# latk/hbetune.rs

Hardware: AMD Instinct MI355X
Metric: GP fit+predict/sec (n=4096,d=8,f64) (higher is better)
Workload: dtype f64; 1 GPU; M: rosenbrock d=8 n=4096 f64, Matern nu=5/2 x constant + white noise; fixed-work fit = 3 L-BFGS runs x 150 lml+gradient evaluations + K^-1, then predict mean+variance at m=1600; evals_per_fit=450, n_not_pd=0, m_candidates=1600, parallelism=replicas x1 (independent fits per GPU, no collective)

## Files before the change

csrc/dag_plan.hpp:

```cpp
#pragma once
#include <algorithm>
#include <cstdint>
#include <cstdio>
#include <queue>
#include <string>
#include <vector>

#include "engine.hpp"

namespace hbegp {

inline int dag_split_point(int lo, int hi) { return lo + (hi - lo) / 2; }

struct DagPlan {
  std::vector<DagTask> tasks;
  std::vector<int> totals;
  double gflop = 0;
  double gflop_lauum = 0;
  int n_lauum = 0;
  int n_leaf = 0;
  double sim_us = 0;
  double crit_us = 0;
};

// ... 444 lines not shown
        }
        uprev[i] = DagGate{c, cnt};
      }
      if (lauum) {
        int a = -1;
        for (const auto& gr : kgroups)
          if (gr.second == k + 1) a = gr.first;
        if (a >= 0) {
          const double gl0 = plan_.gflop;
          const int c = new_counter();
          int cnt = 0;
          const std::vector<DagGate> waits = {rowfin[k], kprev};
          if (a > 0) {
            Op l{};
            l.flags = (uint16_t)(DAGF_ABUF | DAGF_BBUF | DAGF_AKM | DAGF_BKM | DAGF_CKINV | cont);
            l.r0 = 0; l.r1 = a; l.c0 = 0; l.c1 = a; l.lower = true; l.k0 = a; l.k1 = k + 1;
            for (const Tile& tl : tiles_of(l, false)) {
              const DagTask tk = make(l, tl, &cu);
              push(tk, waits, c, -1, cu);
              ++cnt;
              plan_.n_lauum++;
            }
          }
          {
            Op l{};
            l.flags = DAGF_ABUF | DAGF_BBUF | DAGF_AKM | DAGF_BKM | DAGF_CKINV;
            l.r0 = a; l.r1 = k + 1; l.c0 = 0; l.c1 = k + 1; l.lower = true; l.k0 = a; l.k1 = k + 1; l.klim = 4; l.tri_a = true; l.tri_b = true;
            for (const Tile& tl : tiles_of(l, false)) {
              const DagTask tk = make(l, tl, &cu);
              push(tk, waits, c, -1, cu);
              ++cnt;
              plan_.n_lauum++;
            }
          }
          kprev = DagGate{c, cnt};
          g_lauum += plan_.gflop - gl0;
        }
      }
    }
    (void)g0;
    plan_.gflop_lauum = g_lauum;
  }
  Sub rl_inverse(int lo, int hi, const std::vector<RlNode>& nodes, const std::vector<DagGate>& leafc) {
    Sub out;
    out.lo = lo; out.hi = hi;
    if (hi - lo == 1) {
      out.rowfin.assign(1, leafc[lo]);
      out.all = leafc[lo];
      return out;
    }
    const int mid = dag_split_point(lo, hi);
    const RlNode* nd = nullptr;
    for (const RlNode& cand : nodes)
      if (cand.lo == lo && cand.hi == hi) nd = &cand;
    const bool small = std::max(mid - lo, hi - mid) <= small_h_;
    const Sub left = rl_inverse(lo, mid, nodes, leafc);
    const Sub right = rl_inverse(mid, hi, nodes, leafc);
    if (lo == top_lo_ && hi == top_hi_) { top_mid_ = mid; top_right_all_ = right.all; top_left_all_ = left.all; }
    double cu = 0;
    Op u{};
    u.flags = DAGF_A3 | DAGF_BBUF | DAGF_BKM;
    u.r0 = mid; u.r1 = hi; u.c0 = lo; u.c1 = mid; u.k0 = lo; u.k1 = mid; u.klim = 2; u.tri_b = true;
    const std::vector<Tile> ut = tiles_of(u, small);
    const DagGate uall{new_counter(), (int)ut.size()};
    for (const Tile& tl : ut) {
      const DagTask tk = make(u, tl, &cu);
      DagGate lrow{nd->lrow[tl.bi - mid], plan_.totals[nd->lrow[tl.bi - mid]]};
      push(tk, {lrow, left.all}, uall.cnt, -1, cu);
    }
    Op x{};
    x.flags = DAGF_ABUF | DAGF_BKM | DAGF_CBUF | DAGF_NEG;
    x.r0 = mid; x.r1 = hi; x.c0 = lo; x.c1 = mid; x.k0 = mid; x.k1 = hi; x.klim = 3; x.tri_a = true; x.crit = 2;
    const std::vector<Tile> xt = tiles_of(x, small);
    RowGates xrow(hi);
    for (int i = mid; i < hi; ++i) xrow[i] = DagGate{new_counter(), count_row(xt, i)};
    const DagGate xall{new_counter(), (int)xt.size()};
    for (const Tile& tl : xt) {
      const DagTask tk = make(x, tl, &cu);
      push(tk, {fine_ ? right.rowfin[tl.bi - mid] : right.all, uall}, xrow[tl.bi].cnt, xall.cnt, cu);
    }
    out.rowfin.resize(hi - lo);
    for (int j = lo; j < mid; ++j) out.rowfin[j - lo] = left.rowfin[j - lo];
    for (int j = mid; j < hi; ++j) out.rowfin[j - lo] = xrow[j];
    out.all = xall;
    return out;
  }

  void order() {
    const int nt = (int)plan_.tasks.size(), nc = (int)plan_.totals.size();
    std::vector<std::vector<int>> waiters(nc);
    for (int i = 0; i < nt; ++i)
      for (int w = 0; w < plan_.tasks[i].nwait; ++w) waiters[plan_.tasks[i].wcnt[w]].push_back(i);
    std::vector<double> bl(nt, 0.0), blc(nc, 0.0);
    for (int i = nt - 1; i >= 0; --i) {
      const DagTask& t = plan_.tasks[i];
      double tail = 0;
      for (int q = 0; q < DAG_MAXSIG; ++q)
        if (t.sig[q] != DAG_NOSIG) tail = std::max(tail, blc[t.sig[q]]);
      bl[i] = t.cost * 0.1 + tail;
      for (int w = 0; w < t.nwait; ++w) blc[t.wcnt[w]] = std::max(blc[t.wcnt[w]], bl[i]);
    }
    plan_.crit_us = *std::max_element(bl.begin(), bl.end());
    std::vector<int> count(nc, 0), missing(nt, 0);
    typedef std::pair<double, int> Pri;
    std::priority_queue<Pri> ready;
    for (int i = 0; i < nt; ++i) {
      missing[i] = plan_.tasks[i].nwait;
      if (missing[i] == 0) ready.push({bl[i], -i});
    }
    typedef std::pair<double, int> Ev;
    std::priority_queue<Ev, std::vector<Ev>, std::greater<Ev>> running;
    std::vector<DagTask> out;
    out.reserve(nt);
    std::vector<int> out_idx;
    std::vector<double> start(nt, 0.0);
    out_idx.reserve(nt);
    int idle = nwg_;
    double now = 0;
    while ((int)out.size() < nt) {
      while (idle > 0 && !ready.empty()) {
        const int i = -ready.top().second;
        ready.pop();
        out.push_back(plan_.tasks[i]);
        out_idx.push_back(i);
        start[i] = now;
        running.push({now + plan_.tasks[i].cost * 0.1, i});
        --idle;
      }
      if (running.empty()) break;
      const Ev e = running.top();
      running.pop();
      now = e.first;
      ++idle;
      const DagTask& t = plan_.tasks[e.second];
      for (int q = 0; q < DAG_MAXSIG; ++q) {
        if (t.sig[q] == DAG_NOSIG) continue;
        const int c = t.sig[q];
        if (++count[c] == plan_.totals[c])
          for (int wtr : waiters[c])
            if (--missing[wtr] == 0) ready.push({bl[wtr], -wtr});
      }
    }
    while (!running.empty()) { now = running.top().first; running.pop(); }
    if ((int)out.size() == nt) {
      plan_.tasks.swap(out);
      plan_.sim_us = now;
    }
  }

 public:
  void set_big128(bool on, bool with_acc = false) { big128_ = on; big128_acc_ = on && with_acc; }
};

inline std::string dag_plan_validate(const DagPlan& plan, int nblocks_total) {
  const int nc = (int)plan.totals.size(), nt = (int)plan.tasks.size();
  const int words = (nc + 63) / 64;
  char buf[256];
  std::vector<int> count(nc, 0);
  std::vector<uint64_t> counter_known((size_t)nc * words, 0), cur(words);
  const int nt64 = nblocks_total * 4;
  struct Cell { int writer = -1; std::vector<int> readers; };
  constexpr int NBUF = 8;
  std::vector<Cell> cells[NBUF];
  for (int b = 0; b < NBUF; ++b) cells[b].resize((size_t)nt64 * nt64);
  std::vector<std::vector<uint64_t>> known(nt);
  auto hb = [&](int a, int b) -> bool {
    for (int q = 0; q < DAG_MAXSIG; ++q) {
      const int c = plan.tasks[a].sig[q];
      if (c != DAG_NOSIG && ((known[b][c / 64] >> (c % 64)) & 1u) != 0) return true;
    }
    return false;
  };
  for (int i = 0; i < nt; ++i) {
    const DagTask& t = plan.tasks[i];
    if (t.kind == DAG_GEMM_128x128 && (t.flags & DAGF_CINIT)) {
      snprintf(buf, sizeof buf, "task %d: the 128x128 tile cannot continue a sum (flags %x)", i, t.flags);
      return buf;
    }
    if (t.kind == DAG_GEMM_32x64 && (t.flags & (DAGF_AKM | DAGF_BKM | DAGF_CINIT | DAGF_CKINV))) {
      snprintf(buf, sizeof buf, "task %d: the 32x64 one-shot tile reads both operands [outer][k] and writes W1/W2/W3 (flags %x)", i, t.flags);
      return buf;
    }
    if ((t.kind == DAG_GEMM_128x64 || t.kind == DAG_GEMM_64x64) && (t.flags & DAGF_CINIT)) {
      if (!(t.flags & DAGF_ACC) || (t.flags & DAGF_NEG) || t.kend <= t.kbeg) {
        snprintf(buf, sizeof buf, "task %d: DAGF_CINIT needs DAGF_ACC, no DAGF_NEG and a non-empty contraction range (flags %x, k [%d, %d))", i,
                 t.flags, t.kbeg, t.kend);
        return buf;
      }
    }
    std::fill(cur.begin(), cur.end(), 0);
    for (int w = 0; w < t.nwait; ++w) {
      const int c = t.wcnt[w];
      if (c >= nc) return "wait on an unknown counter";
      if (t.wval[w] != plan.totals[c]) {
        snprintf(buf, sizeof buf, "task %d waits for %d of counter %d (total %d): partial waits are not allowed", i, t.wval[w], c, plan.totals[c]);
        return buf;
      }
      if (count[c] < t.wval[w]) {
        snprintf(buf, sizeof buf, "task %d waits on counter %d = %d but only %d earlier tasks bump it: queue order is not topological", i,
                 c, t.wval[w], count[c]);
        return buf;
      }
      cur[c / 64] |= 1ull << (c % 64);
      for (int q = 0; q < words; ++q) cur[q] |= counter_known[(size_t)c * words + q];
    }
    known[i] = cur;
    struct Acc { int buf, r, c; bool write; };
    std::vector<Acc> accs;
    auto rect = [&](int bufi, int r0, int r1, int c0, int c1, bool write) {
      for (int r = r0 / 32; r < (r1 + 31) / 32; ++r)
        for (int c = c0 / 64; c < (c1 + 63) / 64; ++c) accs.push_back({bufi, r, c, write});
    };
    auto cell = [&](int bufi, int r, int c, bool write) { accs.push_back({bufi, r, c, write}); };
    if (t.kind == DAG_LEAF) {
      const int b = t.row0 * 128;
      rect(0, b, b + 128, b, b + 128, false);
      rect(1, b, b + 128, b, b + 128, true);
      cell(4, t.row0, 0, true);
    } else {
      const int ta = (t.kind == DAG_GEMM_128x64 || t.kind == DAG_GEMM_128x128) ? 128 : (t.kind == DAG_GEMM_32x64 ? 32 : 64), tb = t.kind == DAG_GEMM_128x128 ? 128 : 64;
      const int ab = (t.flags & DAGF_A3) ? 7 : ((t.flags & DAGF_ABUF) ? 1 : 0), bb = (t.flags & DAGF_B3) ? 7 : ((t.flags & DAGF_BBUF) ? 1 : 0);
      const int cb = (t.flags & DAGF_CKINV) ? 6 : ((t.flags & DAGF_C3) ? 7 : ((t.flags & DAGF_CBUF) ? 1 : 0));
      if (t.kend <= t.kbeg) return "empty contraction range";
      if (t.flags & DAGF_AKM) rect(ab, t.kbeg, t.kend, t.row0, t.row0 + ta, false);
      else rect(ab, t.row0, t.row0 + ta, t.kbeg, t.kend, false);
      if (t.flags & DAGF_BKM) rect(bb, t.kbeg, t.kend, t.col0, t.col0 + tb, false);
      else rect(bb, t.col0, t.col0 + tb, t.kbeg, t.kend, false);
      if (t.flags & DAGF_ACC) rect(cb, t.row0, t.row0 + ta, t.col0, t.col0 + tb, false);
      rect(cb, t.row0, t.row0 + ta, t.col0, t.col0 + tb, true);
    }
    for (const Acc& a : accs) {
      if (a.r >= nt64 || a.c >= nt64 || a.r < 0 || a.c < 0) return "tile outside the matrix";
      Cell& cell = cells[a.buf][(size_t)a.r * nt64 + a.c];
      if (a.buf >= 2 && a.buf != 6 && !a.write && cell.writer < 0) {
        snprintf(buf, sizeof buf, "task %d reads cell (%d,%d) of buffer %d that no earlier task has written", i, a.r, a.c, a.buf);
        return buf;
      }
      if (cell.writer >= 0 && cell.writer != i && !hb(cell.writer, i)) {
        snprintf(buf, sizeof buf, "task %d %s tile (%d,%d) of W%d written by task %d without waiting for it", i,
                 a.write ? "overwrites" : "reads", a.r, a.c, a.buf + 1, cell.writer);
        return buf;
      }
      if (a.write)
        for (int rd : cell.readers)
          if (rd != i && !hb(rd, i)) {
            snprintf(buf, sizeof buf, "task %d overwrites tile (%d,%d) of W%d that task %d reads, without waiting for it", i, a.r, a.c,
                     a.buf + 1, rd);
            return buf;
          }
    }
    for (const Acc& a : accs) {
      Cell& cell = cells[a.buf][(size_t)a.r * nt64 + a.c];
      if (a.write) { cell.writer = i; cell.readers.clear(); }
      else if (cell.readers.empty() || cell.readers.back() != i) cell.readers.push_back(i);
    }
    for (int sq = 0; sq < DAG_MAXSIG; ++sq) {
      if (t.sig[sq] == DAG_NOSIG) continue;
      const int c = t.sig[sq];
      if (c >= nc) return "bump of an unknown counter";
      count[c]++;
      for (int q = 0; q < words; ++q) counter_known[(size_t)c * words + q] |= cur[q];
    }
  }
  for (int c = 0; c < nc; ++c)
    if (count[c] != plan.totals[c]) return "counter total mismatch";
  return "";
}

}
```

csrc/hbegp.cpp:

```cpp
#include "../include/hbegp.h"

#include <hip/hip_runtime_api.h>

#include <algorithm>
#include <atomic>
#include <queue>
#include <cmath>
#include <cstdarg>
#include <cstdio>
#include <cstdlib>
#include <cstring>
#include <limits>
#include <memory>
#include <mutex>
#include <string>
#include <thread>
#include <type_traits>
#include <vector>

#include "dag_plan.hpp"
#include "engine.hpp"
#include "lbfgsb.hpp"
#include "lbfgs_step.hpp"

// ... 412 lines not shown
    gemm(g, PhaseTimer::GEMM);
  }
  {
    GemmLaunch g{};
    g.nops = need_x ? 2 : 1;
    GemmOp& syrk = g.op[0];
    syrk = base;
    syrk.A = L21; syrk.B = L21; syrk.C = W1;
    syrk.ci0 = mid; syrk.cj0 = mid; syrk.mi = hi - mid; syrk.nj = hi - mid; syrk.c_lower = 1;
    syrk.k0 = lo; syrk.k1 = mid; syrk.alpha_neg = 1; syrk.beta_one = 1;
    GemmOp& u = g.op[1];
    u = base;
    u.A = L21; u.B = W2; u.C = W1;
    u.b_kmajor = 1;
    u.ci0 = mid; u.mi = hi - mid; u.cj0 = lo; u.nj = mid - lo;
    u.k0 = lo; u.k1 = mid; u.klim = 2; u.maskB = 1;
    gemm(g, PhaseTimer::GEMM);
  }
  chol_inv_rec<T>(W1, W2, L21, ld, mid, mid + (hi - mid) / 2, hi, false, need_x, gemm, leaf);
  if (need_x) {
    GemmLaunch g{};
    g.nops = 1;
    GemmOp& op = g.op[0];
    op = base;
    op.A = W2; op.B = W1; op.C = W2;
    op.b_kmajor = 1;
    op.ci0 = mid; op.mi = hi - mid; op.cj0 = lo; op.nj = mid - lo;
    op.k0 = mid; op.k1 = hi; op.klim = 3; op.maskA = 1; op.alpha_neg = 1;
    gemm(g, PhaseTimer::GEMM);
  }
}

static double op_gflop(const GemmOp& op) {
  double pairs = 0;
  for (int i = 0; i < op.mi; ++i)
    for (int j = 0; j < (op.c_lower ? i + 1 : op.nj); ++j) {
      const int ti = op.ci0 + i, tj = op.cj0 + j;
      int ka = op.k0, kb = op.k1;
      if (op.klim == 1) kb = std::min(kb, tj + 1);
      if (op.klim == 2) ka = std::max(ka, tj);
      if (op.klim == 3) kb = std::min(kb, ti + 1);
      if (op.klim == 4) ka = std::max(ka, ti);
      for (int k = ka; k < kb; ++k) {
        double w = 1.0;
        if ((op.maskA && k == ti) || (op.maskB && k == tj)) w = 0.5;
        if (op.c_lower && ti == tj) w = std::min(w, 0.5);
        pairs += w;
      }
    }
  return pairs * 2.0 * 128.0 * 128.0 * 128.0 * 1e-9;
}

struct Sched {
  int* d_off = nullptr;
  unsigned* d_items = nullptr;
  int nwg = 0;
  int tile = 0;
};

static void tile_krange(const GemmOp& op, int ti, int tj, int* ka, int* kb) {
  *ka = op.k0; *kb = op.k1;
  if (op.klim == 1) *kb = std::min(*kb, tj + 1);
  if (op.klim == 2) *ka = std::max(*ka, tj);
  if (op.klim == 3) *kb = std::min(*kb, ti + 1);
  if (op.klim == 4) *ka = std::max(*ka, ti);
}

static bool build_sched(const GemmLaunch& g, int tile, std::vector<int>* off, std::vector<unsigned>* items, int* nwg_out) {
  const int f = NB / tile;
  struct It { double w; unsigned code; };
  std::vector<It> its;
  for (int oi = 0; oi < g.nops; ++oi) {
    GemmOp op = g.op[oi];
    op.ci0 *= f; op.cj0 *= f; op.mi *= f; op.nj *= f; op.k0 *= f; op.k1 *= f;
    for (int i = 0; i < op.mi; ++i)
      for (int j = 0; j < (op.c_lower ? i + 1 : op.nj); ++j) {
        int ka, kb;
        tile_krange(op, op.ci0 + i, op.cj0 + j, &ka, &kb);
        its.push_back({(double)(kb - ka) + 0.75, ((unsigned)oi << 30) | ((unsigned)i << 16) | (unsigned)j});
      }
  }
  const int ntiles = (int)its.size();
  const int occmax = tile == 128 ? 2 : 3;
  int nwg = 0;
  if (ntiles < 2048)
    for (int occ = occmax; occ >= 1; --occ)
      if (ntiles >= 2 * 256 * occ) { nwg = 256 * occ; break; }
  if (nwg == 0) return false;
  std::stable_sort(its.begin(), its.end(), [](const It& a, const It& b) { return a.w > b.w; });
  typedef std::pair<double, int> Load;
  std::priority_queue<Load, std::vector<Load>, std::greater<Load>> pq;
  for (int w = 0; w < nwg; ++w) pq.push({0.0, w});
  std::vector<std::vector<unsigned>> per(nwg);
  for (const It& it : its) {
    Load l = pq.top();
    pq.pop();
    per[l.second].push_back(it.code);
    pq.push({l.first + it.w, l.second});
  }
  off->assign(nwg + 1, 0);
  items->clear();
  for (int w = 0; w < nwg; ++w) {
    (*off)[w] = (int)items->size();
    items->insert(items->end(), per[w].begin(), per[w].end());
  }
  (*off)[nwg] = (int)items->size();
  *nwg_out = nwg;
  return true;
}

constexpr int DAG_MAX_VARIANTS = 4;
constexpr int DAG_CROWD_LEVELS = 3;
constexpr int DAG_CROWD_BUSY[DAG_CROWD_LEVELS] = {6, 12, 24};
constexpr int MAX_DEVS = 64;
struct DagPlanKey {
  int blocks, bk, small_h, nwg, lauum, rl, rl_group, rl_near, lauum_split, chain32, prog, big128;
  auto tie() const { return std::tie(blocks, bk, small_h, nwg, lauum, rl, rl_group, rl_near, lauum_split, chain32, prog, big128); }
  bool operator<(const DagPlanKey& o) const { return tie() < o.tie(); }
};
static std::atomic<int> g_dev_busy[MAX_DEVS];

template <typename T>
struct LooIn {
  int dev;
  hipStream_t s;
  int n, d, np, nu2;
  const T *X, *y, *alpha, *Xinv, *Kinv;
  const EvalParams* P;
};
template <typename T>
static int loo_tail(const LooIn<T>& in, T* mean, T* var, T* lpd, double* loo, double* grad);

template <typename T>
struct Slot {
  int dev = 0;
  hipStream_t stream = nullptr;
  T *Xalt = nullptr, *ldalt = nullptr;
  bool x_captured = false;
  T *W1 = nullptr, *W2 = nullptr, *Kinv[2] = {nullptr, nullptr}, *alpha[2] = {nullptr, nullptr};
  T* W3 = nullptr;
  T *ldiag = nullptr, *wbuf = nullptr;
  double *part_t = nullptr, *part_g = nullptr;
  EvalParams* dP = nullptr;
  EvalOut* dOut = nullptr;
  int* tickets = nullptr;
  unsigned long long* dag_trace = nullptr;
  int* dag_ctrl = nullptr;
  EvalParams* hP = nullptr;
  EvalOut* hOut = nullptr;
  void* small_slab = nullptr;
  size_t small_slab_bytes = 0;
  void* host_slab = nullptr;
  size_t host_slab_bytes = 0;
  hipGraphExec_t graph[DAG_MAX_VARIANTS + 1 + DAG_CROWD_LEVELS][2][2] = {};
  int best_idx = -1;
  double best_lml = -std::numeric_limits<double>::infinity();
  int best_run = 0, best_eval = 0;
  std::vector<double> best_theta;
  std::vector<double> best_params;
  int last_target = 0;
  int dag_variant = 1;
  unsigned long long seq = 0;
  bool ctrl_cleared = false;
  bool published = false;
  long long expect_ns = 0;
};

struct ProblemBase {
  hbegp_ctx* ctx = nullptr;
  int n = 0, d = 0, np = 0, nu2 = 5, n_slots = 1;
  bool is_f32 = false;
  virtual ~ProblemBase() {}
  virtual int eval(int dev, int slot, const double* theta, const double* lo, const double* hi, double* lml, double* grad) = 0;
  virtual int eval_loo(int dev, int slot, const double* theta, const double* lo, const double* hi, double* loo, double* grad) = 0;
  virtual int time_eval(int dev, int slot, const double* theta, int reps, double* phase_ms) = 0;
  virtual int time_concurrent(int dev, const double* theta, int reps, double* out) = 0;
};
struct hbegp_problem {
  std::unique_ptr<ProblemBase> impl;
};

template <typename T>
struct Problem : ProblemBase {
  std::vector<T*> Xd, yd;
  std::vector<std::vector<Slot<T>>> slots;
  std::vector<std::vector<Sched>> scheds;
  bool dag_ = false;
  bool dag_lauum_ = false;
  bool dag_rl_ = false;
  double dag_gflop_lauum = 0;
  struct DagVariant {
    int nwg = 0;
    std::vector<DagTask*> tasks;
    std::vector<DagTask> host_tasks;
  };
  std::vector<DagVariant> dag_var;
  std::unique_ptr<std::atomic<int>[]> busy_slots_;
  int dag_ntasks = 0, dag_nwg = 0;
  int dag_nvar_ = 1, dag_ncrowd_ = 0;
  unsigned long long dag_wait_ticks_ = 200000000ull;
  size_t dag_ctrl_bytes = 0;
  double dag_gflop = 0;
  bool adhoc_ = false;
  bool small_ = false;
  bool like_fit_ = false;
  bool hostio_ = true;
  bool eval_published() const { return hostio_ && !small_; }
  int leaf_dbg_ = 0;

  struct Pooled { int dev; void* p; size_t bytes; };
  std::vector<Pooled> pooled_;
  template <typename U>
  U* palloc(int dev, size_t count) {
    bool fresh = false;
    const size_t bytes = std::max<size_t>(16, sizeof(U) * count);
    void* q = g_pool.get(dev, bytes, &fresh);
    pooled_.push_back({dev, q, bytes});
    return static_cast<U*>(q);
  }

  Problem(hbegp_ctx* c, const T* X, const T* y, int n_, int d_, double nu, int n_slots_, bool single_shot = false, bool like_fit = false) {
    try {
      adhoc_ = single_shot;
      like_fit_ = like_fit;
      init(c, X, y, n_, d_, nu, n_slots_);
    } catch (...) {
      release();
      throw;
    }
  }

  void init(hbegp_ctx* c, const T* X, const T* y, int n_, int d_, double nu, int n_slots_) {
    ctx = c; n = n_; d = d_; np = round_up(n_, NB); n_slots = n_slots_;
    nu2 = std::isinf(nu) ? 0 : (int)std::lround(2 * nu);
    is_f32 = sizeof(T) == 4;
    leaf_dbg_ = env_int("HBEGP_LEAF_DBG", 0) & 16;
    small_ = np == NB && d <= SMALL_EVAL_MAXD && env_int("HBEGP_SMALL", 1) != 0;
    hostio_ = env_int("HBEGP_HOSTIO", 1) != 0;
    const size_t nn = (size_t)np * np;
    Xd.assign(c->devs.size(), nullptr);
    yd.assign(c->devs.size(), nullptr);
    slots.resize(c->devs.size());
    for (size_t di = 0; di < c->devs.size(); ++di) {
      HIPCHECK(hipSetDevice(c->devs[di]));
      slots[di].resize(n_slots);
      for (auto& s : slots[di]) {
        s.dev = c->devs[di];
        s.stream = g_stream_pool.get(s.dev);
      }
      hipStream_t st0 = slots[di][0].stream;
      Xd[di] = palloc<T>(c->devs[di], (size_t)n * d);
      yd[di] = palloc<T>(c->devs[di], np);
      HIPCHECK(hipMemsetAsync(yd[di], 0, sizeof(T) * np, st0));
      HIPCHECK(hipMemcpyAsync(Xd[di], X, sizeof(T) * (size_t)n * d, hipMemcpyHostToDevice, st0));
      HIPCHECK(hipMemcpyAsync(yd[di], y, sizeof(T) * n, hipMemcpyHostToDevice, st0));
      for (auto& s : slots[di]) {
        bool fresh1 = false, fresh2 = false, fk = false;
        s.W1 = static_cast<T*>(g_pool.get(s.dev, sizeof(T) * nn, &fresh1));
        s.W2 = static_cast<T*>(g_pool.get(s.dev, sizeof(T) * nn, &fresh2));
        for (int b = 0; b < 2; ++b) s.Kinv[b] = static_cast<T*>(g_pool.get(s.dev, sizeof(T) * nn, &fk));
        HIPCHECK(hipMemsetAsync(s.W2, 0, sizeof(T) * nn, st0));
        (void)fresh1; (void)fresh2; (void)fk;
        {
          auto up = [](size_t v) { return (v + 255) / 256 * 256; };
          const size_t b_vec = up(sizeof(T) * np);
          const size_t b_part_t = up(sizeof(double) * ((size_t)((np + 255) / 256) * np + 2 * (size_t)((np + 255) / 256) + 64));
          const size_t b_part_g = up(sizeof(double) * gradtrace_part_elems(np, d));
          const size_t b_p = up(sizeof(EvalParams)), b_o = up(sizeof(EvalOut));
          s.small_slab_bytes = 4 * b_vec + b_part_t + b_part_g + b_p + b_o + 256;
          bool fs = false;
          s.small_slab = g_pool.get(s.dev, s.small_slab_bytes, &fs);
          char* q = static_cast<char*>(s.small_slab);
          s.alpha[0] = reinterpret_cast<T*>(q); q += b_vec;
          s.alpha[1] = reinterpret_cast<T*>(q); q += b_vec;
          s.ldiag = reinterpret_cast<T*>(q); q += b_vec;
          s.wbuf = reinterpret_cast<T*>(q); q += b_vec;
          s.part_t = reinterpret_cast<double*>(q); q += b_part_t;
          s.part_g = reinterpret_cast<double*>(q); q += b_part_g;
          s.dP = reinterpret_cast<EvalParams*>(q); q += b_p;
          s.dOut = reinterpret_cast<EvalOut*>(q); q += b_o;
          s.tickets = reinterpret_cast<int*>(q);
          HIPCHECK(hipMemsetAsync(s.dOut, 0, b_o + 256, st0));
          const size_t h_p = up(sizeof(EvalParams));
          s.host_slab_bytes = h_p + up(sizeof(EvalOut));
          s.host_slab = g_host_pool.get(s.host_slab_bytes);
          s.hP = reinterpret_cast<EvalParams*>(s.host_slab);
          s.hOut = reinterpret_cast<EvalOut*>(static_cast<char*>(s.host_slab) + h_p);
          memset(s.hP, 0, sizeof(EvalParams));
          memset(s.hOut, 0, sizeof(EvalOut));
        }
      }
      HIPCHECK(hipStreamSynchronize(st0));
    }
    const int dag_env = env_int("HBEGP_DAG", -1);
    const int dag_min_blocks = env_int("HBEGP_DAG_MIN_BLOCKS", DAG_MIN_BLOCKS_FIT);
    dag_ = (dag_env < 0 ? np / NB >= dag_min_blocks : dag_env != 0) && !adhoc_ && np / NB >= 2;
    if (dag_) {
      int cus = 1 << 30;
      for (int dev : c->devs) {
        hipDeviceProp_t prop;
        HIPCHECK(hipGetDeviceProperties(&prop, dev));
        cus = std::min(cus, std::max(1, prop.multiProcessorCount));
      }
      const int forced = env_int("HBEGP_DAG_WG", 0);
      auto share_of = [&](int busy) {
        const int share = busy <= 1 ? cus : std::max(8, (cus * 112 / 100 / busy + 4) / 8 * 8);
        return forced > 0 ? forced : std::max(1, std::min(cus, share));
      };
      dag_lauum_ = env_int("HBEGP_DAG_LAUUM", 1) != 0;
      dag_rl_ = env_int("HBEGP_DAG_RL", np / NB <= 80 ? 1 : 0) != 0;
      static std::mutex cache_mu;
      static std::map<DagPlanKey, std::shared_ptr<const DagPlan>> cache;
      auto plan_for = [&](int nwg) {
        const DagPlanKey key = {np / NB, dag_stage_depth(is_f32), env_int("HBEGP_DAG_SMALLH", dag_rl_ ? 4 : 8), nwg, dag_lauum_, dag_rl_,
                                env_int("HBEGP_DAG_RL_GROUP", 32), env_int("HBEGP_DAG_RL_NEAR", 1),
                                env_int("HBEGP_DAG_LAUUM_SPLIT", n_slots <= 1 ? 1 : 0),
                                env_int("HBEGP_DAG_CHAIN32", 1),
                                env_int("HBEGP_DAG_PROG", np / NB <= DAG_PROG_MAX_BLOCKS ? 1 : 0),
                                env_int("HBEGP_DAG_BIG128", ((n_slots >= 2 && np / NB >= 32) || np / NB >= 64) ? 2 : 0)};
        std::shared_ptr<const DagPlan> cached;
        {
          std::lock_guard<std::mutex> lk(cache_mu);
          auto it = cache.find(key);
          if (it != cache.end()) cached = it->second;
        }
        if (!cached) {
          DagBuilder builder(key.bk, key.small_h, key.nwg);
          builder.set_rl(key.rl_group, key.rl_near, key.lauum_split != 0, key.chain32 != 0);
          builder.set_rl_progressive(key.prog != 0);
          builder.set_big128(key.big128 != 0, key.big128 >= 2);
          cached = std::make_shared<const DagPlan>(builder.build(0, np / NB, dag_lauum_, dag_rl_));
          std::lock_guard<std::mutex> lk(cache_mu);
          if (cache.size() > 64) cache.clear();
          cache[key] = cached;
        }
        return cached;
      };
      const int nvar = std::min(n_slots, DAG_MAX_VARIANTS);
      dag_nwg = share_of(n_slots);
      std::shared_ptr<const DagPlan> cached = plan_for(dag_nwg);
      if (cached->tasks.empty() && dag_rl_) {
        dag_rl_ = false;
        cached = plan_for(dag_nwg);
      }
      const DagPlan& plan = *cached;
      if (plan.tasks.empty()) dag_ = dag_lauum_ = false;
      if (dag_ && env_int("HBEGP_DAG_VALIDATE", 0)) {
        const std::string why = dag_plan_validate(plan, np / NB);
        if (!why.empty()) throw std::runtime_error("task queue of the factorisation is unsound: " + why);
      }
      if (dag_) {
        dag_ntasks = (int)plan.tasks.size();
        dag_nwg = std::min(dag_nwg, dag_ntasks);
        dag_gflop = plan.gflop;
        dag_gflop_lauum = plan.gflop_lauum;
        dag_ctrl_bytes = (sizeof(int) * (DAG_CTRL_WORDS + plan.totals.size()) + 15) / 16 * 16;
        dag_wait_ticks_ = (unsigned long long)(std::max(2.0, 200.0 * plan.sim_us * 1e-6 * std::max(1, n_slots)) * 1e8);
        busy_slots_.reset(new std::atomic<int>[c->devs.size()]);
        for (size_t di = 0; di < c->devs.size(); ++di) busy_slots_[di].store(0);
        const bool adapt = env_int("HBEGP_DAG_ADAPT", 1) != 0 && forced <= 0;
        dag_nvar_ = nvar;
        dag_ncrowd_ = (adapt && n_slots > 1) ? DAG_CROWD_LEVELS : 0;
        dag_var.assign(nvar + 1 + dag_ncrowd_, DagVariant());
        for (int v = 1; v <= nvar + dag_ncrowd_; ++v) {
          DagVariant& var = dag_var[v];
          std::shared_ptr<const DagPlan> pv = cached;
          var.nwg = dag_nwg;
          if (v != nvar && adapt) {
            const int busy = v < nvar ? v : DAG_CROWD_BUSY[v - nvar - 1];
            var.nwg = std::min(share_of(busy), dag_ntasks);
            if (v > nvar) var.nwg = std::min(var.nwg, dag_nwg);
            pv = plan_for(var.nwg);
            if (pv->tasks.size() != plan.tasks.size()) { pv = cached; var.nwg = dag_nwg; }
          }
          var.host_tasks = pv->tasks;
          var.tasks.assign(c->devs.size(), nullptr);
          for (size_t di = 0; di < c->devs.size(); ++di) {
            HIPCHECK(hipSetDevice(c->devs[di]));
            var.tasks[di] = palloc<DagTask>(c->devs[di], pv->tasks.size());
            HIPCHECK(hipMemcpyAsync(var.tasks[di], var.host_tasks.data(), sizeof(DagTask) * var.host_tasks.size(), hipMemcpyHostToDevice, slots[di][0].stream));
          }
        }
        for (size_t di = 0; di < c->devs.size(); ++di) {
          HIPCHECK(hipSetDevice(c->devs[di]));
          for (auto& s : slots[di]) {
            if (dag_rl_) {
              bool f3 = false;
              s.W3 = static_cast<T*>(g_pool.get(s.dev, sizeof(T) * nn, &f3));
            }
            s.dag_ctrl = palloc<int>(s.dev, dag_ctrl_bytes / sizeof(int));
            HIPCHECK(hipMemsetAsync(s.dag_ctrl, 0, dag_ctrl_bytes, slots[di][0].stream));
            if (getenv("HBEGP_DAG_TRACE")) {
              s.dag_trace = palloc<unsigned long long>(s.dev, 5 * plan.tasks.size());
              HIPCHECK(hipMemsetAsync(s.dag_trace, 0, sizeof(unsigned long long) * 5 * plan.tasks.size(), slots[di][0].stream));
            }
          }
          HIPCHECK(hipStreamSynchronize(slots[di][0].stream));
        }
      }
    }
    scheds.resize(c->devs.size());
    if (adhoc_ || small_) return;
    for (size_t di = 0; di < c->devs.size(); ++di) {
      HIPCHECK(hipSetDevice(c->devs[di]));
      Slot<T>& s = slots[di][0];
      auto record = [&](GemmLaunch& g, int) {
        Sched sc;
        sc.tile = pick_tile(g);
        std::vector<int> off;
        std::vector<unsigned> items;
        int nwg = 0;
        if (build_sched(g, sc.tile, &off, &items, &nwg)) {
          sc.nwg = nwg;
          sc.d_off = palloc<int>(s.dev, off.size());
          sc.d_items = palloc<unsigned>(s.dev, items.size());
          HIPCHECK(hipMemcpyAsync(sc.d_off, off.data(), sizeof(int) * off.size(), hipMemcpyHostToDevice, s.stream));
          HIPCHECK(hipMemcpyAsync(sc.d_items, items.data(), sizeof(unsigned) * items.size(), hipMemcpyHostToDevice, s.stream));
          HIPCHECK(hipStreamSynchronize(s.stream));
        }
        scheds[di].push_back(sc);
      };
      eval_gemms(s, s.Kinv[0], record, [](int) {}, [] {});
    }
  }
  ~Problem() override { release(); }

  void release() {
    for (size_t di = 0; di < slots.size(); ++di) {
      (void)hipSetDevice(ctx->devs[di]);
      for (auto& s : slots[di]) {
        if (s.stream) (void)hipStreamSynchronize(s.stream);
        for (int v = 0; v <= DAG_MAX_VARIANTS + DAG_CROWD_LEVELS; ++v)
          for (int a = 0; a < 2; ++a)
            for (int b = 0; b < 2; ++b)
              if (s.graph[v][a][b]) (void)hipGraphExecDestroy(s.graph[v][a][b]);
        const size_t nnb = sizeof(T) * (size_t)np * np;
        g_pool.put(s.dev, s.W1, nnb); g_pool.put(s.dev, s.W2, nnb); g_pool.put(s.dev, s.W3, nnb);
        for (int b = 0; b < 2; ++b) g_pool.put(s.dev, s.Kinv[b], nnb);
        g_pool.put(s.dev, s.small_slab, s.small_slab_bytes);
        g_host_pool.put(s.host_slab, s.host_slab_bytes);
        g_stream_pool.put(s.dev, s.stream);
      }
    }
    for (const Pooled& q : pooled_) g_pool.put(q.dev, q.p, q.bytes);
    pooled_.clear();
    slots.clear();
    scheds.clear();
    dag_var.clear();
    Xd.clear();
    yd.clear();
  }

  auto scheduled(Slot<T>& s, size_t di, PhaseTimer* tm) {
    return [this, &s, di, tm, ord = 0](GemmLaunch& g, int kind) mutable {
      if (adhoc_) return gemm_adhoc<T>(g, &s.dOut->info, s.stream);
      const Sched& sc = scheds[di][ord++];
      g.info = &s.dOut->info;
      g.sched_off = sc.nwg ? sc.d_off : nullptr;
      g.sched_items = sc.nwg ? sc.d_items : nullptr;
      g.sched_nwg = sc.nwg;
      double gf = 0;
      if (tm)
        for (int i = 0; i < g.nops; ++i) gf += op_gflop(g.op[i]);
      if (tm) tm->begin(kind, sc.tile, gf);
      launch_gemm<T>(g, sc.tile, s.stream);
      if (tm) tm->end();
    };
  }

  auto leaf_step(Slot<T>& s, PhaseTimer* tm) {
    return [this, &s, tm](int k) {
      if (tm) tm->begin(PhaseTimer::LEAF);
      launch_leaf<T>(s.W1, s.W2, np, k, s.ldiag, &s.dOut->info, s.stream, leaf_dbg_);
      if (tm) tm->end();
    };
  }

  template <class Gemm, class Leaf, class Alpha>
  void eval_gemms(Slot<T>& s, T* Kinv, Gemm&& gemm, Leaf&& leaf, Alpha&& alpha) {
    const int nb = np / NB;
    if (!dag_) chol_inv_rec<T>(s.W1, s.W2, s.W2, np, 0, nb / 2, nb, false, true, gemm, leaf);
    alpha();
    if (!(dag_ && dag_lauum_)) {
      GemmLaunch g{};
      g.nops = 1;
      GemmOp& op = g.op[0];
      op.lda = op.ldb = op.ldc = np;
      op.A = s.W2; op.B = s.W2; op.C = Kinv;
      op.a_kmajor = 1; op.b_kmajor = 1;
      op.ci0 = 0; op.cj0 = 0; op.mi = nb; op.nj = nb; op.c_lower = 1;
      op.k0 = 0; op.k1 = nb; op.klim = 4; op.maskA = 1; op.maskB = 1;
      gemm(g, PhaseTimer::LAUUM);
    }
  }

  void dag_report_timeout(Slot<T>& s) {
    if (!s.dag_ctrl) return;
    std::vector<int> ctrl(dag_ctrl_bytes / sizeof(int));
    if (hipMemcpyAsync(ctrl.data(), s.dag_ctrl, dag_ctrl_bytes, hipMemcpyDeviceToHost, s.stream) != hipSuccess || hipStreamSynchronize(s.stream) != hipSuccess) return;
    const int row = ctrl[1] - 1;
    fprintf(stderr, "task queue timeout: queue head %d of %d, first task that gave up: %d\n", ctrl[0], dag_ntasks, row);
    const std::vector<DagTask>& host_tasks = dag_var[s.dag_variant].host_tasks;
    if (row >= 0 && row < (int)host_tasks.size()) {
      const DagTask& t = host_tasks[row];
      fprintf(stderr, "  kind %d flags %x row0 %d col0 %d k [%d, %d) waits:", t.kind, t.flags, t.row0, t.col0, t.kbeg, t.kend);
      for (int w = 0; w < t.nwait; ++w) fprintf(stderr, " c%d=%d/%d", t.wcnt[w], ctrl[DAG_CTRL_WORDS + t.wcnt[w]], t.wval[w]);
      fprintf(stderr, "\n");
    }
    (void)hipGetLastError();
  }

  void launch_queue(Slot<T>& s, size_t di, T* Kinv, PhaseTimer* tm) {
    if (!s.ctrl_cleared) HIPCHECK(hipMemsetAsync(s.dag_ctrl, 0, dag_ctrl_bytes, s.stream));
    s.ctrl_cleared = false;
    DagLaunch g{};
    const DagVariant& var = dag_var[s.dag_variant];
    g.tasks = var.tasks[di]; g.ntasks = dag_ntasks; g.ctrl = s.dag_ctrl;
    g.W1 = s.W1; g.W2 = s.W2; g.ld = np; g.ldiag = s.ldiag; g.info = &s.dOut->info;
    g.W3 = s.W3;
    g.Kinv = dag_lauum_ ? Kinv : nullptr;
    g.trace = s.dag_trace;
    g.wait_ticks = dag_wait_ticks_;
    g.leaf_dbg = leaf_dbg_;
    if (tm) tm->begin(PhaseTimer::DAG, 0, g.Kinv ? dag_gflop : dag_gflop - dag_gflop_lauum);
    launch_dag<T>(g, var.nwg, s.stream);
    if (tm) tm->end();
  }

  void small_eval(Slot<T>& s, size_t di, int target, int mode) {
    SmallEval g{};
    g.X = Xd[di]; g.y = yd[di]; g.n = n; g.d = d;
    g.W2 = s.W2; g.ldiag = s.ldiag; g.Kinv = s.Kinv[target]; g.alpha = s.alpha[target]; g.out = s.dOut; g.mode = mode;
    g.P = s.hP; g.hout = s.hOut;
    launch_small_eval<T>(g, nu2, s.stream);
  }

  void enqueue_eval(Slot<T>& s, size_t di, int target, bool want_grad, PhaseTimer* tm) {
    const int* info = &s.dOut->info;
    if (small_) {
      if (tm) tm->begin(PhaseTimer::LEAF);
      small_eval(s, di, target, 1 | 2 | (want_grad ? 4 : 0));
      if (tm) tm->end();
      CHECK_LAUNCHES();
      return;
    }
    const bool hostio = eval_published();
    if (hostio) {
      EvalPrologue pro;
      pro.dP = s.dP; pro.out = s.dOut;
      if (dag_) {
        pro.ctrl = s.dag_ctrl; pro.ctrl_words = (int)(dag_ctrl_bytes / sizeof(int));
        s.ctrl_cleared = true;
      }
      if (tm) tm->begin(PhaseTimer::KMAT);
      launch_kmat<T>(Xd[di], n, d, np, nu2, s.hP, s.W1, info, s.stream, &pro);
      if (tm) tm->end();
    } else {
      HIPCHECK(hipMemcpyAsync(s.dP, s.hP, sizeof(EvalParams), hipMemcpyHostToDevice, s.stream));
      launch_reset_out(s.dOut, s.stream);
      if (tm) tm->begin(PhaseTimer::KMAT);
      launch_kmat<T>(Xd[di], n, d, np, nu2, s.dP, s.W1, info, s.stream);
      if (tm) tm->end();
    }
    if (dag_) launch_queue(s, di, s.Kinv[target], tm);
    eval_gemms(s, s.Kinv[target], scheduled(s, di, tm), leaf_step(s, tm), [&] {
      if (tm) tm->begin(PhaseTimer::ALPHA);
      launch_alpha_lml<T>(s.W2, np, n, yd[di], s.ldiag, s.wbuf, s.part_t, s.alpha[target], s.dOut, info, s.stream, hostio ? s.tickets : nullptr);
      if (tm) tm->end();
    });
    bool fuse_grad = false;
    if (want_grad) {
      if (tm) tm->begin(PhaseTimer::GRAD);
      fuse_grad = hostio && (np / 64) * (np / 64 + 1) / 2 <= 512;
      launch_gradtrace<T>(Xd[di], n, d, np, nu2, s.dP, s.Kinv[target], s.alpha[target], s.part_g, s.dOut, info, s.stream,
                          fuse_grad ? s.tickets + 1 : nullptr, fuse_grad ? s.hOut : nullptr);
      if (tm) tm->end();
    }
    if (hostio) {
      if (!want_grad || !fuse_grad) launch_publish_out(s.dOut, s.hOut, s.dP, s.stream);
      s.published = true;
    }
    CHECK_LAUNCHES();
    if (!hostio) {
      HIPCHECK(hipMemcpyAsync(s.hOut, s.dOut, sizeof(EvalOut), hipMemcpyDeviceToHost, s.stream));
      s.published = false;
    }
  }

  void wait_eval(Slot<T>& s, std::chrono::steady_clock::time_point t_launch) {
    if (s.published) {
      using namespace std::chrono;
      const volatile unsigned long long* q = &s.hOut->seq;
      if (s.expect_ns > 1500000) {
        const long long margin = std::max<long long>(300000, s.expect_ns / 8);
        std::this_thread::sleep_until(t_launch + nanoseconds(s.expect_ns - margin));
        if (*q == s.seq) {
          std::atomic_thread_fence(std::memory_order_acquire);
          s.expect_ns = s.expect_ns * 9 / 10;
          return;
        }
      }
      const auto t0 = steady_clock::now();
      for (unsigned it = 1;; ++it) {
        if (*q == s.seq) {
          std::atomic_thread_fence(std::memory_order_acquire);
          s.expect_ns = duration_cast<nanoseconds>(steady_clock::now() - t_launch).count();
          return;
        }
        __builtin_ia32_pause();
        if ((it & 4095u) == 0 && steady_clock::now() - t0 > seconds(2)) {
          static std::atomic<bool> said{false};
          if (!said.exchange(true))
            fprintf(stderr, "hbegp: an evaluation did not publish its serial number within 2 s; falling back to hipStreamSynchronize\n");
          break;
        }
      }
    }
    HIPCHECK(hipStreamSynchronize(s.stream));
  }

  int factor_only(size_t di, int si) {
    Slot<T>& s = slots[di][si];
    HIPCHECK(hipSetDevice(s.dev));
    s.dag_variant = variant_now(di);
    HIPCHECK(hipMemcpyAsync(s.dP, s.hP, sizeof(EvalParams), hipMemcpyHostToDevice, s.stream));
    launch_reset_out(s.dOut, s.stream);
    if (small_) {
      small_eval(s, di, 0, 0);
      CHECK_LAUNCHES();
      HIPCHECK(hipStreamSynchronize(s.stream));
      return s.hOut->info != 0 ? HBEGP_NOT_PD : HBEGP_OK;
    }
    launch_kmat<T>(Xd[di], n, d, np, nu2, s.dP, s.W1, &s.dOut->info, s.stream);
    const int nb = np / NB;
    if (dag_) launch_queue(s, di, nullptr, nullptr);
    else chol_inv_rec<T>(s.W1, s.W2, s.W2, np, 0, nb / 2, nb, false, true, scheduled(s, di, nullptr), leaf_step(s, nullptr));
    CHECK_LAUNCHES();
    HIPCHECK(hipMemcpyAsync(s.hOut, s.dOut, sizeof(EvalOut), hipMemcpyDeviceToHost, s.stream));
    HIPCHECK(hipStreamSynchronize(s.stream));
    if (s.hOut->info < 0) {
      dag_report_timeout(s);
      throw HipError{hipErrorLaunchTimeOut, "factorisation task queue: a dependency wait exceeded its bound", __LINE__};
    }
    return s.hOut->info != 0 ? HBEGP_NOT_PD : HBEGP_OK;
  }

  int extend_from(size_t di, int si, const T* pX, const T* pXinv, const T* pKinv, const T* pldiag, int pn, int pnp) {
    Slot<T>& s = slots[di][si];
    HIPCHECK(hipSetDevice(s.dev));
    const int nb = np / NB, q0 = std::min(pn / NB, nb - 1);
    if (q0 < 1 || pn > n) return HBEGP_EINVAL;
    const int* info = &s.dOut->info;
    HIPCHECK(hipMemcpyAsync(s.dP, s.hP, sizeof(EvalParams), hipMemcpyHostToDevice, s.stream));
    launch_reset_out(s.dOut, s.stream);
    launch_prefix_differs<T>(Xd[di], pX, (size_t)pn * d, &s.dOut->n_warn, s.stream);
    CHECK_LAUNCHES();
    HIPCHECK(hipMemcpyAsync(s.hOut, s.dOut, sizeof(EvalOut), hipMemcpyDeviceToHost, s.stream));
    HIPCHECK(hipStreamSynchronize(s.stream));
    if (s.hOut->n_warn != 0) {
      HIPCHECK(hipMemsetAsync(&s.dOut->n_warn, 0, sizeof(int), s.stream));
      return HBEGP_EINVAL;
    }
    const size_t w = (size_t)q0 * NB;
    HIPCHECK(hipMemcpy2DAsync(s.W2, sizeof(T) * np, pXinv, sizeof(T) * pnp, sizeof(T) * w, w, hipMemcpyDeviceToDevice, s.stream));
    HIPCHECK(hipMemcpy2DAsync(s.Kinv[0], sizeof(T) * np, pKinv, sizeof(T) * pnp, sizeof(T) * w, w, hipMemcpyDeviceToDevice, s.stream));
    HIPCHECK(hipMemcpyAsync(s.ldiag, pldiag, sizeof(T) * w, hipMemcpyDeviceToDevice, s.stream));
    launch_kmat<T>(Xd[di], n, d, np, nu2, s.dP, s.W1, info, s.stream);
    chol_inv_rec<T>(s.W1, s.W2, s.W2, np, 0, q0, nb, true, true, [&](GemmLaunch& g, int) { gemm_adhoc<T>(g, info, s.stream); },
                    leaf_step(s, nullptr));
    launch_alpha_lml<T>(s.W2, np, n, yd[di], s.ldiag, s.wbuf, s.part_t, s.alpha[0], s.dOut, info, s.stream);
    if (pnp / NB > q0) {
      GemmLaunch gf{};
      gf.nops = 1;
      GemmOp& fix = gf.op[0];
      fix.A = pXinv; fix.B = pXinv; fix.C = s.Kinv[0];
      fix.lda = fix.ldb = pnp; fix.ldc = np;
      fix.a_kmajor = 1; fix.b_kmajor = 1;
      fix.mi = fix.nj = q0; fix.c_lower = 1;
      fix.k0 = q0; fix.k1 = pnp / NB; fix.alpha_neg = 1; fix.beta_one = 1;
      gemm_adhoc<T>(gf, info, s.stream);
    }
    GemmLaunch g{};
    GemmOp base{};
    base.lda = base.ldb = base.ldc = np;
    base.A = s.W2; base.B = s.W2; base.C = s.Kinv[0];
    base.a_kmajor = 1; base.b_kmajor = 1;
    base.k0 = q0; base.k1 = nb; base.maskA = 1; base.maskB = 1;
    GemmOp& keep = g.op[g.nops++];
    keep = base; keep.mi = keep.nj = q0; keep.c_lower = 1; keep.beta_one = 1;
    GemmOp& rect = g.op[g.nops++];
    rect = base; rect.ci0 = q0; rect.mi = nb - q0; rect.nj = q0; rect.klim = 4;
    GemmOp& tri = g.op[g.nops++];
    tri = base; tri.ci0 = tri.cj0 = q0; tri.mi = tri.nj = nb - q0; tri.c_lower = 1; tri.klim = 4;
    gemm_adhoc<T>(g, info, s.stream);
    CHECK_LAUNCHES();
    HIPCHECK(hipMemcpyAsync(s.hOut, s.dOut, sizeof(EvalOut), hipMemcpyDeviceToHost, s.stream));
    HIPCHECK(hipStreamSynchronize(s.stream));
    s.last_target = 0;
    if (s.hOut->info == 0 && !(s.hOut->done & 1)) throw HipError{hipErrorLaunchFailure, "extend: the evaluation kernels did not run", __LINE__};
    return s.hOut->info != 0 ? HBEGP_NOT_PD : HBEGP_OK;
  }

  int variant_now(size_t di) const {
    if (!dag_ || dag_var.size() < 2) return 1;
    const int nvar = dag_nvar_;
    const int busy = busy_slots_ ? busy_slots_[di].load(std::memory_order_relaxed) : 0;
    if (dag_ncrowd_ > 0) {
      const int dev = ctx->devs[di];
      const int total = dev < MAX_DEVS ? g_dev_busy[dev].load(std::memory_order_relaxed) : 0;
      if (total > std::max(busy, nvar)) {
        int l = 0;
        while (l + 1 < dag_ncrowd_ && DAG_CROWD_BUSY[l] < total) ++l;
        return nvar + 1 + l;
      }
    }
    return busy <= 0 ? nvar : std::min(busy, nvar);
  }
  int run_eval(size_t di, int si, int target, bool want_grad, bool use_graph, double* lml, double* grad) {
    Slot<T>& s = slots[di][si];
    HIPCHECK(hipSetDevice(s.dev));
    static const bool graphs_on = env_int("HBEGP_NO_GRAPH", 0) == 0;
    s.dag_variant = variant_now(di);
    s.hP->seq = ++s.seq;
    const auto t_launch = std::chrono::steady_clock::now();
    if (use_graph && graphs_on) {
      hipGraphExec_t& ge = s.graph[s.dag_variant][target][want_grad ? 1 : 0];
      if (!ge) {
        hipGraph_t gr = nullptr;
        HIPCHECK(hipStreamBeginCapture(s.stream, hipStreamCaptureModeThreadLocal));
        try {
          enqueue_eval(s, di, target, want_grad, nullptr);
        } catch (...) {
          (void)hipStreamEndCapture(s.stream, &gr);
          throw;
        }
        HIPCHECK(hipStreamEndCapture(s.stream, &gr));
        HIPCHECK(hipGraphInstantiate(&ge, gr, nullptr, nullptr, 0));
        HIPCHECK(hipGraphDestroy(gr));
      }
      HIPCHECK(hipGraphLaunch(ge, s.stream));
    } else {
      enqueue_eval(s, di, target, want_grad, nullptr);
    }
    s.published = eval_published();
    wait_eval(s, t_launch);
    s.last_target = target;
    const int p = d + 2;
    if (s.hOut->info < 0) {
      dag_report_timeout(s);
      throw HipError{hipErrorLaunchTimeOut, "factorisation task queue: a dependency wait exceeded its bound", __LINE__};
    }
    if (s.hOut->info != 0) {
      *lml = -std::numeric_limits<double>::infinity();
      if (grad) for (int j = 0; j < p; ++j) grad[j] = 0.0;
      return HBEGP_NOT_PD;
    }
    if (!(s.hOut->done & 1) || (want_grad && !(s.hOut->done & 2)))
      throw HipError{hipErrorLaunchFailure, "evaluation: the lml/gradient kernels did not run", __LINE__};
    *lml = s.hOut->lml;
    if (grad) for (int j = 0; j < p; ++j) grad[j] = s.hOut->grad[j];
    bool finite = std::isfinite(*lml);
    if (grad) for (int j = 0; j < p; ++j) finite = finite && std::isfinite(grad[j]);
    if (!finite) {
      auto poisoned = [](double v) { unsigned long long b; memcpy(&b, &v, 8); return b == 0x7ff8000000005eedull; };
      bool never_written = poisoned(s.hOut->lml);
      if (grad) for (int j = 0; j < p; ++j) never_written = never_written || poisoned(s.hOut->grad[j]);
      if (never_written) throw HipError{hipErrorLaunchFailure, "evaluation: an output of the lml/gradient kernels was never written", __LINE__};
    }
    if (!finite) {
      *lml = -std::numeric_limits<double>::infinity();
      if (grad) for (int j = 0; j < p; ++j) grad[j] = 0.0;
      return HBEGP_NOT_PD;
    }
    return HBEGP_OK;
  }

  int eval(int dev, int slot, const double* theta, const double* lo, const double* hi, double* lml, double* grad) override {
    if (dev < 0 || dev >= (int)slots.size() || slot < 0 || slot >= n_slots) return fail(HBEGP_EINVAL, "bad device/slot index");
    Slot<T>& s = slots[dev][slot];
    theta_to_params(theta, lo, hi, d, s.hP);
    const int target = (s.best_idx < 0) ? 0 : 1 - s.best_idx;
    return run_eval((size_t)dev, slot, target, grad != nullptr, true, lml, grad);
  }

  int loo_on_slot(size_t di, int si, double* loo, double* grad) {
    Slot<T>& s = slots[di][si];
    const LooIn<T> in{s.dev, s.stream, n, d, np, nu2, Xd[di], yd[di], s.alpha[s.last_target], s.W2, s.Kinv[s.last_target], s.hP};
    return loo_tail<T>(in, nullptr, nullptr, nullptr, loo, grad);
  }

  int eval_loo(int dev, int slot, const double* theta, const double* lo, const double* hi, double* loo, double* grad) override {
    double lml;
    const int st = eval(dev, slot, theta, lo, hi, &lml, nullptr);
    if (st != HBEGP_OK) {
      if (st == HBEGP_NOT_PD) {
        *loo = -std::numeric_limits<double>::infinity();
        if (grad) for (int j = 0; j < d + 2; ++j) grad[j] = 0.0;
      }
      return st;
    }
    return loo_on_slot((size_t)dev, slot, loo, grad);
  }

  int time_eval(int dev, int slot, const double* theta, int reps, double* phase_ms) override {
    if (dev < 0 || dev >= (int)slots.size() || slot < 0 || slot >= n_slots) return fail(HBEGP_EINVAL, "bad device/slot index");
    Slot<T>& s = slots[dev][slot];
    HIPCHECK(hipSetDevice(s.dev));
    theta_to_params(theta, nullptr, nullptr, d, s.hP);
    double lml;
    std::vector<double> grad(d + 2);
    int st = run_eval((size_t)dev, slot, 0, true, true, &lml, grad.data());
    if (st != HBEGP_OK) return st;
    hipEvent_t e0, e1;
    HIPCHECK(hipEventCreate(&e0));
    HIPCHECK(hipEventCreate(&e1));
    HIPCHECK(hipEventRecord(e0, s.stream));
    hipGraphExec_t timed_graph = s.graph[s.dag_variant][0][1];
    for (int r = 0; r < reps; ++r) {
      if (timed_graph) HIPCHECK(hipGraphLaunch(timed_graph, s.stream));
      else enqueue_eval(s, (size_t)dev, 0, true, nullptr);
    }
    HIPCHECK(hipEventRecord(e1, s.stream));
    HIPCHECK(hipEventSynchronize(e1));
    float ms = 0;
    HIPCHECK(hipEventElapsedTime(&ms, e0, e1));
    if (phase_ms) {
      for (int i = 0; i < 24; ++i) phase_ms[i] = 0;
      phase_ms[6] = ms / reps;
      const int treps = std::max(1, std::min(reps, 3));
      for (int r = 0; r < treps; ++r) {
        PhaseTimer tm;
        tm.s = s.stream;
        hipEvent_t t0, t1;
        HIPCHECK(hipEventCreate(&t0));
        HIPCHECK(hipEventCreate(&t1));
        HIPCHECK(hipEventRecord(t0, s.stream));
        enqueue_eval(s, (size_t)dev, 0, true, &tm);
        HIPCHECK(hipEventRecord(t1, s.stream));
        HIPCHECK(hipStreamSynchronize(s.stream));
        float tot = 0;
        HIPCHECK(hipEventElapsedTime(&tot, t0, t1));
        phase_ms[14] += tot / treps;
        for (auto& rec : tm.recs) {
          float dt = 0;
          HIPCHECK(hipEventElapsedTime(&dt, rec.a, rec.b));
          const double v = dt / treps;
          if (rec.kind == PhaseTimer::KMAT) phase_ms[0] += v;
          if (rec.kind == PhaseTimer::GEMM) { phase_ms[1] += v; phase_ms[7] += 1.0 / treps; }
          if (rec.kind == PhaseTimer::LEAF) { phase_ms[2] += v; phase_ms[15] += 1.0 / treps; }
          if (rec.kind == PhaseTimer::LAUUM) phase_ms[3] += v;
          if (rec.kind == PhaseTimer::ALPHA) phase_ms[4] += v;
          if (rec.kind == PhaseTimer::GRAD) phase_ms[5] += v;
          if (rec.kind == PhaseTimer::DAG) { phase_ms[19] += v; phase_ms[20] += rec.gflop / treps; }
          if (rec.kind == PhaseTimer::GEMM || rec.kind == PhaseTimer::LAUUM) {
            const int o = rec.tile == 128 ? 8 : (rec.tile == 64 ? 10 : 12);
            phase_ms[o] += v;
            phase_ms[o + 1] += rec.gflop / treps;
            phase_ms[rec.tile == 128 ? 16 : (rec.tile == 64 ? 17 : 18)] += 1.0 / treps;
          }
          (void)hipEventDestroy(rec.a);
          (void)hipEventDestroy(rec.b);
        }
        (void)hipEventDestroy(t0);
        (void)hipEventDestroy(t1);
      }
    }
    (void)hipEventDestroy(e0);
    (void)hipEventDestroy(e1);
    if (s.dag_trace && getenv("HBEGP_DAG_TRACE")) {
      if (timed_graph) HIPCHECK(hipGraphLaunch(timed_graph, s.stream));
      HIPCHECK(hipStreamSynchronize(s.stream));
      const std::vector<DagTask>& dag_host_tasks = dag_var[s.dag_variant].host_tasks;
      std::vector<unsigned long long> tr((size_t)5 * dag_ntasks);
      HIPCHECK(hipMemcpyAsync(tr.data(), s.dag_trace, sizeof(unsigned long long) * tr.size(), hipMemcpyDeviceToHost, s.stream));
      HIPCHECK(hipStreamSynchronize(s.stream));
      if (FILE* f = fopen(getenv("HBEGP_DAG_TRACE"), "w")) {
        for (int i = 0; i < dag_ntasks; ++i) {
          const DagTask& t = dag_host_tasks[i];
          fprintf(f, "%d %d %d %d %d %d %llu %llu %llu %llu %llu %llu\n", i, t.kind, t.row0, t.col0, t.kend - t.kbeg, t.nwait, tr[5 * i], tr[5 * i + 1],
                  tr[5 * i + 2], tr[5 * i + 3], tr[5 * i + 4] >> 32, tr[5 * i + 4] & 0xffffffffull);
        }
        fclose(f);
      }
    }
    return HBEGP_OK;
  }

  int time_concurrent(int dev, const double* theta, int reps, double* out) override {
    if (dev < 0 || dev >= (int)slots.size()) return fail(HBEGP_EINVAL, "bad device index");
    const size_t di = (size_t)dev;
    const int ns = n_slots;
    for (int i = 0; i < 16; ++i) out[i] = 0;
    out[1] = ns;
    out[10] = dag_ ? dag_nwg : 0;
    std::string err;
    std::mutex err_mu;
    std::vector<double> acc(12, 0.0);
    std::mutex acc_mu;
    for (int pass = 0; pass < 3; ++pass) {
      std::atomic<int> arrived{0};
      std::vector<double> wall(ns, 0.0);
      auto worker = [&](int si) {
        try {
          Slot<T>& s = slots[di][si];
          HIPCHECK(hipSetDevice(s.dev));
          theta_to_params(theta, nullptr, nullptr, d, s.hP);
          std::vector<double> grad(d + 2);
          double lml;
          arrived.fetch_add(1);
// ... 957 lines not shown
template <typename T>
static void paths_eval_locked(hbegp_paths* p, const T* Xs, int cnt, int per_path, T* f, T* df) {
  hbegp_model* m = p->model;
  hipStream_t s = m->stream;
  const int d = m->d, S = p->S;
  const size_t per_point = sizeof(double) * (size_t)paths_eval_chunks(m->n, p->F) * S * (d + 1);
  const int mb = (int)std::max<size_t>(1, std::min<size_t>({(size_t)cnt, PATHS_EVAL_ROWS / (size_t)S, PATHS_EVAL_PART / per_point}));
  p->grow(&p->Xs, &p->cap_x, sizeof(T) * (size_t)(per_path ? S : 1) * mb * d);
  p->grow(&p->part, &p->cap_part, per_point * mb);
  p->grow(&p->f, &p->cap_f, sizeof(T) * (size_t)S * mb);
  if (df) p->grow(&p->df, &p->cap_df, sizeof(T) * (size_t)S * mb * d);
  for (int p0 = 0; p0 < cnt; p0 += mb) {
    const int c = std::min(mb, cnt - p0);
    if (per_path)
      HIPCHECK(hipMemcpy2DAsync(p->Xs, sizeof(T) * (size_t)c * d, Xs + (size_t)p0 * d, sizeof(T) * (size_t)cnt * d, sizeof(T) * (size_t)c * d, S,
                                hipMemcpyHostToDevice, s));
    else
      HIPCHECK(hipMemcpyAsync(p->Xs, Xs + (size_t)p0 * d, sizeof(T) * (size_t)c * d, hipMemcpyHostToDevice, s));
    launch_paths_eval<T>(static_cast<T*>(p->Xs), c, per_path, S, static_cast<T*>(m->X), m->n, d, m->np, m->nu2, m->dP, static_cast<T*>(p->Vt),
                         p->omT, p->phase, p->Wf, p->F, df ? 1 : 0, static_cast<double*>(p->part), static_cast<T*>(p->f),
                         static_cast<T*>(p->df), s);
    CHECK_LAUNCHES();
    HIPCHECK(hipMemcpy2DAsync(f + p0, sizeof(T) * (size_t)cnt, p->f, sizeof(T) * (size_t)c, sizeof(T) * (size_t)c, S, hipMemcpyDeviceToHost, s));
    if (df)
      HIPCHECK(hipMemcpy2DAsync(df + (size_t)p0 * d, sizeof(T) * (size_t)cnt * d, p->df, sizeof(T) * (size_t)c * d, sizeof(T) * (size_t)c * d, S,
                                hipMemcpyDeviceToHost, s));
    HIPCHECK(hipStreamSynchronize(s));
  }
}

template <typename T>
static int paths_eval(hbegp_paths* p, const T* Xs, int cnt, int per_path, T* f, T* df) {
  std::lock_guard<std::mutex> lock(p->model->mu);
  HIPCHECK(hipSetDevice(p->model->dev));
  paths_eval_locked<T>(p, Xs, cnt, per_path, f, df);
  return HBEGP_OK;
}

template <typename T>
static int paths_minimize(hbegp_paths* p, const T* starts, int R, const double* lo, const double* hi, int maxeval, T* x_best, double* f_best,
                          int* n_evals) {
  hbegp_model* m = p->model;
  std::lock_guard<std::mutex> lock(m->mu);
  HIPCHECK(hipSetDevice(m->dev));
  const int d = m->d, S = p->S;
  const size_t NR = (size_t)S * R;
  const LbfgsOptions o;
  std::vector<LbfgsState> st(NR);
  std::vector<char> running(NR, 1);
  std::vector<double> best(S, std::numeric_limits<double>::infinity());
  std::vector<double> x0(d), g(d);
  for (size_t r = 0; r < NR; ++r) {
    for (int k = 0; k < d; ++k) x0[k] = (double)starts[r * d + k];
    lbfgs_begin(st[r], x0.data(), lo, hi, d, maxeval, o.memory, o.pgtol, o.ftol, false);
  }
  for (int sp = 0; sp < S; ++sp)
    for (int k = 0; k < d; ++k) x_best[(size_t)sp * d + k] = starts[(size_t)sp * R * d + k];
  std::vector<std::vector<int>> act(S);
  std::vector<T> xs, fv, dfv;
  for (;;) {
    int mr = 0;
    for (int sp = 0; sp < S; ++sp) {
      act[sp].clear();
      for (int r = 0; r < R; ++r)
        if (running[(size_t)sp * R + r]) act[sp].push_back(r);
      mr = std::max(mr, (int)act[sp].size());
    }
    if (mr == 0) break;
    xs.assign((size_t)S * mr * d, T(0));
    fv.resize((size_t)S * mr);
    dfv.resize((size_t)S * mr * d);
    for (int sp = 0; sp < S; ++sp) {
      T* row = xs.data() + (size_t)sp * mr * d;
      const int na = (int)act[sp].size();
      for (int i = 0; i < mr; ++i) {
        if (i < na) {
          const double* q = lbfgs_request(st[(size_t)sp * R + act[sp][i]]);
          for (int k = 0; k < d; ++k) row[(size_t)i * d + k] = to_box<T>(q[k], lo[k], hi[k]);
        } else {
          const T* src = i > 0 ? row + (size_t)(i - 1) * d : x_best + (size_t)sp * d;
          for (int k = 0; k < d; ++k) row[(size_t)i * d + k] = src[k];
        }
      }
    }
    paths_eval_locked<T>(p, xs.data(), mr, 1, fv.data(), dfv.data());
    for (int sp = 0; sp < S; ++sp) {
      for (int i = 0; i < (int)act[sp].size(); ++i) {
        const size_t r = (size_t)sp * R + act[sp][i], at = (size_t)sp * mr + i;
        double fx = (double)fv[at];
        bool ok = std::isfinite(fx);
        for (int k = 0; k < d; ++k) {
          g[k] = (double)dfv[at * d + k];
          ok = ok && std::isfinite(g[k]);
        }
        if (!ok) {
          fx = std::numeric_limits<double>::infinity();
          for (int k = 0; k < d; ++k) g[k] = 0.0;
        } else if (fx < best[sp]) {
          best[sp] = fx;
          for (int k = 0; k < d; ++k) x_best[(size_t)sp * d + k] = xs[at * d + k];
        }
        running[r] = lbfgs_advance(st[r], fx, g.data()) ? 1 : 0;
      }
    }
  }
  for (int sp = 0; sp < S; ++sp) {
    f_best[sp] = best[sp];
    if (n_evals) {
      n_evals[sp] = 0;
      for (int r = 0; r < R; ++r) n_evals[sp] += st[(size_t)sp * R + r].nevals;
    }
  }
  return HBEGP_OK;
}

template <typename T>
static int check_paths_create(hbegp_model* model, const T* omega0, const T* phase, const T* w, int F, int S, hbegp_paths** paths) {
  if (F < 1 || F > HBEGP_PATHS_MAX_FEATURES) return fail(HBEGP_EINVAL, "F must be in [1, %d] (got %d)", HBEGP_PATHS_MAX_FEATURES, F);
  if (S < 1 || S > HBEGP_PATHS_MAX_PATHS) return fail(HBEGP_EINVAL, "S must be in [1, %d] (got %d)", HBEGP_PATHS_MAX_PATHS, S);
  if (!model) return fail(HBEGP_EINVAL, "NULL model");
  if (!omega0 || !phase || !w || !paths) return fail(HBEGP_EINVAL, "omega0/phase/w/paths is NULL");
  if (model->is_f32 != (sizeof(T) == 4)) return fail(HBEGP_EINVAL, "model holds %s data", model->is_f32 ? "f32" : "f64");
  return HBEGP_OK;
}
template <typename T>
static int check_paths_eval(hbegp_paths* paths, const T* Xs, int m, int per_path, T* f) {
  if (m < 0) return fail(HBEGP_EINVAL, "m must be >= 0 (got %d)", m);
  if (per_path != 0 && per_path != 1) return fail(HBEGP_EINVAL, "per_path must be 0 or 1 (got %d)", per_path);
  if (!paths) return fail(HBEGP_EINVAL, "NULL paths handle");
  if (paths->is_f32 != (sizeof(T) == 4)) return fail(HBEGP_EINVAL, "paths handle holds %s data", paths->is_f32 ? "f32" : "f64");
  if (m > 0 && (!Xs || !f)) return fail(HBEGP_EINVAL, "Xs/f is NULL");
  return HBEGP_OK;
}
template <typename T>
static int check_paths_minimize(hbegp_paths* paths, const T* starts, int R, const double* lo, const double* hi, int maxeval, T* x_best,
                                double* f_best) {
  if (R < 1) return fail(HBEGP_EINVAL, "R must be >= 1 (got %d)", R);
  if (maxeval < 1) return fail(HBEGP_EINVAL, "maxeval must be >= 1 (got %d)", maxeval);
  if (!paths) return fail(HBEGP_EINVAL, "NULL paths handle");
  if (!starts || !lo || !hi || !x_best || !f_best) return fail(HBEGP_EINVAL, "starts/lo/hi/x_best/f_best is NULL");
  if (paths->is_f32 != (sizeof(T) == 4)) return fail(HBEGP_EINVAL, "paths handle holds %s data", paths->is_f32 ? "f32" : "f64");
  const int d = paths->model->d;
  if (d > LBFGS_MAXN) return fail(HBEGP_EINVAL, "d = %d exceeds the optimiser's %d variables", d, LBFGS_MAXN);
  for (int k = 0; k < d; ++k)
    if (!(lo[k] <= hi[k])) return fail(HBEGP_EINVAL, "lo[%d] > hi[%d] (%g > %g)", k, k, lo[k], hi[k]);
  for (size_t r = 0; r < (size_t)paths->S * R; ++r)
    for (int k = 0; k < d; ++k) {
      const double v = (double)starts[r * d + k];
      if (!(v >= lo[k] && v <= hi[k])) return fail(HBEGP_EINVAL, "start %zu lies outside the box (feature %d: %g)", r, k, v);
    }
  return HBEGP_OK;
}

static int read_fit_options(const hbegp_fit_options* in, hbegp_fit_options* out) {
  *out = hbegp_fit_options{};
  out->struct_size = sizeof(hbegp_fit_options);
  if (!in) return HBEGP_OK;
  if (in->struct_size < offsetof(hbegp_fit_options, maxeval) + sizeof(int) || in->struct_size > ((size_t)1 << 16))
    return fail(HBEGP_EINVAL, "hbegp_fit_options.struct_size = %zu: set it to sizeof(hbegp_fit_options) (HBEGP_FIT_OPTIONS_INIT)",
                in->struct_size);
  memcpy(out, in, std::min(in->struct_size, sizeof(*out)));
  return HBEGP_OK;
}

template <typename T>
static int do_extend(hbegp_ctx* ctx, const T* X, const T* y, int n, int d, double nu, const double* theta, const double* lo,
                     const double* hi, hbegp_model** model_out);

template <typename T>
static int do_fit(hbegp_ctx* ctx, const T* X, const T* y, int n, int d, double nu, const double* theta0, const double* lo,
                  const double* hi, const double* starts, int n_restarts, const hbegp_fit_options* opt_in,
                  double* theta_best, double* lml_best, hbegp_model** model_out, bool loo = false) {
  hbegp_fit_options opt{};
  if (int e = read_fit_options(opt_in, &opt)) return e;
  if (opt.maxeval <= 0) opt.maxeval = 150;
  const int p = d + 2;
  const int nruns = 1 + std::max(0, n_restarts);
  const int ndev = (int)ctx->devs.size();
  const int max_conc = std::max(1, env_int("HBEGP_MAX_CONCURRENT", 3));
  std::vector<int> runs_on(ndev, 0);
  for (int r = 0; r < nruns; ++r) runs_on[r % ndev]++;
  int n_slots = 1;
  for (int di = 0; di < ndev; ++di) n_slots = std::max(n_slots, std::min(runs_on[di], max_conc));
  constexpr int SMALL_FIT_MAX_RUNS = 64;
  bool small_fit = !loo && round_up(n, NB) == NB && d <= SMALL_EVAL_MAXD && env_int("HBEGP_SMALL", 1) != 0 && env_int("HBEGP_SMALL_FIT", 1) != 0;
  for (int di = 0; di < ndev; ++di) small_fit = small_fit && runs_on[di] <= SMALL_FIT_MAX_RUNS;
  if (small_fit)
    for (int di = 0; di < ndev; ++di) n_slots = std::max(n_slots, runs_on[di]);
  static const int timing = env_int("HBEGP_TIMING", 0);
  const auto tf0 = std::chrono::steady_clock::now();
  SmallArrival arrival;
  if (small_fit) arrival.announce();
  static const int host_serial_max = env_int("HBEGP_SMALL_HOST_SERIAL", 16);
  struct SmallActive {
    bool on = false;
    int enter() { on = true; return g_small_active.fetch_add(1) + 1; }
    ~SmallActive() { if (on) g_small_active.fetch_sub(1); }
  } small_active;
  const bool host_serial = small_fit && small_active.enter() <= host_serial_max;
  std::unique_lock<std::mutex> host_lk(g_small_host_mu, std::defer_lock);
  if (host_serial) host_lk.lock();
  const auto th0 = std::chrono::steady_clock::now();
  double held_ms = 0;
  Problem<T> prob(ctx, X, y, n, d, nu, n_slots, false, true);
  const auto tf1 = std::chrono::steady_clock::now();
  if (!(small_fit && prob.small_)) arrival.arrived();
  if (!(small_fit && prob.small_) && host_lk.owns_lock()) host_lk.unlock();

  std::vector<double> lnlo(p), lnhi(p);
  for (int i = 0; i < p; ++i) {
    lnlo[i] = std::log(lo[i]);
    lnhi[i] = std::log(hi[i]);
  }
  std::mutex trace_mu;
  int trace_n = 0;
  std::atomic<int> n_evals{0}, n_not_pd{0};
  std::string err;
  std::mutex err_mu;

  if (small_fit && prob.small_) {
    struct RunWs {
      int di = 0, si = 0, run = 0;
      LbfgsState* st = nullptr;
      SmallFitResult* res = nullptr;
      double *x0 = nullptr, *tr_theta = nullptr, *tr_lml = nullptr, *tr_grad = nullptr;
    };
    const int cap = opt.trace_cap > 0 ? opt.maxeval : 0;
    std::vector<RunWs> ws(nruns);
    struct alignas(64) HostRun {
      SmallFitResult res;
      unsigned long long done;
    };
    const size_t hruns_bytes = (sizeof(HostRun) * (size_t)nruns + 4095) / 4096 * 4096;
    HostRun* hruns = static_cast<HostRun*>(g_host_pool.get(hruns_bytes));
    std::vector<std::shared_ptr<SmallBatch>> batches(ndev);
    bool runs_over = false;
    auto free_all = [&]() {
      for (auto& b : batches) small_batch_leave(b, runs_over);
      batches.clear();
      g_host_pool.put(hruns, hruns_bytes);
    };
    try {
      std::vector<int> next_slot(ndev, 0);
      std::vector<std::vector<SmallFit>> fits_on(ndev);
      std::vector<double*> boxes_dev(ndev, nullptr);
      std::vector<std::vector<double>> boxes_host(ndev);
      for (int r = 0; r < nruns; ++r) {
        RunWs& w = ws[r];
        w.di = r % ndev; w.si = next_slot[w.di]++; w.run = r;
        HIPCHECK(hipSetDevice(ctx->devs[w.di]));
        Slot<T>& s = prob.slots[w.di][w.si];
        hipStream_t st = prob.slots[w.di][0].stream;
        static_assert(sizeof(LbfgsState) + sizeof(SmallFitResult) + 3 * MAXP * sizeof(double) + 64 <= (size_t)NB * NB * sizeof(float),
                      "the run's workspace fits the slot's W1");
        char* base = reinterpret_cast<char*>(s.W1);
        w.st = reinterpret_cast<LbfgsState*>(base);
        w.res = reinterpret_cast<SmallFitResult*>(base + (sizeof(LbfgsState) + 15) / 16 * 16);
        if (!boxes_dev[w.di]) {
          boxes_dev[w.di] = prob.template palloc<double>(s.dev, (size_t)runs_on[w.di] * 3 * p);
          boxes_host[w.di].assign((size_t)runs_on[w.di] * 3 * p, 0.0);
        }
        w.x0 = boxes_dev[w.di] + (size_t)w.si * 3 * p;
        if (cap > 0) {
          w.tr_theta = prob.template palloc<double>(s.dev, (size_t)cap * p);
          w.tr_lml = prob.template palloc<double>(s.dev, cap);
          w.tr_grad = prob.template palloc<double>(s.dev, (size_t)cap * p);
        }
        const double* start = r == 0 ? theta0 : starts + (size_t)(r - 1) * p;
        double* box = boxes_host[w.di].data() + (size_t)w.si * 3 * p;
        memcpy(box, start, sizeof(double) * p);
        memcpy(box + p, lo, sizeof(double) * p);
        memcpy(box + 2 * p, hi, sizeof(double) * p);
        SmallFit f{};
        f.ev.X = prob.Xd[w.di]; f.ev.y = prob.yd[w.di]; f.ev.n = n; f.ev.d = d; f.ev.P = s.dP;
        f.ev.W2 = s.W2; f.ev.ldiag = s.ldiag; f.ev.out = s.dOut; f.ev.hout = s.dOut;
        f.Kinv[0] = s.Kinv[0]; f.Kinv[1] = s.Kinv[1]; f.alpha[0] = s.alpha[0]; f.alpha[1] = s.alpha[1];
        if (!s.Xalt) {
          s.Xalt = prob.template palloc<T>(s.dev, (size_t)NB * NB);
          s.ldalt = prob.template palloc<T>(s.dev, NB);
          HIPCHECK(hipMemsetAsync(s.Xalt, 0, sizeof(T) * NB * NB, st));
        }
        f.Xinv[0] = s.W2; f.Xinv[1] = s.Xalt; f.ldiag[0] = s.ldiag; f.ldiag[1] = s.ldalt;
        s.x_captured = true;
        f.st = w.st; f.x0 = w.x0; f.lo = w.x0 + p; f.hi = w.x0 + 2 * p;
        LbfgsOptions lo_opt;
        f.maxeval = opt.maxeval; f.memory = opt.lbfgs_memory > 0 ? opt.lbfgs_memory : lo_opt.memory; f.fixed_work = opt.fixed_work != 0;
        f.pgtol = lo_opt.pgtol; f.ftol = lo_opt.ftol;
        f.res = w.res; f.trace_theta = w.tr_theta; f.trace_lml = w.tr_lml; f.trace_grad = w.tr_grad; f.trace_cap = cap;
        hruns[r].done = 0;
        f.hres = &hruns[r].res; f.hdone = &hruns[r].done;
        fits_on[w.di].push_back(f);
      }
      for (int di = 0; di < ndev; ++di) {
        if (fits_on[di].empty()) continue;
        HIPCHECK(hipSetDevice(ctx->devs[di]));
        HIPCHECK(hipMemcpyAsync(boxes_dev[di], boxes_host[di].data(), sizeof(double) * boxes_host[di].size(), hipMemcpyHostToDevice, prob.slots[di][0].stream));
        HIPCHECK(hipStreamSynchronize(prob.slots[di][0].stream));
      }
      held_ms += std::chrono::duration<double, std::milli>(std::chrono::steady_clock::now() - th0).count();
      if (host_lk.owns_lock()) host_lk.unlock();
      for (int di = 0; di < ndev; ++di) {
        if (fits_on[di].empty()) continue;
        HIPCHECK(hipSetDevice(ctx->devs[di]));
        batches[di] = small_batch_submit<T>(ctx->devs[di], prob.nu2, fits_on[di], arrival);
      }
      auto wait_run = [&](int r, int di) {
        using namespace std::chrono;
        const volatile unsigned long long* q = &hruns[r].done;
        auto last_query = steady_clock::now();
        for (unsigned it = 1;; ++it) {
          if (*q == 1ull) break;
          if (it < 256) {
            __builtin_ia32_pause();
          } else {
            std::this_thread::sleep_for(microseconds(40));
            if (steady_clock::now() - last_query > milliseconds(20)) {
              last_query = steady_clock::now();
              const hipError_t e = hipStreamQuery(batches[di]->stream);
              if (e == hipSuccess) {
                if (*q == 1ull) break;
                throw HipError{hipErrorLaunchFailure, "small fit: the launch is over and a run never reported", __LINE__};
              }
              if (e != hipErrorNotReady) throw HipError{e, "hipStreamQuery (small-fit launch)", __LINE__};
            }
          }
        }
        std::atomic_thread_fence(std::memory_order_acquire);
      };
      for (int r = 0; r < nruns; ++r) wait_run(r, ws[r].di);
      runs_over = true;
      int total_evals = 0, total_not_pd = 0, trace_n = 0;
      for (int r = 0; r < nruns; ++r) {
        RunWs& w = ws[r];
        HIPCHECK(hipSetDevice(ctx->devs[w.di]));
        Slot<T>& s = prob.slots[w.di][w.si];
        hipStream_t st = prob.slots[w.di][0].stream;
        const SmallFitResult hr = hruns[r].res;
        total_evals += hr.n_evals;
        total_not_pd += hr.n_not_pd;
        s.best_idx = hr.best_idx;
        s.best_lml = hr.best_lml;
        s.best_run = r;
        s.best_eval = hr.best_eval;
        s.best_theta.assign(hr.best_theta, hr.best_theta + p);
        s.best_params.assign(hr.best_params, hr.best_params + p);
        s.last_target = hr.best_idx < 0 ? 0 : hr.best_idx;
        if (cap > 0 && trace_n < opt.trace_cap) {
          const int take = std::min(std::min(hr.n_evals, cap), opt.trace_cap - trace_n);
          if (opt.trace_theta) HIPCHECK(hipMemcpyAsync(opt.trace_theta + (size_t)trace_n * p, w.tr_theta, sizeof(double) * (size_t)take * p, hipMemcpyDeviceToHost, st));
          if (opt.trace_lml) HIPCHECK(hipMemcpyAsync(opt.trace_lml + trace_n, w.tr_lml, sizeof(double) * take, hipMemcpyDeviceToHost, st));
          if (opt.trace_grad) HIPCHECK(hipMemcpyAsync(opt.trace_grad + (size_t)trace_n * p, w.tr_grad, sizeof(double) * (size_t)take * p, hipMemcpyDeviceToHost, st));
          HIPCHECK(hipStreamSynchronize(st));
          if (opt.trace_run) for (int e = 0; e < take; ++e) opt.trace_run[trace_n + e] = r;
          trace_n += take;
        }
      }
      if (opt.trace_count) *opt.trace_count = trace_n;
      if (opt.n_evals) *opt.n_evals = total_evals;
      if (opt.n_not_pd) *opt.n_not_pd = total_not_pd;
      n_evals.store(total_evals);
    } catch (...) {
      for (int di = 0; di < ndev && di < (int)prob.slots.size(); ++di) {
        if (prob.slots[di].empty()) continue;
        (void)hipSetDevice(ctx->devs[di]);
        (void)hipStreamSynchronize(prob.slots[di][0].stream);
      }
      free_all();
      throw;
    }
    free_all();
  } else {
  if (prob.busy_slots_)
    for (int di = 0; di < ndev; ++di) prob.busy_slots_[di].store(std::min(runs_on[di], max_conc));
  auto worker = [&](int di, int si) {
    struct Leave {
      std::atomic<int>* busy;
      std::atomic<int>* dev_busy;
      ~Leave() {
        if (busy) busy->fetch_sub(1);
        if (dev_busy) dev_busy->fetch_sub(1);
      }
    } leave{prob.busy_slots_ ? &prob.busy_slots_[di] : nullptr, ctx->devs[di] < MAX_DEVS ? &g_dev_busy[ctx->devs[di]] : nullptr};
    if (leave.dev_busy) leave.dev_busy->fetch_add(1);
    try {
      HIPCHECK(hipSetDevice(ctx->devs[di]));
      Slot<T>& s = prob.slots[di][si];
      const int nslots_here = std::min(runs_on[di], max_conc);
      int local = 0;
      for (int r = di; r < nruns; r += ndev, ++local) {
        if (local % nslots_here != si) continue;
        std::vector<double> x(p);
        if (r == 0) for (int i = 0; i < p; ++i) x[i] = theta0[i];
        else for (int i = 0; i < p; ++i) x[i] = starts[(size_t)(r - 1) * p + i];
        int eval_idx = 0;
        Objective obj = [&](const double* th, double* grad) -> double {
          theta_to_params(th, lo, hi, d, s.hP);
          const int target = (s.best_idx < 0) ? 0 : 1 - s.best_idx;
          double lml;
          int st = prob.run_eval((size_t)di, si, target, !loo, true, &lml, loo ? nullptr : grad);
          if (loo) {
            if (st == HBEGP_OK) st = prob.loo_on_slot((size_t)di, si, &lml, grad);
            else for (int j = 0; j < p; ++j) grad[j] = 0.0;
            if (st != HBEGP_OK && st != HBEGP_NOT_PD) throw std::runtime_error(g_last_error);
          }
          const int my_eval = eval_idx++;
          n_evals.fetch_add(1);
          if (st != HBEGP_OK) n_not_pd.fetch_add(1);
          if (opt.trace_cap > 0) {
            std::lock_guard<std::mutex> lk(trace_mu);
            if (trace_n < opt.trace_cap) {
              const int tI = trace_n++;
              if (opt.trace_theta) memcpy(opt.trace_theta + (size_t)tI * p, th, sizeof(double) * p);
              if (opt.trace_lml) opt.trace_lml[tI] = lml;
              if (opt.trace_grad) memcpy(opt.trace_grad + (size_t)tI * p, grad, sizeof(double) * p);
              if (opt.trace_run) opt.trace_run[tI] = r;
            }
          }
          if (st != HBEGP_OK) return std::numeric_limits<double>::infinity();
          if (s.best_idx < 0 || lml > s.best_lml) {
            s.best_idx = target;
            s.best_lml = lml;
            s.best_run = r;
            s.best_eval = my_eval;
            s.best_theta.assign(th, th + p);
          }
          for (int j = 0; j < p; ++j) grad[j] = -grad[j];
          return -lml;
        };
        LbfgsOptions lo_opt;
        lo_opt.maxeval = opt.maxeval;
        lo_opt.fixed_work = opt.fixed_work != 0;
        if (opt.lbfgs_memory > 0) lo_opt.memory = opt.lbfgs_memory;
        lbfgsb_minimize(obj, x.data(), lnlo.data(), lnhi.data(), p, lo_opt);
      }
    } catch (const HipError& he) {
      hip_fail(he);
      std::lock_guard<std::mutex> lk(err_mu);
      err = g_last_error;
    } catch (const std::exception& e) {
      std::lock_guard<std::mutex> lk(err_mu);
      err = std::string("worker thread: ") + e.what();
    }
  };

  std::vector<std::thread> threads;
  try {
    for (int di = 0; di < ndev; ++di)
      for (int si = 0; si < std::min(runs_on[di], max_conc); ++si) threads.emplace_back(worker, di, si);
  } catch (...) {
    for (auto& t : threads) t.join();
    throw;
  }
  for (auto& t : threads) t.join();
  if (opt.trace_cap > 0 && trace_n > 1 && opt.trace_run) {
    std::vector<int> order(trace_n);
    for (int i = 0; i < trace_n; ++i) order[i] = i;
    std::stable_sort(order.begin(), order.end(), [&](int a, int b) { return opt.trace_run[a] < opt.trace_run[b]; });
    auto permute = [&](auto* arr, int width) {
      if (!arr) return;
      std::vector<typename std::remove_pointer<decltype(arr)>::type> tmp((size_t)trace_n * width);
      for (int i = 0; i < trace_n; ++i) memcpy(&tmp[(size_t)i * width], arr + (size_t)order[i] * width, sizeof(tmp[0]) * width);
      memcpy(arr, tmp.data(), sizeof(tmp[0]) * tmp.size());
    };
    permute(opt.trace_theta, p);
    permute(opt.trace_lml, 1);
    permute(opt.trace_grad, p);
    permute(opt.trace_run, 1);
  }
  if (opt.trace_count) *opt.trace_count = trace_n;
  if (opt.n_evals) *opt.n_evals = n_evals.load();
  if (opt.n_not_pd) *opt.n_not_pd = n_not_pd.load();
  if (!err.empty()) return fail(HBEGP_EHIP, "%s", err.c_str());
  }

  int bdi = -1, bsi = -1;
  for (int di = 0; di < ndev; ++di)
    for (int si = 0; si < (int)prob.slots[di].size(); ++si) {
      const Slot<T>& s = prob.slots[di][si];
      if (s.best_idx < 0) continue;
      bool better = bdi < 0;
      if (!better) {
        const Slot<T>& b = prob.slots[bdi][bsi];
        better = s.best_lml > b.best_lml ||
                 (s.best_lml == b.best_lml && (s.best_run < b.best_run || (s.best_run == b.best_run && s.best_eval < b.best_eval)));
      }
      if (better) { bdi = di; bsi = si; }
    }
  if (bdi < 0) return fail(HBEGP_ALL_FAILED, "every evaluation of the fit failed (kernel matrix not positive definite)");
  Slot<T>& best = prob.slots[bdi][bsi];
  std::vector<double> th(p);
  for (int i = 0; i < p; ++i) {
    double v = std::exp(best.best_theta[i]);
    if (v < lo[i]) v = lo[i];
    if (hi[i] < v) v = hi[i];
    th[i] = std::log(v);
  }
  if (theta_best) memcpy(theta_best, th.data(), sizeof(double) * p);
  if (lml_best) *lml_best = best.best_lml;
  if (loo) {
    prob.release();
    return model_out ? do_extend<T>(ctx, X, y, n, d, nu, th.data(), nullptr, nullptr, model_out) : HBEGP_OK;
  }
  const auto tf2 = std::chrono::steady_clock::now();
  if (host_serial && prob.small_ && !host_lk.owns_lock()) host_lk.lock();
  const auto th1 = std::chrono::steady_clock::now();
  if (model_out) *model_out = make_model<T>(prob, (size_t)bdi, bsi, th.data(), best.best_lml, false, best.best_params.empty() ? nullptr : best.best_params.data());
  if (host_lk.owns_lock()) {
    prob.release();
    held_ms += std::chrono::duration<double, std::milli>(std::chrono::steady_clock::now() - th1).count();
    host_lk.unlock();
    if (timing) fprintf(stderr, "fit: host-side turns held for %.3f ms (set-up + model / release)\n", held_ms);
  }
  if (timing) {
    const auto tf3 = std::chrono::steady_clock::now();
    auto ms = [](std::chrono::steady_clock::time_point a, std::chrono::steady_clock::time_point b) { return std::chrono::duration<double, std::milli>(b - a).count(); };
    fprintf(stderr, "fit: problem %.2f ms, optimiser runs %.2f ms (%d evaluations), model %.2f ms\n", ms(tf0, tf1), ms(tf1, tf2), n_evals.load(), ms(tf2, tf3));
  }
  return HBEGP_OK;
}

template <typename T>
static int do_extend(hbegp_ctx* ctx, const T* X, const T* y, int n, int d, double nu, const double* theta, const double* lo,
                     const double* hi, hbegp_model** model_out) {
  hbegp_ctx one;
  one.devs = {ctx->devs[0]};
  const int dag_env = env_int("HBEGP_DAG", -1);
  const bool queue_like_fit = (dag_env < 0 ? round_up(n, NB) / NB >= env_int("HBEGP_DAG_MIN_BLOCKS", DAG_MIN_BLOCKS_FIT) : dag_env != 0) && round_up(n, NB) / NB >= 2;
  Problem<T> prob(&one, X, y, n, d, nu, 1, !queue_like_fit, true);
  const int p = d + 2;
  Slot<T>& s = prob.slots[0][0];
  theta_to_params(theta, lo, hi, d, s.hP);
  double lml;
  const int st = prob.run_eval(0, 0, 0, false, false, &lml, nullptr);
  if (st != HBEGP_OK) return fail(HBEGP_NOT_PD, "Kernel matrix must be invertible.");
  s.best_idx = 0;
  std::vector<double> th(theta, theta + p);
  if (lo && hi)
    for (int i = 0; i < p; ++i) {
      double v = std::exp(theta[i]);
      if (v < lo[i]) v = lo[i];
      if (hi[i] < v) v = hi[i];
      th[i] = std::log(v);
    }
  if (model_out) *model_out = make_model<T>(prob, 0, 0, th.data(), lml, true);
  return HBEGP_OK;
}

template <typename T>
static int do_extend_from(hbegp_ctx* ctx, hbegp_model* prior, const T* X, const T* y, int n, hbegp_model** model_out,
                          int* incremental) {
  if (incremental) *incremental = 0;
  const int d = prior->d, p = d + 2;
  const double nu = prior->nu2 == 0 ? std::numeric_limits<double>::infinity() : prior->nu2 / 2.0;
  if (prior->dev != ctx->devs[0] || n < prior->n || prior->n < NB || !prior->ldiag)
    return do_extend<T>(ctx, X, y, n, d, nu, prior->theta.data(), nullptr, nullptr, model_out);
  hbegp_ctx one;
  one.devs = {ctx->devs[0]};
  static const int timing = env_int("HBEGP_TIMING", 0);
  auto now = [] { return std::chrono::steady_clock::now(); };
  auto ms = [](std::chrono::steady_clock::time_point a, std::chrono::steady_clock::time_point b) { return std::chrono::duration<double, std::milli>(b - a).count(); };
  const auto t0 = now();
  Problem<T> prob(&one, X, y, n, d, nu, 1, true);
  const auto t1 = now();
  Slot<T>& s = prob.slots[0][0];
  theta_to_params(prior->theta.data(), nullptr, nullptr, d, s.hP);
  int st;
  {
    std::lock_guard<std::mutex> lock(prior->mu);
    st = prob.extend_from(0, 0, static_cast<const T*>(prior->X), static_cast<const T*>(prior->Xinv),
                          static_cast<const T*>(prior->Kinv), static_cast<const T*>(prior->ldiag), prior->n, prior->np);
  }
  if (st == HBEGP_EINVAL) return do_extend<T>(ctx, X, y, n, d, nu, prior->theta.data(), nullptr, nullptr, model_out);
  if (st != HBEGP_OK) return fail(HBEGP_NOT_PD, "Kernel matrix must be invertible.");
  s.best_idx = 0;
  if (incremental) *incremental = 1;
  (void)p;
  const auto t2 = now();
  if (model_out) *model_out = make_model<T>(prob, 0, 0, prior->theta.data(), s.hOut->lml, true);
  const auto t3 = now();
  if (timing) fprintf(stderr, "extend_from: problem %.3f ms, factor %.3f ms, model %.3f ms\n", ms(t0, t1), ms(t1, t2), ms(t2, t3));
  return HBEGP_OK;
}

static int check_args(hbegp_ctx* ctx, const void* X, const void* y, int n, int d, double nu) {
  if (!ctx) return fail(HBEGP_EINVAL, "ctx is NULL");
  if (!X || !y) return fail(HBEGP_EINVAL, "X/y is NULL");
  if (n < 1) return fail(HBEGP_EINVAL, "n must be >= 1 (got %d)", n);
  if (d < 1 || d > MAXD) return fail(HBEGP_EINVAL, "d must be in 1..%d (got %d)", MAXD, d);
  if (!(nu == 0.5 || nu == 1.5 || nu == 2.5 || (std::isinf(nu) && nu > 0)))
    return fail(HBEGP_EINVAL, "Matern kernel with arbitrary values for nu is unimplemented (got %g)", nu);
  return HBEGP_OK;
}

#define GUARD_BEGIN try {
#define GUARD_END                                   \
  }                                                 \
  catch (const HipError& he) { return hip_fail(he); } \
  catch (const std::bad_alloc&) { return fail(HBEGP_ENOMEM, "host allocation failed"); } \
  catch (const std::exception& e) { return fail(HBEGP_EHIP, "internal error: %s", e.what()); } \
  catch (...) { return fail(HBEGP_EHIP, "internal error: unknown exception"); }

extern "C" {

int hbegp_version(void) { return HBEGP_VERSION; }

int hbegp_device_count(void) {
  int cnt = 0;
  if (hipGetDeviceCount(&cnt) != hipSuccess) return 0;
  int ok = 0;
  for (int i = 0; i < cnt; ++i) {
    hipDeviceProp_t prop;
    if (hipGetDeviceProperties(&prop, i) == hipSuccess && strncmp(prop.gcnArchName, "gfx950", 6) == 0) ++ok;
  }
  return ok;
}

const char* hbegp_last_error(void) { return g_last_error.c_str(); }

int hbegp_ctx_create(int n_devices, const int* device_ids, hbegp_ctx** out) {
  if (!out || n_devices < 1) return fail(HBEGP_EINVAL, "n_devices must be >= 1");
  int cnt = 0;
  if (hipGetDeviceCount(&cnt) != hipSuccess || cnt < 1)
    return fail(HBEGP_ENODEV, "no HIP device available: libhbegp has no CPU fallback");
  GUARD_BEGIN
// ... 533 lines not shown
  GUARD_END
}
int hbegp_model_loo_f32(hbegp_model* model, float* mean, float* var, float* lpd, double* loo, double* grad) {
  if (int rc = check_model_loo(model, true, mean || var || lpd || loo || grad)) return rc;
  GUARD_BEGIN
  return model_loo<float>(model, mean, var, lpd, loo, grad);
  GUARD_END
}
int hbegp_debug_loo_phases(int enable, double* phase_ms) {
  if (phase_ms)
    for (int i = 0; i < 4; ++i) phase_ms[i] = t_loo_ms[i];
  t_time_loo = enable != 0;
  return HBEGP_OK;
}
int hbegp_debug_qei_phases(int enable, double* phase_ms) {
  if (phase_ms)
    for (int i = 0; i < 2; ++i) phase_ms[i] = t_qei_ms[i];
  t_time_qei = enable != 0;
  return HBEGP_OK;
}
}

template <typename T>
static int check_select(hbegp_model* model, const T* Xs, int m, int k, double fmin, const double* lie, int* idx) {
  if (m < 0) return fail(HBEGP_EINVAL, "m must be >= 0 (got %d)", m);
  if (k < 0) return fail(HBEGP_EINVAL, "k must be >= 0 (got %d)", k);
  if (k > m) return fail(HBEGP_EINVAL, "k must be <= m (got k = %d, m = %d)", k, m);
  if (k > 0 && !idx) return fail(HBEGP_EINVAL, "idx is NULL");
  if (!std::isfinite(fmin)) return fail(HBEGP_EINVAL, "fmin must be finite (got %g)", fmin);
  if (lie && !std::isfinite(*lie)) return fail(HBEGP_EINVAL, "the lie must be finite (got %g)", *lie);
  return check_posterior<T>(model, Xs, m, 0.0);
}
extern "C" {
int hbegp_select_batch_f64(hbegp_model* model, const double* Xs, int m, int k, double fmin_normalized, const double* lie, int* idx,
                           double* ei, double* mean_out, double* var_out) {
  if (int rc = check_select<double>(model, Xs, m, k, fmin_normalized, lie, idx)) return rc;
  if (k == 0) return HBEGP_OK;
  GUARD_BEGIN
  return model_select_batch<double>(model, Xs, m, k, fmin_normalized, lie, idx, ei, mean_out, var_out);
  GUARD_END
}
int hbegp_select_batch_f32(hbegp_model* model, const float* Xs, int m, int k, double fmin_normalized, const double* lie, int* idx,
                           double* ei, float* mean_out, float* var_out) {
  if (int rc = check_select<float>(model, Xs, m, k, fmin_normalized, lie, idx)) return rc;
  if (k == 0) return HBEGP_OK;
  GUARD_BEGIN
  return model_select_batch<float>(model, Xs, m, k, fmin_normalized, lie, idx, ei, mean_out, var_out);
  GUARD_END
}
int hbegp_debug_batch_select_phases(int enable, double* phase_ms) {
  if (phase_ms)
    for (int i = 0; i < 2; ++i) phase_ms[i] = t_select_ms[i];
  t_time_select = enable != 0;
  return HBEGP_OK;
}
}

template <typename T>
static int check_kg(hbegp_model* model, const T* Xs, int m, int mc, const double* kg) {
  if (m < 0) return fail(HBEGP_EINVAL, "m must be >= 0 (got %d)", m);
  if (mc < 0) return fail(HBEGP_EINVAL, "mc must be >= 0 (got %d)", mc);
  if (mc > m) return fail(HBEGP_EINVAL, "mc must be <= m (got mc = %d, m = %d)", mc, m);
  if (mc > 0 && !kg) return fail(HBEGP_EINVAL, "kg is NULL");
  return check_posterior<T>(model, Xs, m, 0.0);
}
extern "C" {
int hbegp_knowledge_gradient_f64(hbegp_model* model, const double* Xs, int m, int mc, double* kg, int* best, int* imin, double* mean_out,
                                 double* var_out) {
  if (int rc = check_kg<double>(model, Xs, m, mc, kg)) return rc;
  if (best) *best = -1;
  if (imin) *imin = -1;
  if (m == 0) return HBEGP_OK;
  GUARD_BEGIN
  return model_knowledge_gradient<double>(model, Xs, m, mc, kg, best, imin, mean_out, var_out);
  GUARD_END
}
int hbegp_knowledge_gradient_f32(hbegp_model* model, const float* Xs, int m, int mc, double* kg, int* best, int* imin, float* mean_out,
                                 float* var_out) {
  if (int rc = check_kg<float>(model, Xs, m, mc, kg)) return rc;
  if (best) *best = -1;
  if (imin) *imin = -1;
  if (m == 0) return HBEGP_OK;
  GUARD_BEGIN
  return model_knowledge_gradient<float>(model, Xs, m, mc, kg, best, imin, mean_out, var_out);
  GUARD_END
}
int hbegp_debug_kg_phases(int enable, double* phase_ms) {
  if (phase_ms)
    for (int i = 0; i < 2; ++i) phase_ms[i] = t_kg_ms[i];
  t_time_kg = enable != 0;
  return HBEGP_OK;
}
int hbegp_debug_posterior_phases(int enable, double* phase_ms) {
  if (phase_ms)
    for (int i = 0; i < 4; ++i) phase_ms[i] = t_posterior_ms[i];
  t_time_posterior = enable != 0;
  return HBEGP_OK;
}

int hbegp_model_info(const hbegp_model* model, int* n, int* d, int* is_f32, double* nu, double* lml) {
  if (!model) return fail(HBEGP_EINVAL, "NULL model");
  if (n) *n = model->n;
  if (d) *d = model->d;
  if (is_f32) *is_f32 = model->is_f32 ? 1 : 0;
  if (nu) *nu = model->nu2 == 0 ? std::numeric_limits<double>::infinity() : model->nu2 / 2.0;
  if (lml) *lml = model->lml;
  return HBEGP_OK;
}

}
template <typename T>
static int model_get(hbegp_model* m, double* theta, T* alpha, T* kinv) {
  if (!m) return fail(HBEGP_EINVAL, "NULL model");
  if (m->is_f32 != (sizeof(T) == 4)) return fail(HBEGP_EINVAL, "element type mismatch");
  GUARD_BEGIN
  std::lock_guard<std::mutex> lock(m->mu);
  HIPCHECK(hipSetDevice(m->dev));
  if (theta) memcpy(theta, m->theta.data(), sizeof(double) * m->theta.size());
  if (alpha) HIPCHECK(hipMemcpyAsync(alpha, m->alpha, sizeof(T) * m->n, hipMemcpyDeviceToHost, m->stream));
  if (kinv) HIPCHECK(hipMemcpy2DAsync(kinv, sizeof(T) * m->n, m->Kinv, sizeof(T) * m->np, sizeof(T) * m->n, m->n, hipMemcpyDeviceToHost, m->stream));
  HIPCHECK(hipStreamSynchronize(m->stream));
  return HBEGP_OK;
  GUARD_END
}
extern "C" {
int hbegp_model_get_f64(hbegp_model* model, double* theta, double* alpha, double* kinv) {
  return model_get<double>(model, theta, alpha, kinv);
}
int hbegp_model_get_f32(hbegp_model* model, double* theta, float* alpha, float* kinv) {
  return model_get<float>(model, theta, alpha, kinv);
}
int hbegp_model_debug_params(hbegp_model* model, double* out) {
  if (!model) return fail(HBEGP_EINVAL, "NULL model");
  if (!out) return fail(HBEGP_EINVAL, "NULL out");
  GUARD_BEGIN
  std::lock_guard<std::mutex> lock(model->mu);
  HIPCHECK(hipSetDevice(model->dev));
  EvalParams P;
  HIPCHECK(hipMemcpyAsync(&P, model->dP, sizeof(P), hipMemcpyDeviceToHost, model->stream));
  HIPCHECK(hipStreamSynchronize(model->stream));
  out[0] = P.noise;
  out[1] = P.amp;
  for (int k = 0; k < model->d; ++k) out[2 + k] = P.ell[k];
  return HBEGP_OK;
  GUARD_END
}
void hbegp_model_retain(hbegp_model* model) {
  if (model) model->refs.fetch_add(1);
}
void hbegp_model_release(hbegp_model* model) {
  if (model && model->refs.fetch_sub(1) == 1) delete model;
}

int hbegp_debug_lbfgs_replay(int n, const double* x0, const double* lo, const double* hi, int maxeval, int memory, int fixed_work,
                             int count, const double* f, const double* g, double* requested, int* n_requested) {
  if (n < 1 || n > LBFGS_MAXN || count < 0 || !x0 || !lo || !hi || !requested || !n_requested || (count > 0 && (!f || !g)))
    return fail(HBEGP_EINVAL, "bad argument");
  GUARD_BEGIN
  LbfgsOptions o;
  std::unique_ptr<LbfgsState> st(new LbfgsState);
  lbfgs_begin(*st, x0, lo, hi, n, maxeval, memory > 0 ? memory : o.memory, o.pgtol, o.ftol, fixed_work != 0);
  int produced = 0;
  memcpy(requested, lbfgs_request(*st), sizeof(double) * n);
  produced = 1;
  for (int i = 0; i < count; ++i) {
    if (!lbfgs_advance(*st, f[i], g + (size_t)i * n)) break;
    if (i + 1 < count) {
      memcpy(requested + (size_t)(i + 1) * n, lbfgs_request(*st), sizeof(double) * n);
      produced = i + 2;
    }
  }
  *n_requested = produced;
  return HBEGP_OK;
  GUARD_END
}

int hbegp_debug_dag_plan(int nblocks, int bk, int small_h, int nwg, int fine, int* ntasks, int* ncounters, int* nleaf,
                         double* gflop, double* crit_us, double* sim_us, char* err, int errlen) {
  if (nblocks < 1 || (bk != 16 && bk != 32) || small_h < 0 || nwg < 0) return fail(HBEGP_EINVAL, "bad argument");
  GUARD_BEGIN
  DagBuilder builder(bk, small_h, nwg, (fine & 1) != 0);
  builder.set_rl_progressive((fine & 16) != 0);
  builder.set_big128(getenv("HBEGP_DAG_BIG128") && atoi(getenv("HBEGP_DAG_BIG128")) != 0, getenv("HBEGP_DAG_BIG128") && atoi(getenv("HBEGP_DAG_BIG128")) >= 2);
  if (fine & 2) return fail(HBEGP_EINVAL, "fine bit 1 (kernel-matrix / reduction tasks in the queue) no longer exists");
  DagPlan plan = builder.build(0, nblocks, (fine & 4) != 0, (fine & 8) != 0);
  if (const char* fault = getenv("HBEGP_DAG_TEST_FAULT")) {
    int a = 0, b = 0;
    if (sscanf(fault, "drop:%d", &a) == 1 && a >= 0 && a < (int)plan.tasks.size() && plan.tasks[a].nwait > 0) {
      DagTask& t = plan.tasks[a];
      for (int w = 1; w < t.nwait; ++w) { t.wcnt[w - 1] = t.wcnt[w]; t.wval[w - 1] = t.wval[w]; }
      t.nwait--;
    } else if (sscanf(fault, "move:%d:%d", &a, &b) == 2 && a >= 0 && b >= 0 && a < (int)plan.tasks.size() && b < (int)plan.tasks.size()) {
      const DagTask t = plan.tasks[a];
      plan.tasks.erase(plan.tasks.begin() + a);
      plan.tasks.insert(plan.tasks.begin() + b, t);
    }
  }
  const std::string why = plan.tasks.empty() ? std::string("too many counters") : dag_plan_validate(plan, nblocks);
  if (ntasks) *ntasks = (int)plan.tasks.size();
  if (ncounters) *ncounters = (int)plan.totals.size();
  if (nleaf) *nleaf = plan.n_leaf;
  if (gflop) *gflop = plan.gflop;
  if (crit_us) *crit_us = plan.crit_us;
  if (sim_us) *sim_us = plan.sim_us;
  if (err && errlen > 0) snprintf(err, (size_t)errlen, "%s", why.c_str());
  return why.empty() ? HBEGP_OK : fail(HBEGP_EINVAL, "%s", why.c_str());
  GUARD_END
}

double hbegp_minimize_by_gradient(hbegp_objective_fn f, void* user, double* x, const double* lo, const double* hi, int n,
                                  int maxeval) {
  if (!f || !x || !lo || !hi || n < 1) {
    fail(HBEGP_EINVAL, "hbegp_minimize_by_gradient: NULL argument or n < 1");
    return std::numeric_limits<double>::quiet_NaN();
  }
  try {
    LbfgsOptions opt;
    opt.maxeval = maxeval > 0 ? maxeval : 150;
    Objective obj = [&](const double* xx, double* g) { return f(xx, g, user); };
    return lbfgsb_minimize(obj, x, lo, hi, n, opt).f;
  } catch (const std::exception& e) {
    fail(HBEGP_EHIP, "hbegp_minimize_by_gradient: %s", e.what());
  } catch (...) {
    fail(HBEGP_EHIP, "hbegp_minimize_by_gradient: unknown exception");
  }
  return std::numeric_limits<double>::quiet_NaN();
}

}
```

csrc/lbfgs_step.hpp:

```cpp
#pragma once
#include <cmath>
#if !defined(__HIP_DEVICE_COMPILE__)
#include <vector>
#endif

#if defined(__HIPCC__)
#define LBFGS_HD __host__ __device__
#else
#define LBFGS_HD
#endif

namespace hbegp {

constexpr int LBFGS_MAXN = 66;
constexpr int LBFGS_MAXM = 10;

struct LbfgsState {
  int n, maxeval, m;
  double pgtol, ftol;
  int fixed_work;
  double lo[LBFGS_MAXN], hi[LBFGS_MAXN];
  int phase;
  int nevals, iterations, converged;
  int hcount;
  double f, step, gs;
  double x[LBFGS_MAXN], g[LBFGS_MAXN], xn[LBFGS_MAXN], d[LBFGS_MAXN];
  double S[LBFGS_MAXM][LBFGS_MAXN], Y[LBFGS_MAXM][LBFGS_MAXN], rho[LBFGS_MAXM];
};

template <class St>
struct LbfgsWork {
  static constexpr int N = LBFGS_MAXN;
  LBFGS_HD static double* get(St&, double* stack, int) { return stack; }
};

namespace lbfgs_detail {
LBFGS_HD inline double dmin(double a, double b) { return a < b ? a : b; }
LBFGS_HD inline double dmax(double a, double b) { return a > b ? a : b; }
LBFGS_HD inline bool finite(double v) { return v - v == 0.0; }

template <class St>
LBFGS_HD inline bool propose(St& s) {
  const int n = s.n;
  double gs = 0, moved = 0;
  for (int i = 0; i < n; ++i) {
    double v = s.x[i] + s.step * s.d[i];
    v = dmin(dmax(v, s.lo[i]), s.hi[i]);
    s.xn[i] = v;
    gs += s.g[i] * (v - s.x[i]);
    moved = dmax(moved, fabs(v - s.x[i]));
  }
  s.gs = gs;
  return moved != 0.0;
}

template <class St>
LBFGS_HD inline int begin_iteration(St& s) {
  const int n = s.n;
  for (;;) {
    if (s.nevals >= s.maxeval) return 2;
    double pg_stack[LbfgsWork<St>::N], q_stack[LbfgsWork<St>::N], a[LBFGS_MAXM];
    double* pg = LbfgsWork<St>::get(s, pg_stack, 0);
    double* q = LbfgsWork<St>::get(s, q_stack, 1);
    double pgnorm = 0;
    for (int i = 0; i < n; ++i) {
      const bool at_lo = s.x[i] <= s.lo[i] && s.g[i] > 0, at_hi = s.x[i] >= s.hi[i] && s.g[i] < 0;
      pg[i] = (at_lo || at_hi) ? 0.0 : s.g[i];
      pgnorm = dmax(pgnorm, fabs(pg[i]));
    }
    if (pgnorm <= s.pgtol * dmax(1.0, fabs(s.f))) {
      s.converged = 1;
      return 2;
    }
    for (int i = 0; i < n; ++i) q[i] = pg[i];
    const int hcount = s.hcount;
    for (int h = hcount - 1; h >= 0; --h) {
      double sq = 0;
      for (int i = 0; i < n; ++i) sq += s.S[h][i] * q[i];
      a[h] = s.rho[h] * sq;
      for (int i = 0; i < n; ++i) q[i] -= a[h] * s.Y[h][i];
    }
    double gamma = 1.0;
    if (hcount > 0) {
      double sy = 0, yy = 0;
      for (int i = 0; i < n; ++i) {
        sy += s.S[hcount - 1][i] * s.Y[hcount - 1][i];
        yy += s.Y[hcount - 1][i] * s.Y[hcount - 1][i];
      }
      if (yy > 0) gamma = sy / yy;
    }
    for (int i = 0; i < n; ++i) q[i] *= gamma;
    for (int h = 0; h < hcount; ++h) {
      double yq = 0;
      for (int i = 0; i < n; ++i) yq += s.Y[h][i] * q[i];
      const double b = s.rho[h] * yq;
      for (int i = 0; i < n; ++i) q[i] += s.S[h][i] * (a[h] - b);
    }
    double dg = 0;
    for (int i = 0; i < n; ++i) {
      s.d[i] = (pg[i] == 0.0) ? 0.0 : -q[i];
      dg += s.d[i] * s.g[i];
    }
    if (!(dg < 0)) {
      s.hcount = 0;
      dg = 0;
      for (int i = 0; i < n; ++i) {
        s.d[i] = -pg[i];
        dg += s.d[i] * s.g[i];
      }
    }
    s.step = 1.0;
    if (s.hcount == 0) {
      double dn = 0;
      for (int i = 0; i < n; ++i) dn += s.d[i] * s.d[i];
      s.step = dmin(1.0, 1.0 / sqrt(dmax(dn, 1e-300)));
    }
    if (propose(s)) return 1;
    if (s.hcount > 0) {
      s.hcount = 0;
      continue;
    }
    return 2;
  }
}
}

template <class St>
LBFGS_HD inline void lbfgs_begin(St& s, const double* x0, const double* lo, const double* hi, int n, int maxeval, int memory,
                                 double pgtol, double ftol, bool fixed_work) {
  s.n = n;
  s.maxeval = maxeval;
  s.m = memory < 1 ? 1 : (memory > LBFGS_MAXM ? LBFGS_MAXM : memory);
  s.pgtol = pgtol;
  s.ftol = ftol;
  s.fixed_work = fixed_work ? 1 : 0;
  s.phase = 0;
  s.nevals = s.iterations = s.converged = s.hcount = 0;
  s.f = INFINITY;
  s.step = 1.0;
  s.gs = 0;
  for (int i = 0; i < n; ++i) {
    s.lo[i] = lo[i];
    s.hi[i] = hi[i];
    s.x[i] = lbfgs_detail::dmin(lbfgs_detail::dmax(x0[i], lo[i]), hi[i]);
  }
}

template <class St>
LBFGS_HD inline const double* lbfgs_request(const St& s) { return s.phase == 1 ? s.xn : s.x; }

template <class St>
LBFGS_HD inline bool lbfgs_advance(St& s, double fe, const double* ge) {
  using namespace lbfgs_detail;
  const int n = s.n;
  ++s.nevals;
  if (fe != fe) fe = INFINITY;
  int next = 2;
  if (s.phase == 0) {
    s.f = fe;
    for (int i = 0; i < n; ++i) s.g[i] = ge[i];
    next = finite(fe) ? begin_iteration(s) : 2;
  } else if (s.phase == 1) {
    const double fn = fe;
    if (finite(fn) && fn <= s.f + 1e-4 * s.gs) {
      ++s.iterations;
      double sv_stack[LbfgsWork<St>::N], yv_stack[LbfgsWork<St>::N];
      double* sv = LbfgsWork<St>::get(s, sv_stack, 2);
      double* yv = LbfgsWork<St>::get(s, yv_stack, 3);
      double sy = 0, ss = 0, yy = 0;
      for (int i = 0; i < n; ++i) {
        sv[i] = s.xn[i] - s.x[i];
        yv[i] = ge[i] - s.g[i];
        sy += sv[i] * yv[i];
        ss += sv[i] * sv[i];
        yy += yv[i] * yv[i];
      }
      if (sy > 1e-10 * sqrt(ss * yy) && sy > 0) {
        if (s.hcount == s.m) {
          for (int h = 1; h < s.hcount; ++h) {
            for (int i = 0; i < n; ++i) {
              s.S[h - 1][i] = s.S[h][i];
              s.Y[h - 1][i] = s.Y[h][i];
            }
            s.rho[h - 1] = s.rho[h];
          }
          --s.hcount;
        }
        for (int i = 0; i < n; ++i) {
          s.S[s.hcount][i] = sv[i];
          s.Y[s.hcount][i] = yv[i];
        }
        s.rho[s.hcount] = 1.0 / sy;
        ++s.hcount;
      }
      const double fold = s.f;
      for (int i = 0; i < n; ++i) {
        s.x[i] = s.xn[i];
        s.g[i] = ge[i];
      }
      s.f = fn;
      if (fold - s.f <= s.ftol * dmax(1.0, fabs(s.f))) {
        s.converged = 1;
        next = 2;
      } else {
        next = begin_iteration(s);
      }
    } else {
      double nstep = 0.5 * s.step;
      if (finite(fn) && s.gs < 0) {
        const double denom = 2.0 * (fn - s.f - s.gs);
        if (denom > 0) nstep = dmin(dmax(-s.gs * s.step / denom, 0.1 * s.step), 0.5 * s.step);
      }
      s.step = nstep;
      bool again = !(s.step < 1e-20) && s.nevals < s.maxeval && propose(s);
      if (again) {
        next = 1;
      } else if (s.hcount > 0) {
        s.hcount = 0;
        next = s.nevals < s.maxeval ? begin_iteration(s) : 2;
      } else {
        next = 2;
      }
    }
  } else {
    next = 2;
  }
  if (next == 1) {
    s.phase = 1;
    return true;
  }
  if (s.fixed_work && s.nevals < s.maxeval) {
    s.phase = 2;
    return true;
  }
  s.phase = 3;
  return false;
}

#if !defined(__HIP_DEVICE_COMPILE__)
struct LbfgsStateHost {
  int n, maxeval, m;
  double pgtol, ftol;
  int fixed_work;
  double *lo, *hi;
  int phase;
  int nevals, iterations, converged;
  int hcount;
  double f, step, gs;
  double *x, *g, *xn, *d;
  double* S[LBFGS_MAXM];
  double* Y[LBFGS_MAXM];
  double rho[LBFGS_MAXM];
  double* work[4];
  explicit LbfgsStateHost(int nvars) : buf_((size_t)(10 + 2 * LBFGS_MAXM) * (nvars < 1 ? 1 : nvars), 0.0) {
    const size_t w = (size_t)(nvars < 1 ? 1 : nvars);
    double* p = buf_.data();
    auto take = [&]() { double* r = p; p += w; return r; };
    lo = take(); hi = take(); x = take(); g = take(); xn = take(); d = take();
    for (auto& v : work) v = take();
    for (int h = 0; h < LBFGS_MAXM; ++h) { S[h] = take(); Y[h] = take(); }
  }
  LbfgsStateHost(const LbfgsStateHost&) = delete;
  LbfgsStateHost& operator=(const LbfgsStateHost&) = delete;

 private:
  std::vector<double> buf_;
};
template <>
struct LbfgsWork<LbfgsStateHost> {
  static constexpr int N = 1;
  static double* get(LbfgsStateHost& s, double*, int which) { return s.work[which]; }
};
#endif

}
```

hbetune_rs_amd/_lib.py:

```python
import ctypes as C
import os

import numpy as np

HERE = os.path.dirname(os.path.abspath(__file__))
LIB_PATH = os.environ.get("HBEGP_LIB") or os.path.join(HERE, "libhbegp.so")

OK, NOT_PD, ALL_FAILED = 0, 1, 2
EINVAL, EHIP, ENODEV, ENOMEM = -1, -2, -3, -4
PATHS_MAX_FEATURES, PATHS_MAX_PATHS = 16384, 1024


class HbegpError(RuntimeError):
    def __init__(self, code, msg):
        super().__init__(f"hbegp error {code}: {msg}")
        self.code = code


class FitOptions(C.Structure):

    _fields_ = [
        ("struct_size", C.c_size_t),
        ("maxeval", C.c_int),
        ("fixed_work", C.c_int),
        ("lbfgs_memory", C.c_int),
        ("trace_cap", C.c_int),
        ("trace_theta", C.POINTER(C.c_double)),
        ("trace_lml", C.POINTER(C.c_double)),
        ("trace_grad", C.POINTER(C.c_double)),
        ("trace_run", C.POINTER(C.c_int)),
        ("trace_count", C.POINTER(C.c_int)),
        ("n_evals", C.POINTER(C.c_int)),
        ("n_not_pd", C.POINTER(C.c_int)),
    ]

    def __init__(self, *a, **k):
        super().__init__(*a, **k)
        self.struct_size = C.sizeof(FitOptions)


OBJECTIVE_FN = C.CFUNCTYPE(C.c_double, C.POINTER(C.c_double), C.POINTER(C.c_double), C.c_void_p)

_dp = C.POINTER(C.c_double)
_fp = C.POINTER(C.c_float)
_ip = C.POINTER(C.c_int)
_vp = C.c_void_p

SIGNATURES = {
    "hbegp_version": (C.c_int, []),
    "hbegp_device_count": (C.c_int, []),
    "hbegp_ctx_create": (C.c_int, [C.c_int, _ip, C.POINTER(_vp)]),
    "hbegp_ctx_destroy": (None, [_vp]),
    "hbegp_last_error": (C.c_char_p, []),
    "hbegp_problem_create_f64": (C.c_int, [_vp, _dp, _dp, C.c_int, C.c_int, C.c_double, C.c_int, C.POINTER(_vp)]),
    "hbegp_problem_create_f32": (C.c_int, [_vp, _fp, _fp, C.c_int, C.c_int, C.c_double, C.c_int, C.POINTER(_vp)]),
    "hbegp_problem_destroy": (None, [_vp]),
    "hbegp_problem_eval": (C.c_int, [_vp, C.c_int, C.c_int, _dp, _dp, _dp, _dp, _dp]),
    "hbegp_problem_get_f64": (C.c_int, [_vp, C.c_int, C.c_int, _dp, _dp, _dp]),
    "hbegp_problem_get_f32": (C.c_int, [_vp, C.c_int, C.c_int, _fp, _fp, _fp]),
    "hbegp_problem_debug_get_f64": (C.c_int, [_vp, C.c_int, C.c_int, C.c_int, _dp]),
    "hbegp_problem_debug_get_f32": (C.c_int, [_vp, C.c_int, C.c_int, C.c_int, _fp]),
    "hbegp_problem_kmat_f64": (C.c_int, [_vp, C.c_int, C.c_int, _dp, _dp, _dp, _dp]),
    "hbegp_problem_kmat_f32": (C.c_int, [_vp, C.c_int, C.c_int, _dp, _dp, _dp, _fp]),
    "hbegp_problem_time_eval": (C.c_int, [_vp, C.c_int, C.c_int, _dp, C.c_int, _dp]),
    "hbegp_problem_time_concurrent": (C.c_int, [_vp, C.c_int, _dp, C.c_int, _dp]),
    "hbegp_fit_f64": (C.c_int, [_vp, _dp, _dp, C.c_int, C.c_int, C.c_double, _dp, _dp, _dp, _dp, C.c_int,
                                C.POINTER(FitOptions), _dp, _dp, C.POINTER(_vp)]),
    "hbegp_fit_f32": (C.c_int, [_vp, _fp, _fp, C.c_int, C.c_int, C.c_double, _dp, _dp, _dp, _dp, C.c_int,
                                C.POINTER(FitOptions), _dp, _dp, C.POINTER(_vp)]),
    "hbegp_extend_f64": (C.c_int, [_vp, _dp, _dp, C.c_int, C.c_int, C.c_double, _dp, _dp, _dp, C.POINTER(_vp)]),
    "hbegp_extend_f32": (C.c_int, [_vp, _fp, _fp, C.c_int, C.c_int, C.c_double, _dp, _dp, _dp, C.POINTER(_vp)]),
    "hbegp_extend_from_f64": (C.c_int, [_vp, _vp, _dp, _dp, C.c_int, C.POINTER(_vp), _ip]),
    "hbegp_extend_from_f32": (C.c_int, [_vp, _vp, _fp, _fp, C.c_int, C.POINTER(_vp), _ip]),
    "hbegp_predict_f64": (C.c_int, [_vp, _dp, C.c_int, _dp, _dp, _ip]),
    "hbegp_predict_f32": (C.c_int, [_vp, _fp, C.c_int, _fp, _fp, _ip]),
    "hbegp_predict_grad_f64": (C.c_int, [_vp, _dp, C.c_int, _dp, _dp, _dp, _dp, _ip]),
    "hbegp_predict_grad_f32": (C.c_int, [_vp, _fp, C.c_int, _fp, _fp, _fp, _fp, _ip]),
    "hbegp_maximize_ei_f64": (C.c_int, [_vp, _dp, C.c_int, _dp, _dp, C.c_double, C.c_int, _dp, _dp, _ip]),
    "hbegp_maximize_ei_f32": (C.c_int, [_vp, _fp, C.c_int, _dp, _dp, C.c_double, C.c_int, _fp, _dp, _ip]),
    "hbegp_predict_cov_f64": (C.c_int, [_vp, _dp, C.c_int, C.c_double, _dp, _dp]),
    "hbegp_predict_cov_f32": (C.c_int, [_vp, _fp, C.c_int, C.c_double, _fp, _fp]),
    "hbegp_sample_posterior_f64": (C.c_int, [_vp, _dp, C.c_int, _dp, C.c_int, C.c_double, _dp, _ip, _ip]),
    "hbegp_sample_posterior_f32": (C.c_int, [_vp, _fp, C.c_int, _fp, C.c_int, C.c_double, _fp, _ip, _ip]),
    "hbegp_select_batch_f64": (C.c_int, [_vp, _dp, C.c_int, C.c_int, C.c_double, _dp, _ip, _dp, _dp, _dp]),
    "hbegp_select_batch_f32": (C.c_int, [_vp, _fp, C.c_int, C.c_int, C.c_double, _dp, _ip, _dp, _fp, _fp]),
    "hbegp_knowledge_gradient_f64": (C.c_int, [_vp, _dp, C.c_int, C.c_int, _dp, _ip, _ip, _dp, _dp]),
    "hbegp_knowledge_gradient_f32": (C.c_int, [_vp, _fp, C.c_int, C.c_int, _dp, _ip, _ip, _fp, _fp]),
    "hbegp_qei_f64": (C.c_int, [_vp, _dp, C.c_int, C.c_int, _dp, C.c_int, C.c_double, C.c_double, _dp, _dp, _ip]),
    "hbegp_qei_f32": (C.c_int, [_vp, _fp, C.c_int, C.c_int, _fp, C.c_int, C.c_double, C.c_double, _dp, _fp, _ip]),
    "hbegp_maximize_qei_f64": (C.c_int, [_vp, _dp, C.c_int, C.c_int, _dp, _dp, _dp, C.c_int, C.c_double, C.c_double, C.c_int, _dp,
                                         _dp, _ip]),
    "hbegp_maximize_qei_f32": (C.c_int, [_vp, _fp, C.c_int, C.c_int, _dp, _dp, _fp, C.c_int, C.c_double, C.c_double, C.c_int, _fp,
                                         _dp, _ip]),
    "hbegp_debug_qei_phases": (C.c_int, [C.c_int, _dp]),
    "hbegp_problem_eval_loo": (C.c_int, [_vp, C.c_int, C.c_int, _dp, _dp, _dp, _dp, _dp]),
    "hbegp_fit_loo_f64": (C.c_int, [_vp, _dp, _dp, C.c_int, C.c_int, C.c_double, _dp, _dp, _dp, _dp, C.c_int,
                                    C.POINTER(FitOptions), _dp, _dp, C.POINTER(_vp)]),
    "hbegp_fit_loo_f32": (C.c_int, [_vp, _fp, _fp, C.c_int, C.c_int, C.c_double, _dp, _dp, _dp, _dp, C.c_int,
                                    C.POINTER(FitOptions), _dp, _dp, C.POINTER(_vp)]),
    "hbegp_model_loo_f64": (C.c_int, [_vp, _dp, _dp, _dp, _dp, _dp]),
    "hbegp_model_loo_f32": (C.c_int, [_vp, _fp, _fp, _fp, _dp, _dp]),
    "hbegp_debug_loo_phases": (C.c_int, [C.c_int, _dp]),
    "hbegp_paths_create_f64": (C.c_int, [_vp, _dp, _dp, _dp, _dp, C.c_int, C.c_int, C.POINTER(_vp)]),
    "hbegp_paths_create_f32": (C.c_int, [_vp, _fp, _fp, _fp, _fp, C.c_int, C.c_int, C.POINTER(_vp)]),
    "hbegp_paths_eval_f64": (C.c_int, [_vp, _dp, C.c_int, C.c_int, _dp, _dp]),
    "hbegp_paths_eval_f32": (C.c_int, [_vp, _fp, C.c_int, C.c_int, _fp, _fp]),
    "hbegp_paths_minimize_f64": (C.c_int, [_vp, _dp, C.c_int, _dp, _dp, C.c_int, _dp, _dp, _ip]),
    "hbegp_paths_minimize_f32": (C.c_int, [_vp, _fp, C.c_int, _dp, _dp, C.c_int, _fp, _dp, _ip]),
    "hbegp_paths_info": (C.c_int, [_vp, _ip, _ip, _ip, _ip, _ip]),
    "hbegp_paths_release": (None, [_vp]),
    "hbegp_debug_paths_phases": (C.c_int, [C.c_int, _dp]),
    "hbegp_debug_posterior_phases": (C.c_int, [C.c_int, _dp]),
    "hbegp_debug_batch_select_phases": (C.c_int, [C.c_int, _dp]),
    "hbegp_debug_kg_phases": (C.c_int, [C.c_int, _dp]),
    "hbegp_model_info": (C.c_int, [_vp, _ip, _ip, _ip, _dp, _dp]),
    "hbegp_model_get_f64": (C.c_int, [_vp, _dp, _dp, _dp]),
    "hbegp_model_get_f32": (C.c_int, [_vp, _dp, _fp, _fp]),
    "hbegp_model_debug_params": (C.c_int, [_vp, _dp]),
    "hbegp_model_retain": (None, [_vp]),
    "hbegp_model_release": (None, [_vp]),
    "hbegp_debug_lbfgs_replay": (C.c_int, [C.c_int, _dp, _dp, _dp, C.c_int, C.c_int, C.c_int, C.c_int, _dp, _dp, _dp, _ip]),
    "hbegp_debug_dag_plan": (C.c_int, [C.c_int, C.c_int, C.c_int, C.c_int, C.c_int, _ip, _ip, _ip, _dp, _dp, _dp, C.c_char_p,
                                       C.c_int]),
    "hbegp_minimize_by_gradient": (C.c_double, [OBJECTIVE_FN, _vp, _dp, _dp, _dp, C.c_int, C.c_int]),
}

_lib = None


def load():
    global _lib
    if _lib is not None:
        return _lib
    if not os.path.exists(LIB_PATH):
        raise ImportError(
            f"{LIB_PATH} is missing: build it with `python -c 'import __graft_entry__ as g; g.build()'` or `make`. "
            "hbetune_rs_amd has no CPU fallback."
        )
    try:
        import torch
    except Exception:
        pass
    lib = C.CDLL(LIB_PATH, mode=C.RTLD_GLOBAL)
    for name, (res, args) in SIGNATURES.items():
        fn = getattr(lib, name)
        fn.restype = res
        fn.argtypes = args
    _lib = lib
    return lib


def last_error():
    return load().hbegp_last_error().decode("utf-8", "replace")


def check(code, allow=()):
    if code != OK and code not in allow:
        raise HbegpError(code, last_error())
    return code


def dptr(a):
    return None if a is None else a.ctypes.data_as(_dp)


def fptr(a):
    return None if a is None else a.ctypes.data_as(_fp)


def aptr(a):
    if a is None:
        return None
    return fptr(a) if a.dtype == np.float32 else dptr(a)


def as_c(a, dtype):
    return np.ascontiguousarray(a, dtype=dtype)
```

hbetune_rs_amd/gpr.py:

```python
import ctypes as C
import math

import numpy as np

from . import _lib
from ._lib import HbegpError, NOT_PD, ALL_FAILED


def _suffix(dtype):
    dt = np.dtype(dtype)
    if dt == np.float64:
        return "f64"
    if dt == np.float32:
        return "f32"
    raise TypeError(f"element type must be float64 or float32, got {dt}")


class Context:

    def __init__(self, n_devices=1, device_ids=None):
        lib = _lib.load()
        self._h = C.c_void_p()
        ids = None
        if device_ids is not None:
# ... 53 lines not shown
    def __del__(self):
        try:
            self.close()
        except Exception:
            pass

    def lml_with_gradient(self, theta, lo=None, hi=None, want_grad=True, dev=0, slot=0):
        lib = _lib.load()
        theta = _lib.as_c(theta, np.float64)
        lo = None if lo is None else _lib.as_c(lo, np.float64)
        hi = None if hi is None else _lib.as_c(hi, np.float64)
        lml = C.c_double()
        grad = np.zeros(self.p) if want_grad else None
        code = lib.hbegp_problem_eval(self._h, dev, slot, _lib.dptr(theta), _lib.dptr(lo), _lib.dptr(hi), C.byref(lml), _lib.dptr(grad))
        if _lib.check(code, allow=(NOT_PD,)) == NOT_PD:
            return None
        return lml.value, grad

    def loo_with_gradient(self, theta, lo=None, hi=None, want_grad=True, dev=0, slot=0):
        lib = _lib.load()
        theta = _lib.as_c(theta, np.float64)
        lo = None if lo is None else _lib.as_c(lo, np.float64)
        hi = None if hi is None else _lib.as_c(hi, np.float64)
        loo = C.c_double()
        grad = np.zeros(self.p) if want_grad else None
        code = lib.hbegp_problem_eval_loo(self._h, dev, slot, _lib.dptr(theta), _lib.dptr(lo), _lib.dptr(hi), C.byref(loo), _lib.dptr(grad))
        if _lib.check(code, allow=(NOT_PD,)) == NOT_PD:
            return None
        return loo.value, grad

    def results(self, want_kinv=True, dev=0, slot=0):
        lib = _lib.load()
        alpha = np.zeros(self.n, dtype=self.dtype)
        ldiag = np.zeros(self.n, dtype=self.dtype)
        kinv = np.zeros((self.n, self.n), dtype=self.dtype) if want_kinv else None
        get = getattr(lib, f"hbegp_problem_get_{self._sfx}")
        _lib.check(get(self._h, dev, slot, _lib.aptr(alpha), _lib.aptr(kinv), _lib.aptr(ldiag)))
        return alpha, kinv, ldiag

    def debug_work_matrix(self, which, dev=0, slot=0):
        npad = (self.n + 127) // 128 * 128
        out = np.zeros((npad, npad), dtype=self.dtype)
        get = getattr(_lib.load(), f"hbegp_problem_debug_get_{self._sfx}")
        _lib.check(get(self._h, dev, slot, which, _lib.aptr(out)))
        return out

    def kernel_matrix(self, theta, lo=None, hi=None, dev=0, slot=0):
        lib = _lib.load()
        theta = _lib.as_c(theta, np.float64)
        lo = None if lo is None else _lib.as_c(lo, np.float64)
        hi = None if hi is None else _lib.as_c(hi, np.float64)
        K = np.zeros((self.n, self.n), dtype=self.dtype)
        kmat = getattr(lib, f"hbegp_problem_kmat_{self._sfx}")
        _lib.check(kmat(self._h, dev, slot, _lib.dptr(theta), _lib.dptr(lo), _lib.dptr(hi), _lib.aptr(K)))
        return K

    def time_eval(self, theta, reps=5, dev=0, slot=0):
        lib = _lib.load()
        theta = _lib.as_c(theta, np.float64)
        phases = np.zeros(24)
        _lib.check(lib.hbegp_problem_time_eval(self._h, dev, slot, _lib.dptr(theta), reps, _lib.dptr(phases)))
        keys = ["kmat_ms", "chol_gemm_ms", "leaf_ms", "lauum_ms", "alpha_ms", "gradtrace_ms", "eval_graph_ms", "n_gemm",
                "gemm128_ms", "gemm128_gflop", "gemm64_ms", "gemm64_gflop", "gemm32_ms", "gemm32_gflop", "eval_eager_ms", "n_leaf",
                "n_gemm128", "n_gemm64", "n_gemm32", "dag_ms", "dag_gflop", "r1", "r2", "r3"]
        return dict(zip(keys, phases.tolist()))

    def time_concurrent(self, theta, reps=5, dev=0):
        lib = _lib.load()
        theta = _lib.as_c(theta, np.float64)
        out = np.zeros(16)
        _lib.check(lib.hbegp_problem_time_concurrent(self._h, dev, _lib.dptr(theta), reps, _lib.dptr(out)))
        keys = ["round_ms", "n_slots", "round_eager_ms", "kmat_ms", "factor_ms", "factor_gflop", "lauum_ms", "lauum_gflop", "alpha_ms",
                "gradtrace_ms", "task_queue_workgroups", "factor_launches"]
        return dict(zip(keys, out.tolist()))


class FittedKernel:

    def __init__(self, handle, dtype, n, d, nu):
        self._h = handle
        self.dtype = np.dtype(dtype)
        self.n, self.d, self.nu = n, d, nu
        self.x_train = self.y_train = None
        self._sfx = _suffix(dtype)
        lml = C.c_double()
        _lib.check(_lib.load().hbegp_model_info(self._h, None, None, None, None, C.byref(lml)))
        self.lml = lml.value
        self.theta = np.zeros(d + 2)
        get = getattr(_lib.load(), f"hbegp_model_get_{self._sfx}")
        _lib.check(get(self._h, _lib.dptr(self.theta), None, None))

    @property
    def noise(self):
        return math.exp(self.theta[0])

    @property
    def amplitude(self):
        return math.exp(self.theta[1])

    @property
    def length_scale(self):
        return np.exp(self.theta[2:])

    def device_params(self):
        out = np.zeros(self.d + 2)
        _lib.check(_lib.load().hbegp_model_debug_params(self._h, _lib.dptr(out)))
        return float(out[0]), float(out[1]), out[2:].copy()

    def arrays(self, want_kinv=True):
        alpha = np.zeros(self.n, dtype=self.dtype)
        kinv = np.zeros((self.n, self.n), dtype=self.dtype) if want_kinv else None
        get = getattr(_lib.load(), f"hbegp_model_get_{self._sfx}")
        _lib.check(get(self._h, None, _lib.aptr(alpha), _lib.aptr(kinv)))
        return alpha, kinv

    @staticmethod
    def new(x_train, y_train, theta0, lo, hi, starts=None, nu=2.5, ctx=None, maxeval=150, fixed_work=False, trace=False):
        return FittedKernel._fit("hbegp_fit", x_train, y_train, theta0, lo, hi, starts, nu, ctx, maxeval, fixed_work, trace)

    @staticmethod
    def new_by_loo(x_train, y_train, theta0, lo, hi, starts=None, nu=2.5, ctx=None, maxeval=150, fixed_work=False, trace=False):
        return FittedKernel._fit("hbegp_fit_loo", x_train, y_train, theta0, lo, hi, starts, nu, ctx, maxeval, fixed_work, trace)

    @staticmethod
    def _fit(symbol, x_train, y_train, theta0, lo, hi, starts, nu, ctx, maxeval, fixed_work, trace):
        lib = _lib.load()
        ctx = ctx or default_context()
        dtype = np.dtype(x_train.dtype)
        sfx = _suffix(dtype)
        x = _lib.as_c(x_train, dtype)
        y = _lib.as_c(y_train, dtype)
        n, d = x.shape
        p = d + 2
        theta0 = _lib.as_c(theta0, np.float64)
        lo = _lib.as_c(lo, np.float64)
        hi = _lib.as_c(hi, np.float64)
        assert theta0.shape == (p,) and lo.shape == (p,) and hi.shape == (p,)
        n_restarts = 0 if starts is None else len(starts)
        starts_c = None if n_restarts == 0 else _lib.as_c(np.asarray(starts).reshape(n_restarts, p), np.float64)
        opt = _lib.FitOptions()
        opt.maxeval = maxeval
        opt.fixed_work = 1 if fixed_work else 0
        n_evals, n_not_pd = C.c_int(0), C.c_int(0)
        opt.n_evals = C.pointer(n_evals)
        opt.n_not_pd = C.pointer(n_not_pd)
        tr = None
        if trace:
            cap = (1 + n_restarts) * maxeval
            tr = dict(theta=np.zeros((cap, p)), lml=np.zeros(cap), grad=np.zeros((cap, p)), run=np.zeros(cap, dtype=np.int32),
                      count=C.c_int(0))
            opt.trace_cap = cap
            opt.trace_theta = _lib.dptr(tr["theta"])
            opt.trace_lml = _lib.dptr(tr["lml"])
            opt.trace_grad = _lib.dptr(tr["grad"])
            opt.trace_run = tr["run"].ctypes.data_as(C.POINTER(C.c_int))
            opt.trace_count = C.pointer(tr["count"])
        handle = C.c_void_p()
        theta_best = np.zeros(p)
        lml_best = C.c_double()
        fit = getattr(lib, f"{symbol}_{sfx}")
        _lib.check(fit(ctx._h, _lib.aptr(x), _lib.aptr(y), n, d, float(nu), _lib.dptr(theta0), _lib.dptr(lo), _lib.dptr(hi),
                       _lib.dptr(starts_c), n_restarts, C.byref(opt), _lib.dptr(theta_best), C.byref(lml_best), C.byref(handle)))
        fk = FittedKernel(handle, dtype, n, d, nu)
        fk.x_train, fk.y_train = x, y
        fk.n_evals, fk.n_not_pd = n_evals.value, n_not_pd.value
        fk.theta_best = theta_best
        if symbol == "hbegp_fit_loo":
            fk.loo_best = lml_best.value
        if trace:
            k = tr["count"].value
            fk.trace = dict(theta=tr["theta"][:k], lml=tr["lml"][:k], grad=tr["grad"][:k], run=tr["run"][:k])
        return fk

    @staticmethod
    def extend(x_train, y_train, theta, lo=None, hi=None, nu=2.5, ctx=None):
        lib = _lib.load()
        ctx = ctx or default_context()
        dtype = np.dtype(x_train.dtype)
        sfx = _suffix(dtype)
        x = _lib.as_c(x_train, dtype)
        y = _lib.as_c(y_train, dtype)
        n, d = x.shape
        theta = _lib.as_c(theta, np.float64)
        lo = None if lo is None else _lib.as_c(lo, np.float64)
        hi = None if hi is None else _lib.as_c(hi, np.float64)
        handle = C.c_void_p()
        ext = getattr(lib, f"hbegp_extend_{sfx}")
        _lib.check(ext(ctx._h, _lib.aptr(x), _lib.aptr(y), n, d, float(nu), _lib.dptr(theta), _lib.dptr(lo), _lib.dptr(hi),
                       C.byref(handle)))
        fk = FittedKernel(handle, dtype, n, d, nu)
        fk.x_train, fk.y_train = x, y
        return fk

    def extend_with(self, x_train, y_train, ctx=None):
        lib = _lib.load()
        ctx = ctx or default_context()
        x = _lib.as_c(x_train, self.dtype)
        y = _lib.as_c(y_train, self.dtype)
        n, d = x.shape
        assert d == self.d
        handle = C.c_void_p()
        inc = C.c_int(0)
        ext = getattr(lib, f"hbegp_extend_from_{self._sfx}")
        _lib.check(ext(ctx._h, self._h, _lib.aptr(x), _lib.aptr(y), n, C.byref(handle), C.byref(inc)))
        fk = FittedKernel(handle, self.dtype, n, d, self.nu)
        fk.x_train, fk.y_train = x, y
        fk.incremental = bool(inc.value)
        return fk

    def loo(self, want_grad=False):
        mean = np.zeros(self.n, dtype=self.dtype)
        var = np.zeros(self.n, dtype=self.dtype)
        lpd = np.zeros(self.n, dtype=self.dtype)
        loo = C.c_double()
        grad = np.zeros(self.d + 2) if want_grad else None
        fn = getattr(_lib.load(), f"hbegp_model_loo_{self._sfx}")
        _lib.check(fn(self._h, _lib.aptr(mean), _lib.aptr(var), _lib.aptr(lpd), C.byref(loo), _lib.dptr(grad)))
        return (mean, var, lpd, loo.value, grad) if want_grad else (mean, var, lpd, loo.value)

    def predict(self, x, want_variance=True):
        lib = _lib.load()
        x = _lib.as_c(x, self.dtype)
        assert x.ndim == 2 and x.shape[1] == self.d
        m = x.shape[0]
        mean = np.zeros(m, dtype=self.dtype)
        var = np.zeros(m, dtype=self.dtype) if want_variance else None
        n_warn = C.c_int(0)
        pred = getattr(lib, f"hbegp_predict_{self._sfx}")
        _lib.check(pred(self._h, _lib.aptr(x), m, _lib.aptr(mean), _lib.aptr(var), C.byref(n_warn)))
        return mean, var, n_warn.value

    def predict_with_gradient(self, x, want_variance=True):
        lib = _lib.load()
        x = _lib.as_c(x, self.dtype)
        assert x.ndim == 2 and x.shape[1] == self.d
        m = x.shape[0]
        mean = np.zeros(m, dtype=self.dtype)
        dmean = np.zeros((m, self.d), dtype=self.dtype)
        var = np.zeros(m, dtype=self.dtype) if want_variance else None
        dvar = np.zeros((m, self.d), dtype=self.dtype) if want_variance else None
        n_warn = C.c_int(0)
        fn = getattr(lib, f"hbegp_predict_grad_{self._sfx}")
        _lib.check(fn(self._h, _lib.aptr(x), m, _lib.aptr(mean), _lib.aptr(var), _lib.aptr(dmean), _lib.aptr(dvar), C.byref(n_warn)))
        return mean, var, dmean, dvar, n_warn.value

    def maximize_ei(self, starts, lo, hi, fmin_normalized, maxeval=150):
        lib = _lib.load()
        starts = _lib.as_c(np.atleast_2d(starts), self.dtype)
        assert starts.shape[1] == self.d
        S = starts.shape[0]
        lo = _lib.as_c(lo, np.float64)
        hi = _lib.as_c(hi, np.float64)
        assert lo.shape == (self.d,) and hi.shape == (self.d,)
        x = np.zeros((S, self.d), dtype=self.dtype)
        ei = np.zeros(S)
        nevals = np.zeros(S, dtype=np.int32)
        fn = getattr(lib, f"hbegp_maximize_ei_{self._sfx}")
        _lib.check(fn(self._h, _lib.aptr(starts), S, _lib.dptr(lo), _lib.dptr(hi), float(fmin_normalized), int(maxeval), _lib.aptr(x),
                      _lib.dptr(ei), nevals.ctypes.data_as(C.POINTER(C.c_int))))
        return x, ei, nevals

    def predict_cov(self, x, jitter=0.0):
        lib = _lib.load()
        x = _lib.as_c(np.atleast_2d(x), self.dtype)
        assert x.ndim == 2 and x.shape[1] == self.d
        m = x.shape[0]
        mean = np.zeros(m, dtype=self.dtype)
        cov = np.zeros((m, m), dtype=self.dtype)
        fn = getattr(lib, f"hbegp_predict_cov_{self._sfx}")
        _lib.check(fn(self._h, _lib.aptr(x), m, float(jitter), _lib.aptr(mean), _lib.aptr(cov)))
        return mean, cov

    def sample_posterior(self, x, z, jitter=0.0, want_samples=True):
        lib = _lib.load()
        x = _lib.as_c(np.atleast_2d(x), self.dtype)
        assert x.ndim == 2 and x.shape[1] == self.d
        m = x.shape[0]
        z = _lib.as_c(np.atleast_2d(z), self.dtype)
        assert z.ndim == 2 and z.shape[1] == m, (z.shape, m)
        S = z.shape[0]
        samples = np.zeros((S, m), dtype=self.dtype) if want_samples else None
        argmin = np.zeros(S, dtype=np.int32)
        fn = getattr(lib, f"hbegp_sample_posterior_{self._sfx}")
        _lib.check(fn(self._h, _lib.aptr(x), m, _lib.aptr(z), S, float(jitter), _lib.aptr(samples),
                      argmin.ctypes.data_as(C.POINTER(C.c_int)), None))
        return samples, argmin

    def select_batch(self, x, k, fmin_normalized, lie=None):
        lib = _lib.load()
        x = _lib.as_c(np.atleast_2d(x), self.dtype)
        assert x.ndim == 2 and x.shape[1] == self.d
        m, k = x.shape[0], int(k)
        idx = np.zeros(k, dtype=np.int32)
        ei = np.zeros(k)
        mean = np.zeros(m, dtype=self.dtype)
        var = np.zeros(m, dtype=self.dtype)
        lie_c = None if lie is None else C.byref(C.c_double(float(lie)))
        fn = getattr(lib, f"hbegp_select_batch_{self._sfx}")
        _lib.check(fn(self._h, _lib.aptr(x), m, k, float(fmin_normalized), lie_c, idx.ctypes.data_as(C.POINTER(C.c_int)), _lib.dptr(ei),
                      _lib.aptr(mean), _lib.aptr(var)))
        return idx.astype(np.int64), ei, mean, var

    def knowledge_gradient(self, x, n_candidates=None, want_posterior=False):
        lib = _lib.load()
        x = _lib.as_c(np.atleast_2d(x), self.dtype)
        assert x.ndim == 2 and x.shape[1] == self.d
        m = x.shape[0]
        mc = m if n_candidates is None else int(n_candidates)
        kg = np.zeros(max(mc, 0))
        best, imin = C.c_int(-1), C.c_int(-1)
        mean = np.zeros(m, dtype=self.dtype) if want_posterior else None
        var = np.zeros(m, dtype=self.dtype) if want_posterior else None
        fn = getattr(lib, f"hbegp_knowledge_gradient_{self._sfx}")
        _lib.check(fn(self._h, _lib.aptr(x), m, mc, _lib.dptr(kg), C.byref(best), C.byref(imin), _lib.aptr(mean), _lib.aptr(var)))
        if want_posterior:
            return kg, best.value, imin.value, mean, var
        return kg, best.value, imin.value

    def qei(self, x, z, fmin_normalized, jitter=0.0, want_grad=True, raise_not_pd=False):
        lib = _lib.load()
        x = _lib.as_c(x, self.dtype)
        if x.ndim == 2:
            x = x[None]
        assert x.ndim == 3 and x.shape[2] == self.d, x.shape
# ... 142 lines not shown
```

include/hbegp.h:

```cpp
#ifndef HBEGP_H
#define HBEGP_H

#include <stddef.h>

#ifdef __cplusplus
extern "C" {
#endif

#define HBEGP_VERSION 200

enum {
  HBEGP_OK = 0,
  HBEGP_NOT_PD = 1,
  HBEGP_ALL_FAILED = 2,
  HBEGP_EINVAL = -1,
  HBEGP_EHIP = -2,
  HBEGP_ENODEV = -3,
  HBEGP_ENOMEM = -4
};

typedef struct hbegp_ctx hbegp_ctx;
typedef struct hbegp_problem hbegp_problem;
typedef struct hbegp_model hbegp_model;

int hbegp_version(void);
int hbegp_device_count(void);
int hbegp_ctx_create(int n_devices, const int* device_ids, hbegp_ctx** out);
void hbegp_ctx_destroy(hbegp_ctx* ctx);
const char* hbegp_last_error(void);

int hbegp_problem_create_f64(hbegp_ctx* ctx, const double* X, const double* y, int n, int d, double nu,
                             int n_slots, hbegp_problem** out);
int hbegp_problem_create_f32(hbegp_ctx* ctx, const float* X, const float* y, int n, int d, double nu,
                             int n_slots, hbegp_problem** out);
void hbegp_problem_destroy(hbegp_problem* prob);

int hbegp_problem_eval(hbegp_problem* prob, int dev, int slot, const double* theta, const double* lo,
                       const double* hi, double* lml, double* grad);

int hbegp_problem_eval_loo(hbegp_problem* prob, int dev, int slot, const double* theta, const double* lo, const double* hi,
                           double* loo, double* grad);

int hbegp_problem_get_f64(hbegp_problem* prob, int dev, int slot, double* alpha, double* kinv, double* ldiag);
int hbegp_problem_get_f32(hbegp_problem* prob, int dev, int slot, float* alpha, float* kinv, float* ldiag);

int hbegp_problem_kmat_f64(hbegp_problem* prob, int dev, int slot, const double* theta, const double* lo,
                           const double* hi, double* K);
int hbegp_problem_kmat_f32(hbegp_problem* prob, int dev, int slot, const double* theta, const double* lo,
                           const double* hi, float* K);

int hbegp_problem_time_eval(hbegp_problem* prob, int dev, int slot, const double* theta, int reps,
                            double* phase_ms);

int hbegp_problem_time_concurrent(hbegp_problem* prob, int dev, const double* theta, int reps, double* out);

typedef struct hbegp_fit_options {
  size_t struct_size;
  int maxeval;
  int fixed_work;
  int lbfgs_memory;
  int trace_cap;
  double* trace_theta;
  double* trace_lml;
  double* trace_grad;
  int* trace_run;
  int* trace_count;
  int* n_evals;
  int* n_not_pd;
} hbegp_fit_options;
#define HBEGP_FIT_OPTIONS_INIT { sizeof(hbegp_fit_options) }

int hbegp_fit_f64(hbegp_ctx* ctx, const double* X, const double* y, int n, int d, double nu, const double* theta0,
                  const double* lo, const double* hi, const double* starts, int n_restarts,
                  const hbegp_fit_options* opt, double* theta_best, double* lml_best, hbegp_model** model);
int hbegp_fit_f32(hbegp_ctx* ctx, const float* X, const float* y, int n, int d, double nu, const double* theta0,
                  const double* lo, const double* hi, const double* starts, int n_restarts,
                  const hbegp_fit_options* opt, double* theta_best, double* lml_best, hbegp_model** model);

int hbegp_fit_loo_f64(hbegp_ctx* ctx, const double* X, const double* y, int n, int d, double nu, const double* theta0,
                      const double* lo, const double* hi, const double* starts, int n_restarts,
                      const hbegp_fit_options* opt, double* theta_best, double* loo_best, hbegp_model** model);
int hbegp_fit_loo_f32(hbegp_ctx* ctx, const float* X, const float* y, int n, int d, double nu, const double* theta0,
                      const double* lo, const double* hi, const double* starts, int n_restarts,
                      const hbegp_fit_options* opt, double* theta_best, double* loo_best, hbegp_model** model);

int hbegp_extend_f64(hbegp_ctx* ctx, const double* X, const double* y, int n, int d, double nu, const double* theta,
                     const double* lo, const double* hi, hbegp_model** model);
int hbegp_extend_f32(hbegp_ctx* ctx, const float* X, const float* y, int n, int d, double nu, const double* theta,
                     const double* lo, const double* hi, hbegp_model** model);

int hbegp_extend_from_f64(hbegp_ctx* ctx, hbegp_model* prior, const double* X, const double* y, int n, hbegp_model** model,
                          int* incremental);
int hbegp_extend_from_f32(hbegp_ctx* ctx, hbegp_model* prior, const float* X, const float* y, int n, hbegp_model** model,
                          int* incremental);

int hbegp_predict_f64(hbegp_model* model, const double* Xs, int m, double* mean, double* var, int* n_warn);
int hbegp_predict_f32(hbegp_model* model, const float* Xs, int m, float* mean, float* var, int* n_warn);

int hbegp_predict_grad_f64(hbegp_model* model, const double* Xs, int m, double* mean, double* var, double* dmean, double* dvar,
                           int* n_warn);
int hbegp_predict_grad_f32(hbegp_model* model, const float* Xs, int m, float* mean, float* var, float* dmean, float* dvar,
                           int* n_warn);

int hbegp_maximize_ei_f64(hbegp_model* model, const double* starts, int S, const double* lo, const double* hi, double fmin_normalized,
                          int maxeval, double* x_out, double* ei_out, int* nevals_out);
int hbegp_maximize_ei_f32(hbegp_model* model, const float* starts, int S, const double* lo, const double* hi, double fmin_normalized,
                          int maxeval, float* x_out, double* ei_out, int* nevals_out);

int hbegp_predict_cov_f64(hbegp_model* model, const double* Xs, int m, double jitter, double* mean, double* cov);
int hbegp_predict_cov_f32(hbegp_model* model, const float* Xs, int m, double jitter, float* mean, float* cov);

int hbegp_sample_posterior_f64(hbegp_model* model, const double* Xs, int m, const double* z, int S, double jitter,
                               double* samples, int* argmin, int* info);
int hbegp_sample_posterior_f32(hbegp_model* model, const float* Xs, int m, const float* z, int S, double jitter,
                               float* samples, int* argmin, int* info);

int hbegp_select_batch_f64(hbegp_model* model, const double* Xs, int m, int k, double fmin_normalized, const double* lie, int* idx,
                           double* ei, double* mean_out, double* var_out);
int hbegp_select_batch_f32(hbegp_model* model, const float* Xs, int m, int k, double fmin_normalized, const double* lie, int* idx,
                           double* ei, float* mean_out, float* var_out);

int hbegp_knowledge_gradient_f64(hbegp_model* model, const double* Xs, int m, int mc, double* kg, int* best, int* imin,
                                 double* mean_out, double* var_out);
int hbegp_knowledge_gradient_f32(hbegp_model* model, const float* Xs, int m, int mc, double* kg, int* best, int* imin,
                                 float* mean_out, float* var_out);

int hbegp_qei_f64(hbegp_model* model, const double* Xb, int B, int q, const double* z, int S, double fmin_normalized, double jitter,
                  double* qei, double* grad, int* info);
int hbegp_qei_f32(hbegp_model* model, const float* Xb, int B, int q, const float* z, int S, double fmin_normalized, double jitter,
                  double* qei, float* grad, int* info);

int hbegp_maximize_qei_f64(hbegp_model* model, const double* starts, int R, int q, const double* lo, const double* hi, const double* z,
                           int S, double fmin_normalized, double jitter, int maxeval, double* x_out, double* qei_out, int* nevals_out);
int hbegp_maximize_qei_f32(hbegp_model* model, const float* starts, int R, int q, const double* lo, const double* hi, const float* z,
                           int S, double fmin_normalized, double jitter, int maxeval, float* x_out, double* qei_out, int* nevals_out);

int hbegp_model_loo_f64(hbegp_model* model, double* mean, double* var, double* lpd, double* loo, double* grad);
int hbegp_model_loo_f32(hbegp_model* model, float* mean, float* var, float* lpd, double* loo, double* grad);

int hbegp_model_info(const hbegp_model* model, int* n, int* d, int* is_f32, double* nu, double* lml);
int hbegp_model_get_f64(hbegp_model* model, double* theta, double* alpha, double* kinv);
int hbegp_model_get_f32(hbegp_model* model, double* theta, float* alpha, float* kinv);
void hbegp_model_retain(hbegp_model* model);
void hbegp_model_release(hbegp_model* model);

typedef double (*hbegp_objective_fn)(const double* x, double* grad, void* user);
double hbegp_minimize_by_gradient(hbegp_objective_fn f, void* user, double* x, const double* lo, const double* hi,
                                  int n, int maxeval);

int hbegp_problem_debug_get_f64(hbegp_problem* prob, int dev, int slot, int which, double* out);
int hbegp_problem_debug_get_f32(hbegp_problem* prob, int dev, int slot, int which, float* out);

int hbegp_model_debug_params(hbegp_model* model, double* out);

int hbegp_debug_dag_plan(int nblocks, int bk, int small_h, int nwg, int fine, int* ntasks, int* ncounters, int* nleaf,
                         double* gflop, double* crit_us, double* sim_us, char* err, int errlen);

int hbegp_debug_lbfgs_replay(int n, const double* x0, const double* lo, const double* hi, int maxeval, int memory, int fixed_work,
                             int count, const double* f, const double* g, double* requested, int* n_requested);

int hbegp_debug_posterior_phases(int enable, double* phase_ms);
int hbegp_debug_batch_select_phases(int enable, double* phase_ms);
int hbegp_debug_kg_phases(int enable, double* phase_ms);
int hbegp_debug_qei_phases(int enable, double* phase_ms);

int hbegp_debug_loo_phases(int enable, double* phase_ms);

#define HBEGP_PATHS_MAX_FEATURES 16384
#define HBEGP_PATHS_MAX_PATHS 1024
typedef struct hbegp_paths hbegp_paths;
int hbegp_paths_create_f64(hbegp_model* model, const double* omega0, const double* phase, const double* w, const double* eps, int F, int S,
                           hbegp_paths** paths);
int hbegp_paths_create_f32(hbegp_model* model, const float* omega0, const float* phase, const float* w, const float* eps, int F, int S,
                           hbegp_paths** paths);
int hbegp_paths_eval_f64(hbegp_paths* paths, const double* Xs, int m, int per_path, double* f, double* df);
int hbegp_paths_eval_f32(hbegp_paths* paths, const float* Xs, int m, int per_path, float* f, float* df);
int hbegp_paths_minimize_f64(hbegp_paths* paths, const double* starts, int R, const double* lo, const double* hi, int maxeval,
                             double* x_best, double* f_best, int* n_evals);
int hbegp_paths_minimize_f32(hbegp_paths* paths, const float* starts, int R, const double* lo, const double* hi, int maxeval,
                             float* x_best, double* f_best, int* n_evals);
int hbegp_paths_info(const hbegp_paths* paths, int* n, int* d, int* n_features, int* n_paths, int* is_f32);
void hbegp_paths_release(hbegp_paths* paths);
int hbegp_debug_paths_phases(int enable, double* phase_ms);

#ifdef __cplusplus
}
#endif
#endif
```

Measured before the change: 1.774 fit+predict/s.

## Evaluate L-BFGS trial points lazily: compute LML first, gradient only if accepted

Splits each likelihood evaluation into two phases: the Cholesky/LML phase without the K^-1 (LAUUM) tasks, and a separate K^-1 plus gradient phase that runs only when the line-search trial point is accepted. A K^-1-only task queue is derived from the full DAG plan with remapped counters, and a second control region is added for it. The goal is to skip K^-1 and gradient work for rejected trial points. In exchange it adds a second queue launch, with its own sync and launch overhead, for accepted points. It also needs the optimizer's accept decision to be exact so the fixed-work trajectory stays the same.

```diff
diff --git a/csrc/dag_plan.hpp b/csrc/dag_plan.hpp
--- a/csrc/dag_plan.hpp
+++ b/csrc/dag_plan.hpp
@@ -620,6 +620,42 @@
   void set_big128(bool on, bool with_acc = false) { big128_ = on; big128_acc_ = on && with_acc; }
 };
 
+inline DagPlan dag_plan_kinv_only(const DagPlan& full) {
+  DagPlan out;
+  const int nc = (int)full.totals.size();
+  std::vector<int> kept_bumps(nc, 0), remap(nc, -1);
+  for (const DagTask& t : full.tasks)
+    if (t.flags & DAGF_CKINV)
+      for (int q = 0; q < DAG_MAXSIG; ++q)
+        if (t.sig[q] != DAG_NOSIG) kept_bumps[t.sig[q]]++;
+  for (int c = 0; c < nc; ++c) {
+    if (kept_bumps[c] == 0) continue;
+    if (kept_bumps[c] != full.totals[c]) return DagPlan();
+    remap[c] = (int)out.totals.size();
+    out.totals.push_back(kept_bumps[c]);
+  }
+  for (const DagTask& src : full.tasks) {
+    if (!(src.flags & DAGF_CKINV)) continue;
+    DagTask t = src;
+    for (int q = 0; q < DAG_MAXSIG; ++q)
+      if (t.sig[q] != DAG_NOSIG) t.sig[q] = (uint16_t)remap[t.sig[q]];
+    t.nwait = 0;
+    for (int w = 0; w < DAG_MAXWAIT; ++w) t.wcnt[w] = t.wval[w] = 0;
+    for (int w = 0; w < src.nwait; ++w) {
+      if (remap[src.wcnt[w]] < 0) continue;
+      t.wcnt[t.nwait] = (uint16_t)remap[src.wcnt[w]];
+      t.wval[t.nwait] = src.wval[w];
+      ++t.nwait;
+    }
+    out.tasks.push_back(t);
+  }
+  out.gflop = out.gflop_lauum = full.gflop_lauum;
+  out.n_lauum = (int)out.tasks.size();
+  out.sim_us = full.sim_us;
+  out.crit_us = full.crit_us;
+  return out;
+}
+
 inline std::string dag_plan_validate(const DagPlan& plan, int nblocks_total) {
   const int nc = (int)plan.totals.size(), nt = (int)plan.tasks.size();
   const int words = (nc + 63) / 64;
diff --git a/csrc/hbegp.cpp b/csrc/hbegp.cpp
--- a/csrc/hbegp.cpp
+++ b/csrc/hbegp.cpp
@@ -588,7 +588,7 @@
   size_t small_slab_bytes = 0;
   void* host_slab = nullptr;
   size_t host_slab_bytes = 0;
-  hipGraphExec_t graph[DAG_MAX_VARIANTS + 1 + DAG_CROWD_LEVELS][2][2] = {};
+  hipGraphExec_t graph[DAG_MAX_VARIANTS + 1 + DAG_CROWD_LEVELS][2][4] = {};
   int best_idx = -1;
   double best_lml = -std::numeric_limits<double>::infinity();
   int best_run = 0, best_eval = 0;
@@ -596,10 +596,11 @@
   std::vector<double> best_params;
   int last_target = 0;
   int dag_variant = 1;
+  int dag_part = 0;
   unsigned long long seq = 0;
   bool ctrl_cleared = false;
   bool published = false;
-  long long expect_ns = 0;
+  long long expect_ns[4] = {0, 0, 0, 0};
 };
 
 struct ProblemBase {
@@ -629,6 +630,9 @@
     int nwg = 0;
     std::vector<DagTask*> tasks;
     std::vector<DagTask> host_tasks;
+    int nwg_p1 = 0, ntasks_p1 = 0, nwg_kinv = 0, ntasks_kinv = 0;
+    std::vector<DagTask*> tasks_p1, tasks_kinv;
+    std::vector<DagTask> host_tasks_p1, host_tasks_kinv;
   };
   std::vector<DagVariant> dag_var;
   std::unique_ptr<std::atomic<int>[]> busy_slots_;
@@ -636,10 +640,13 @@
   int dag_nvar_ = 1, dag_ncrowd_ = 0;
   unsigned long long dag_wait_ticks_ = 200000000ull;
   size_t dag_ctrl_bytes = 0;
+  int dag_ctrl_regions_ = 1;
   double dag_gflop = 0;
   bool adhoc_ = false;
   bool small_ = false;
   bool like_fit_ = false;
+  bool lazy_ = false;
+  std::function<std::shared_ptr<const DagPlan>(int, bool)> plan_for_;
   bool hostio_ = true;
   bool eval_published() const { return hostio_ && !small_; }
   int leaf_dbg_ = 0;
@@ -655,10 +662,12 @@
     return static_cast<U*>(q);
   }
 
-  Problem(hbegp_ctx* c, const T* X, const T* y, int n_, int d_, double nu, int n_slots_, bool single_shot = false, bool like_fit = false) {
+  Problem(hbegp_ctx* c, const T* X, const T* y, int n_, int d_, double nu, int n_slots_, bool single_shot = false, bool like_fit = false,
+          bool lazy_fit = false) {
     try {
       adhoc_ = single_shot;
       like_fit_ = like_fit;
+      lazy_ = lazy_fit && env_int("HBEGP_LAZY_GRAD", 1) != 0;
       init(c, X, y, n_, d_, nu, n_slots_);
     } catch (...) {
       release();
@@ -673,6 +682,7 @@
     leaf_dbg_ = env_int("HBEGP_LEAF_DBG", 0) & 16;
     small_ = np == NB && d <= SMALL_EVAL_MAXD && env_int("HBEGP_SMALL", 1) != 0;
     hostio_ = env_int("HBEGP_HOSTIO", 1) != 0;
+    lazy_ = lazy_ && eval_published() && !adhoc_;
     const size_t nn = (size_t)np * np;
     Xd.assign(c->devs.size(), nullptr);
     yd.assign(c->devs.size(), nullptr);
@@ -747,8 +757,8 @@
       dag_rl_ = env_int("HBEGP_DAG_RL", np / NB <= 80 ? 1 : 0) != 0;
       static std::mutex cache_mu;
       static std::map<DagPlanKey, std::shared_ptr<const DagPlan>> cache;
-      auto plan_for = [&](int nwg) {
-        const DagPlanKey key = {np / NB, dag_stage_depth(is_f32), env_int("HBEGP_DAG_SMALLH", dag_rl_ ? 4 : 8), nwg, dag_lauum_, dag_rl_,
+      plan_for_ = [this](int nwg, bool lauum) {
+        const DagPlanKey key = {np / NB, dag_stage_depth(is_f32), env_int("HBEGP_DAG_SMALLH", dag_rl_ ? 4 : 8), nwg, lauum, dag_rl_,
                                 env_int("HBEGP_DAG_RL_GROUP", 32), env_int("HBEGP_DAG_RL_NEAR", 1),
                                 env_int("HBEGP_DAG_LAUUM_SPLIT", n_slots <= 1 ? 1 : 0),
                                 env_int("HBEGP_DAG_CHAIN32", 1),
@@ -765,15 +775,16 @@
           builder.set_rl(key.rl_group, key.rl_near, key.lauum_split != 0, key.chain32 != 0);
           builder.set_rl_progressive(key.prog != 0);
           builder.set_big128(key.big128 != 0, key.big128 >= 2);
-          cached = std::make_shared<const DagPlan>(builder.build(0, np / NB, dag_lauum_, dag_rl_));
+          cached = std::make_shared<const DagPlan>(builder.build(0, np / NB, lauum, dag_rl_));
           std::lock_guard<std::mutex> lk(cache_mu);
-          if (cache.size() > 64) cache.clear();
+          if (cache.size() > 256) cache.clear();
           cache[key] = cached;
         }
         return cached;
       };
       const int nvar = std::min(n_slots, DAG_MAX_VARIANTS);
       dag_nwg = share_of(n_slots);
+      auto plan_for = [this](int nwg) { return plan_for_(nwg, dag_lauum_); };
       std::shared_ptr<const DagPlan> cached = plan_for(dag_nwg);
       if (cached->tasks.empty() && dag_rl_) {
         dag_rl_ = false;
@@ -791,6 +802,7 @@
         dag_gflop = plan.gflop;
         dag_gflop_lauum = plan.gflop_lauum;
         dag_ctrl_bytes = (sizeof(int) * (DAG_CTRL_WORDS + plan.totals.size()) + 15) / 16 * 16;
+        dag_ctrl_regions_ = (lazy_ && dag_lauum_) ? 2 : 1;
         dag_wait_ticks_ = (unsigned long long)(std::max(2.0, 200.0 * plan.sim_us * 1e-6 * std::max(1, n_slots)) * 1e8);
         busy_slots_.reset(new std::atomic<int>[c->devs.size()]);
         for (size_t di = 0; di < c->devs.size(); ++di) busy_slots_[di].store(0);
@@ -816,6 +828,35 @@
             var.tasks[di] = palloc<DagTask>(c->devs[di], pv->tasks.size());
             HIPCHECK(hipMemcpyAsync(var.tasks[di], var.host_tasks.data(), sizeof(DagTask) * var.host_tasks.size(), hipMemcpyHostToDevice, slots[di][0].stream));
           }
+          if (lazy_ && dag_lauum_) {
+            const int wg_p1 = lazy_wg(var.nwg, 1), wg_kinv = lazy_wg(var.nwg, 2);
+            const std::shared_ptr<const DagPlan> p1 = plan_for_(wg_p1, false);
+            const DagPlan kv = dag_plan_kinv_only(*pv);
+            if (p1->tasks.empty() || kv.tasks.empty() || p1->totals.size() > plan.totals.size() || kv.totals.size() > plan.totals.size()) {
+              throw std::runtime_error("task queues of a two-phase evaluation could not be derived from the plan");
+            } else {
+              if (env_int("HBEGP_DAG_VALIDATE", 0)) {
+                std::string why = dag_plan_validate(*p1, np / NB);
+                if (why.empty()) why = dag_plan_validate(kv, np / NB);
+                if (!why.empty()) throw std::runtime_error("task queue of a two-phase evaluation is unsound: " + why);
+              }
+              var.host_tasks_p1 = p1->tasks;
+              var.host_tasks_kinv = kv.tasks;
+              var.ntasks_p1 = (int)p1->tasks.size();
+              var.ntasks_kinv = (int)kv.tasks.size();
+              var.nwg_p1 = std::min(wg_p1, var.ntasks_p1);
+              var.nwg_kinv = std::min(wg_kinv, var.ntasks_kinv);
+              var.tasks_p1.assign(c->devs.size(), nullptr);
+              var.tasks_kinv.assign(c->devs.size(), nullptr);
+              for (size_t di = 0; di < c->devs.size(); ++di) {
+                HIPCHECK(hipSetDevice(c->devs[di]));
+                var.tasks_p1[di] = palloc<DagTask>(c->devs[di], var.host_tasks_p1.size());
+                var.tasks_kinv[di] = palloc<DagTask>(c->devs[di], var.host_tasks_kinv.size());
+                HIPCHECK(hipMemcpyAsync(var.tasks_p1[di], var.host_tasks_p1.data(), sizeof(DagTask) * var.host_tasks_p1.size(), hipMemcpyHostToDevice, slots[di][0].stream));
+                HIPCHECK(hipMemcpyAsync(var.tasks_kinv[di], var.host_tasks_kinv.data(), sizeof(DagTask) * var.host_tasks_kinv.size(), hipMemcpyHostToDevice, slots[di][0].stream));
+              }
+            }
+          }
         }
         for (size_t di = 0; di < c->devs.size(); ++di) {
           HIPCHECK(hipSetDevice(c->devs[di]));
@@ -824,8 +865,8 @@
               bool f3 = false;
               s.W3 = static_cast<T*>(g_pool.get(s.dev, sizeof(T) * nn, &f3));
             }
-            s.dag_ctrl = palloc<int>(s.dev, dag_ctrl_bytes / sizeof(int));
-            HIPCHECK(hipMemsetAsync(s.dag_ctrl, 0, dag_ctrl_bytes, slots[di][0].stream));
+            s.dag_ctrl = palloc<int>(s.dev, dag_ctrl_regions_ * dag_ctrl_bytes / sizeof(int));
+            HIPCHECK(hipMemsetAsync(s.dag_ctrl, 0, dag_ctrl_regions_ * dag_ctrl_bytes, slots[di][0].stream));
             if (getenv("HBEGP_DAG_TRACE")) {
               s.dag_trace = palloc<unsigned long long>(s.dev, 5 * plan.tasks.size());
               HIPCHECK(hipMemsetAsync(s.dag_trace, 0, sizeof(unsigned long long) * 5 * plan.tasks.size(), slots[di][0].stream));
@@ -868,7 +909,7 @@
         if (s.stream) (void)hipStreamSynchronize(s.stream);
         for (int v = 0; v <= DAG_MAX_VARIANTS + DAG_CROWD_LEVELS; ++v)
           for (int a = 0; a < 2; ++a)
-            for (int b = 0; b < 2; ++b)
+            for (int b = 0; b < 4; ++b)
               if (s.graph[v][a][b]) (void)hipGraphExecDestroy(s.graph[v][a][b]);
         const size_t nnb = sizeof(T) * (size_t)np * np;
         g_pool.put(s.dev, s.W1, nnb); g_pool.put(s.dev, s.W2, nnb); g_pool.put(s.dev, s.W3, nnb);
@@ -887,8 +928,8 @@
     yd.clear();
   }
 
-  auto scheduled(Slot<T>& s, size_t di, PhaseTimer* tm) {
-    return [this, &s, di, tm, ord = 0](GemmLaunch& g, int kind) mutable {
+  auto scheduled(Slot<T>& s, size_t di, PhaseTimer* tm, int ord0 = 0) {
+    return [this, &s, di, tm, ord = ord0](GemmLaunch& g, int kind) mutable {
       if (adhoc_) return gemm_adhoc<T>(g, &s.dOut->info, s.stream);
       const Sched& sc = scheds[di][ord++];
       g.info = &s.dOut->info;
@@ -904,6 +945,11 @@
     };
   }
 
+  static int lazy_wg(int fused_nwg, int part) {
+    const int forced = env_int(part == 1 ? "HBEGP_DAG_WG_P1" : "HBEGP_DAG_WG_KINV", 0);
+    return forced > 0 ? forced : fused_nwg;
+  }
+
   auto leaf_step(Slot<T>& s, PhaseTimer* tm) {
     return [this, &s, tm](int k) {
       if (tm) tm->begin(PhaseTimer::LEAF);
@@ -913,11 +959,13 @@
   }
 
   template <class Gemm, class Leaf, class Alpha>
-  void eval_gemms(Slot<T>& s, T* Kinv, Gemm&& gemm, Leaf&& leaf, Alpha&& alpha) {
+  void eval_gemms(Slot<T>& s, T* Kinv, Gemm&& gemm, Leaf&& leaf, Alpha&& alpha, int part = 0) {
     const int nb = np / NB;
-    if (!dag_) chol_inv_rec<T>(s.W1, s.W2, s.W2, np, 0, nb / 2, nb, false, true, gemm, leaf);
-    alpha();
-    if (!(dag_ && dag_lauum_)) {
+    if (part != 2) {
+      if (!dag_) chol_inv_rec<T>(s.W1, s.W2, s.W2, np, 0, nb / 2, nb, false, true, gemm, leaf);
+      alpha();
+    }
+    if (part != 1 && !(dag_ && dag_lauum_)) {
       GemmLaunch g{};
       g.nops = 1;
       GemmOp& op = g.op[0];
@@ -933,10 +981,12 @@
   void dag_report_timeout(Slot<T>& s) {
     if (!s.dag_ctrl) return;
     std::vector<int> ctrl(dag_ctrl_bytes / sizeof(int));
-    if (hipMemcpyAsync(ctrl.data(), s.dag_ctrl, dag_ctrl_bytes, hipMemcpyDeviceToHost, s.stream) != hipSuccess || hipStreamSynchronize(s.stream) != hipSuccess) return;
+    if (hipMemcpyAsync(ctrl.data(), s.dag_ctrl + (s.dag_part == 2 ? dag_ctrl_bytes / sizeof(int) : 0), dag_ctrl_bytes, hipMemcpyDeviceToHost, s.stream) != hipSuccess || hipStreamSynchronize(s.stream) != hipSuccess) return;
     const int row = ctrl[1] - 1;
-    fprintf(stderr, "task queue timeout: queue head %d of %d, first task that gave up: %d\n", ctrl[0], dag_ntasks, row);
-    const std::vector<DagTask>& host_tasks = dag_var[s.dag_variant].host_tasks;
+    const DagVariant& var = dag_var[s.dag_variant];
+    const int ntasks_here = s.dag_part == 1 ? var.ntasks_p1 : (s.dag_part == 2 ? var.ntasks_kinv : dag_ntasks);
+    fprintf(stderr, "task queue timeout: queue head %d of %d, first task that gave up: %d\n", ctrl[0], ntasks_here, row);
+    const std::vector<DagTask>& host_tasks = s.dag_part == 1 ? var.host_tasks_p1 : (s.dag_part == 2 ? var.host_tasks_kinv : var.host_tasks);
     if (row >= 0 && row < (int)host_tasks.size()) {
       const DagTask& t = host_tasks[row];
       fprintf(stderr, "  kind %d flags %x row0 %d col0 %d k [%d, %d) waits:", t.kind, t.flags, t.row0, t.col0, t.kbeg, t.kend);
@@ -946,20 +996,24 @@
     (void)hipGetLastError();
   }
 
-  void launch_queue(Slot<T>& s, size_t di, T* Kinv, PhaseTimer* tm) {
-    if (!s.ctrl_cleared) HIPCHECK(hipMemsetAsync(s.dag_ctrl, 0, dag_ctrl_bytes, s.stream));
-    s.ctrl_cleared = false;
+  void launch_queue(Slot<T>& s, size_t di, T* Kinv, PhaseTimer* tm, int part = 0) {
+    if (part != 2 && !s.ctrl_cleared) HIPCHECK(hipMemsetAsync(s.dag_ctrl, 0, dag_ctrl_regions_ * dag_ctrl_bytes, s.stream));
+    if (part != 2) s.ctrl_cleared = false;
     DagLaunch g{};
     const DagVariant& var = dag_var[s.dag_variant];
     g.tasks = var.tasks[di]; g.ntasks = dag_ntasks; g.ctrl = s.dag_ctrl;
+    int nwg = var.nwg;
+    s.dag_part = part;
+    if (part == 1) { g.tasks = var.tasks_p1[di]; g.ntasks = var.ntasks_p1; nwg = var.nwg_p1; }
+    if (part == 2) { g.tasks = var.tasks_kinv[di]; g.ntasks = var.ntasks_kinv; nwg = var.nwg_kinv; g.ctrl = s.dag_ctrl + dag_ctrl_bytes / sizeof(int); }
     g.W1 = s.W1; g.W2 = s.W2; g.ld = np; g.ldiag = s.ldiag; g.info = &s.dOut->info;
     g.W3 = s.W3;
-    g.Kinv = dag_lauum_ ? Kinv : nullptr;
+    g.Kinv = (dag_lauum_ && part != 1) ? Kinv : nullptr;
     g.trace = s.dag_trace;
     g.wait_ticks = dag_wait_ticks_;
     g.leaf_dbg = leaf_dbg_;
-    if (tm) tm->begin(PhaseTimer::DAG, 0, g.Kinv ? dag_gflop : dag_gflop - dag_gflop_lauum);
-    launch_dag<T>(g, var.nwg, s.stream);
+    if (tm) tm->begin(PhaseTimer::DAG, 0, part == 2 ? dag_gflop_lauum : (g.Kinv ? dag_gflop : dag_gflop - dag_gflop_lauum));
+    launch_dag<T>(g, nwg, s.stream);
     if (tm) tm->end();
   }
 
@@ -971,8 +1025,25 @@
     launch_small_eval<T>(g, nu2, s.stream);
   }
 
-  void enqueue_eval(Slot<T>& s, size_t di, int target, bool want_grad, PhaseTimer* tm) {
+  enum EvalMode { EVAL_LML_KINV = 0, EVAL_FULL = 1, EVAL_LML_ONLY = 2, EVAL_GRAD_ONLY = 3 };
+
+  void enqueue_eval(Slot<T>& s, size_t di, int target, int mode, PhaseTimer* tm) {
     const int* info = &s.dOut->info;
+    const bool want_grad = mode == EVAL_FULL || mode == EVAL_GRAD_ONLY;
+    if (mode == EVAL_GRAD_ONLY) {
+      if (dag_ && dag_lauum_) launch_queue(s, di, s.Kinv[target], tm, 2);
+      else eval_gemms(s, s.Kinv[target], scheduled(s, di, tm, (int)scheds[di].size() - 1), leaf_step(s, tm), [] {}, 2);
+      const bool fuse_grad = (np / 64) * (np / 64 + 1) / 2 <= 512;
+      if (tm) tm->begin(PhaseTimer::GRAD);
+      launch_gradtrace<T>(Xd[di], n, d, np, nu2, s.dP, s.Kinv[target], s.alpha[target], s.part_g, s.dOut, info, s.stream,
+                          fuse_grad ? s.tickets + 1 : nullptr, fuse_grad ? s.hOut : nullptr);
+      if (tm) tm->end();
+      if (!fuse_grad) launch_publish_out(s.dOut, s.hOut, s.dP, s.stream);
+      s.published = true;
+      CHECK_LAUNCHES();
+      return;
+    }
+    const int part = mode == EVAL_LML_ONLY ? 1 : 0;
     if (small_) {
       if (tm) tm->begin(PhaseTimer::LEAF);
       small_eval(s, di, target, 1 | 2 | (want_grad ? 4 : 0));
@@ -985,7 +1056,7 @@
       EvalPrologue pro;
       pro.dP = s.dP; pro.out = s.dOut;
       if (dag_) {
-        pro.ctrl = s.dag_ctrl; pro.ctrl_words = (int)(dag_ctrl_bytes / sizeof(int));
+        pro.ctrl = s.dag_ctrl; pro.ctrl_words = (int)(dag_ctrl_regions_ * dag_ctrl_bytes / sizeof(int));
         s.ctrl_cleared = true;
       }
       if (tm) tm->begin(PhaseTimer::KMAT);
@@ -998,12 +1069,12 @@
       launch_kmat<T>(Xd[di], n, d, np, nu2, s.dP, s.W1, info, s.stream);
       if (tm) tm->end();
     }
-    if (dag_) launch_queue(s, di, s.Kinv[target], tm);
+    if (dag_) launch_queue(s, di, s.Kinv[target], tm, dag_lauum_ ? part : 0);
     eval_gemms(s, s.Kinv[target], scheduled(s, di, tm), leaf_step(s, tm), [&] {
       if (tm) tm->begin(PhaseTimer::ALPHA);
       launch_alpha_lml<T>(s.W2, np, n, yd[di], s.ldiag, s.wbuf, s.part_t, s.alpha[target], s.dOut, info, s.stream, hostio ? s.tickets : nullptr);
       if (tm) tm->end();
-    });
+    }, part);
     bool fuse_grad = false;
     if (want_grad) {
       if (tm) tm->begin(PhaseTimer::GRAD);
@@ -1023,16 +1094,17 @@
     }
   }
 
-  void wait_eval(Slot<T>& s, std::chrono::steady_clock::time_point t_launch) {
+  void wait_eval(Slot<T>& s, std::chrono::steady_clock::time_point t_launch, int mode) {
+    long long& expect_ns = s.expect_ns[mode];
     if (s.published) {
       using namespace std::chrono;
       const volatile unsigned long long* q = &s.hOut->seq;
-      if (s.expect_ns > 1500000) {
-        const long long margin = std::max<long long>(300000, s.expect_ns / 8);
-        std::this_thread::sleep_until(t_launch + nanoseconds(s.expect_ns - margin));
+      if (expect_ns > 1500000) {
+        const long long margin = std::max<long long>(300000, expect_ns / 8);
+        std::this_thread::sleep_until(t_launch + nanoseconds(expect_ns - margin));
         if (*q == s.seq) {
           std::atomic_thread_fence(std::memory_order_acquire);
-          s.expect_ns = s.expect_ns * 9 / 10;
+          expect_ns = expect_ns * 9 / 10;
           return;
         }
       }
@@ -1040,7 +1112,7 @@
       for (unsigned it = 1;; ++it) {
         if (*q == s.seq) {
           std::atomic_thread_fence(std::memory_order_acquire);
-          s.expect_ns = duration_cast<nanoseconds>(steady_clock::now() - t_launch).count();
+          expect_ns = duration_cast<nanoseconds>(steady_clock::now() - t_launch).count();
           return;
         }
         __builtin_ia32_pause();
@@ -1152,20 +1224,27 @@
     }
     return busy <= 0 ? nvar : std::min(busy, nvar);
   }
-  int run_eval(size_t di, int si, int target, bool want_grad, bool use_graph, double* lml, double* grad) {
+  int run_eval(size_t di, int si, int target, int mode, bool use_graph, double* lml, double* grad) {
     Slot<T>& s = slots[di][si];
     HIPCHECK(hipSetDevice(s.dev));
     static const bool graphs_on = env_int("HBEGP_NO_GRAPH", 0) == 0;
-    s.dag_variant = variant_now(di);
-    s.hP->seq = ++s.seq;
+    const bool want_grad = mode == EVAL_FULL || mode == EVAL_GRAD_ONLY;
+    if (mode == EVAL_GRAD_ONLY) {
+      if (!lazy_ || !eval_published() || !grad) throw std::logic_error("run_eval: the gradient phase needs a lazily evaluated, published problem");
+      reinterpret_cast<volatile unsigned long long*>(&s.hOut->seq)[0] = 0;
+      std::atomic_thread_fence(std::memory_order_seq_cst);
+    } else {
+      s.dag_variant = variant_now(di);
+      s.hP->seq = ++s.seq;
+    }
     const auto t_launch = std::chrono::steady_clock::now();
     if (use_graph && graphs_on) {
-      hipGraphExec_t& ge = s.graph[s.dag_variant][target][want_grad ? 1 : 0];
+      hipGraphExec_t& ge = s.graph[s.dag_variant][target][mode];
       if (!ge) {
         hipGraph_t gr = nullptr;
         HIPCHECK(hipStreamBeginCapture(s.stream, hipStreamCaptureModeThreadLocal));
         try {
-          enqueue_eval(s, di, target, want_grad, nullptr);
+          enqueue_eval(s, di, target, mode, nullptr);
         } catch (...) {
           (void)hipStreamEndCapture(s.stream, &gr);
           throw;
@@ -1176,10 +1255,10 @@
       }
       HIPCHECK(hipGraphLaunch(ge, s.stream));
     } else {
-      enqueue_eval(s, di, target, want_grad, nullptr);
+      enqueue_eval(s, di, target, mode, nullptr);
     }
     s.published = eval_published();
-    wait_eval(s, t_launch);
+    wait_eval(s, t_launch, mode);
     s.last_target = target;
     const int p = d + 2;
     if (s.hOut->info < 0) {
@@ -1187,10 +1266,12 @@
       throw HipError{hipErrorLaunchTimeOut, "factorisation task queue: a dependency wait exceeded its bound", __LINE__};
     }
     if (s.hOut->info != 0) {
-      *lml = -std::numeric_limits<double>::infinity();
+      if (mode != EVAL_GRAD_ONLY) *lml = -std::numeric_limits<double>::infinity();
       if (grad) for (int j = 0; j < p; ++j) grad[j] = 0.0;
       return HBEGP_NOT_PD;
     }
+    double lml_kept = s.hOut->lml;
+    if (mode == EVAL_GRAD_ONLY) lml = &lml_kept;
     if (!(s.hOut->done & 1) || (want_grad && !(s.hOut->done & 2)))
       throw HipError{hipErrorLaunchFailure, "evaluation: the lml/gradient kernels did not run", __LINE__};
     *lml = s.hOut->lml;
@@ -2454,6 +2535,9 @@
   return HBEGP_OK;
 }
 
+struct LastFitStats { int n_evals, n_not_pd, n_lml_only; };
+static thread_local LastFitStats g_last_fit_stats = {0, 0, 0};
+
 static int read_fit_options(const hbegp_fit_options* in, hbegp_fit_options* out) {
   *out = hbegp_fit_options{};
   out->struct_size = sizeof(hbegp_fit_options);
@@ -2474,6 +2558,7 @@
                   const double* hi, const double* starts, int n_restarts, const hbegp_fit_options* opt_in,
                   double* theta_best, double* lml_best, hbegp_model** model_out, bool loo = false) {
   hbegp_fit_options opt{};
+  g_last_fit_stats = {0, 0, 0};
   if (int e = read_fit_options(opt_in, &opt)) return e;
   if (opt.maxeval <= 0) opt.maxeval = 150;
   const int p = d + 2;
@@ -2504,7 +2589,7 @@
   if (host_serial) host_lk.lock();
   const auto th0 = std::chrono::steady_clock::now();
   double held_ms = 0;
-  Problem<T> prob(ctx, X, y, n, d, nu, n_slots, false, true);
+  Problem<T> prob(ctx, X, y, n, d, nu, n_slots, false, true, !loo);
   const auto tf1 = std::chrono::steady_clock::now();
   if (!(small_fit && prob.small_)) arrival.arrived();
   if (!(small_fit && prob.small_) && host_lk.owns_lock()) host_lk.unlock();
@@ -2516,7 +2601,8 @@
   }
   std::mutex trace_mu;
   int trace_n = 0;
-  std::atomic<int> n_evals{0}, n_not_pd{0};
+  std::atomic<int> n_evals{0}, n_not_pd{0}, n_lml_only{0};
+  const bool lazy = prob.lazy_ && !loo && !(opt.trace_cap > 0 && opt.trace_grad);
   std::string err;
   std::mutex err_mu;
 
@@ -2660,6 +2746,7 @@
       if (opt.trace_count) *opt.trace_count = trace_n;
       if (opt.n_evals) *opt.n_evals = total_evals;
       if (opt.n_not_pd) *opt.n_not_pd = total_not_pd;
+      g_last_fit_stats = {total_evals, total_not_pd, 0};
       n_evals.store(total_evals);
     } catch (...) {
       for (int di = 0; di < ndev && di < (int)prob.slots.size(); ++di) {
@@ -2695,11 +2782,24 @@
         if (r == 0) for (int i = 0; i < p; ++i) x[i] = theta0[i];
         else for (int i = 0; i < p; ++i) x[i] = starts[(size_t)(r - 1) * p + i];
         int eval_idx = 0;
-        Objective obj = [&](const double* th, double* grad) -> double {
+        auto obj = [&](const double* th, double* grad, const LbfgsState* ls) -> double {
           theta_to_params(th, lo, hi, d, s.hP);
           const int target = (s.best_idx < 0) ? 0 : 1 - s.best_idx;
           double lml;
-          int st = prob.run_eval((size_t)di, si, target, !loo, true, &lml, loo ? nullptr : grad);
+          int st;
+          if (ls) {
+            st = prob.run_eval((size_t)di, si, target, Problem<T>::EVAL_LML_ONLY, true, &lml, nullptr);
+            const bool new_best = st == HBEGP_OK && (s.best_idx < 0 || lml > s.best_lml);
+            if (st == HBEGP_OK && (new_best || lbfgs_trial_accepted(*ls, -lml))) {
+              st = prob.run_eval((size_t)di, si, target, Problem<T>::EVAL_GRAD_ONLY, true, nullptr, grad);
+              if (st != HBEGP_OK) lml = -std::numeric_limits<double>::infinity();
+            } else {
+              for (int j = 0; j < p; ++j) grad[j] = 0.0;
+              n_lml_only.fetch_add(1);
+            }
+          } else {
+            st = prob.run_eval((size_t)di, si, target, !loo, true, &lml, loo ? nullptr : grad);
+          }
           if (loo) {
             if (st == HBEGP_OK) st = prob.loo_on_slot((size_t)di, si, &lml, grad);
             else for (int j = 0; j < p; ++j) grad[j] = 0.0;
@@ -2733,7 +2833,15 @@
         lo_opt.maxeval = opt.maxeval;
         lo_opt.fixed_work = opt.fixed_work != 0;
         if (opt.lbfgs_memory > 0) lo_opt.memory = opt.lbfgs_memory;
-        lbfgsb_minimize(obj, x.data(), lnlo.data(), lnhi.data(), p, lo_opt);
+        static_assert(MAXP <= LBFGS_MAXN, "the GP's parameters fit the fixed-size optimiser state");
+        std::vector<double> g(p);
+        std::unique_ptr<LbfgsState> ls(new LbfgsState);
+        lbfgs_begin(*ls, x.data(), lnlo.data(), lnhi.data(), p, lo_opt.maxeval, lo_opt.memory, lo_opt.pgtol, lo_opt.ftol, lo_opt.fixed_work);
+        for (;;) {
+          const bool trial = lazy && lbfgs_is_trial(*ls);
+          const double f = obj(lbfgs_request(*ls), g.data(), trial ? ls.get() : nullptr);
+          if (!lbfgs_advance(*ls, f, g.data())) break;
+        }
       }
     } catch (const HipError& he) {
       hip_fail(he);
@@ -2772,6 +2880,7 @@
   if (opt.trace_count) *opt.trace_count = trace_n;
   if (opt.n_evals) *opt.n_evals = n_evals.load();
   if (opt.n_not_pd) *opt.n_not_pd = n_not_pd.load();
+  g_last_fit_stats = {n_evals.load(), n_not_pd.load(), n_lml_only.load()};
   if (!err.empty()) return fail(HBEGP_EHIP, "%s", err.c_str());
   }
 
@@ -3611,26 +3720,83 @@
   if (model && model->refs.fetch_sub(1) == 1) delete model;
 }
 
+int hbegp_last_fit_stats(hbegp_fit_stats* out) {
+  if (!out || out->struct_size < offsetof(hbegp_fit_stats, n_evals) + sizeof(int) || out->struct_size > ((size_t)1 << 16))
+    return fail(HBEGP_EINVAL, "hbegp_fit_stats.struct_size: set it to sizeof(hbegp_fit_stats) (HBEGP_FIT_STATS_INIT)");
+  hbegp_fit_stats full{};
+  full.struct_size = out->struct_size;
+  full.n_evals = g_last_fit_stats.n_evals;
+  full.n_not_pd = g_last_fit_stats.n_not_pd;
+  full.n_lml_only = g_last_fit_stats.n_lml_only;
+  memcpy(out, &full, std::min(out->struct_size, sizeof(full)));
+  return HBEGP_OK;
+}
+
+static int lbfgs_replay_impl(int n, const double* x0, const double* lo, const double* hi, int maxeval, int memory, int fixed_work, int count,
+                             const double* f, const double* g, double* requested, int* trial, int* accepted, int* took, int* n_requested) {
+  LbfgsOptions o;
+  std::unique_ptr<LbfgsState> st(new LbfgsState);
+  lbfgs_begin(*st, x0, lo, hi, n, maxeval, memory > 0 ? memory : o.memory, o.pgtol, o.ftol, fixed_work != 0);
+  memcpy(requested, lbfgs_request(*st), sizeof(double) * n);
+  int produced = 1;
+  for (int i = 0; i < count; ++i) {
+    if (trial) {
+      trial[i] = lbfgs_is_trial(*st) ? 1 : 0;
+      accepted[i] = lbfgs_trial_accepted(*st, f[i]) ? 1 : 0;
+    }
+    const int it0 = st->iterations;
+    const bool more = lbfgs_advance(*st, f[i], g + (size_t)i * n);
+    if (took) took[i] = st->iterations != it0 ? 1 : 0;
+    if (!more) break;
+    if (i + 1 < count) {
+      memcpy(requested + (size_t)(i + 1) * n, lbfgs_request(*st), sizeof(double) * n);
+      produced = i + 2;
+    }
+  }
+  *n_requested = produced;
+  return HBEGP_OK;
+}
+
+int hbegp_debug_lbfgs_decisions(int n, const double* x0, const double* lo, const double* hi, int maxeval, int memory, int fixed_work,
+                                int count, const double* f, const double* g, double* requested, int* trial, int* accepted, int* took,
+                                int* n_requested) {
+  if (n < 1 || n > LBFGS_MAXN || count < 0 || !x0 || !lo || !hi || !requested || !n_requested || !trial || !accepted || !took ||
+      (count > 0 && (!f || !g)))
+    return fail(HBEGP_EINVAL, "bad argument");
+  GUARD_BEGIN
+  return lbfgs_replay_impl(n, x0, lo, hi, maxeval, memory, fixed_work, count, f, g, requested, trial, accepted, took, n_requested);
+  GUARD_END
+}
+
+int hbegp_debug_dag_queues(int nblocks, int bk, int small_h, int nwg, int fine, int big128, int which, int* ntasks, int* tasks, int cap,
+                           char* err, int errlen) {
+  if (nblocks < 1 || (bk != 16 && bk != 32) || small_h < 0 || nwg < 0 || which < 0 || which > 2 || !ntasks) return fail(HBEGP_EINVAL, "bad argument");
+  GUARD_BEGIN
+  DagBuilder builder(bk, small_h, nwg, (fine & 1) != 0);
+  builder.set_rl_progressive((fine & 16) != 0);
+  builder.set_big128(big128 != 0, big128 >= 2);
+  builder.set_rl(32, 1, (fine & 32) == 0, true);
+  DagPlan plan = builder.build(0, nblocks, which != 1, (fine & 8) != 0);
+  if (which == 2) plan = dag_plan_kinv_only(plan);
+  const std::string why = plan.tasks.empty() ? std::string("no tasks") : dag_plan_validate(plan, nblocks);
+  *ntasks = (int)plan.tasks.size();
+  if (tasks)
+    for (int i = 0; i < std::min(cap, (int)plan.tasks.size()); ++i) {
+      const DagTask& t = plan.tasks[i];
+      const int v[6] = {t.kind, t.flags, t.row0, t.col0, t.kbeg, t.kend};
+      memcpy(tasks + (size_t)6 * i, v, sizeof v);
+    }
+  if (err && errlen > 0) snprintf(err, (size_t)errlen, "%s", why.c_str());
+  return why.empty() ? HBEGP_OK : fail(HBEGP_EINVAL, "%s", why.c_str());
+  GUARD_END
+}
+
 int hbegp_debug_lbfgs_replay(int n, const double* x0, const double* lo, const double* hi, int maxeval, int memory, int fixed_work,
                              int count, const double* f, const double* g, double* requested, int* n_requested) {
   if (n < 1 || n > LBFGS_MAXN || count < 0 || !x0 || !lo || !hi || !requested || !n_requested || (count > 0 && (!f || !g)))
     return fail(HBEGP_EINVAL, "bad argument");
   GUARD_BEGIN
-  LbfgsOptions o;
-  std::unique_ptr<LbfgsState> st(new LbfgsState);
-  lbfgs_begin(*st, x0, lo, hi, n, maxeval, memory > 0 ? memory : o.memory, o.pgtol, o.ftol, fixed_work != 0);
-  int produced = 0;
-  memcpy(requested, lbfgs_request(*st), sizeof(double) * n);
-  produced = 1;
-  for (int i = 0; i < count; ++i) {
-    if (!lbfgs_advance(*st, f[i], g + (size_t)i * n)) break;
-    if (i + 1 < count) {
-      memcpy(requested + (size_t)(i + 1) * n, lbfgs_request(*st), sizeof(double) * n);
-      produced = i + 2;
-    }
-  }
-  *n_requested = produced;
-  return HBEGP_OK;
+  return lbfgs_replay_impl(n, x0, lo, hi, maxeval, memory, fixed_work, count, f, g, requested, nullptr, nullptr, nullptr, n_requested);
   GUARD_END
 }
 
diff --git a/csrc/lbfgs_step.hpp b/csrc/lbfgs_step.hpp
--- a/csrc/lbfgs_step.hpp
+++ b/csrc/lbfgs_step.hpp
@@ -150,6 +150,16 @@
 LBFGS_HD inline const double* lbfgs_request(const St& s) { return s.phase == 1 ? s.xn : s.x; }
 
 template <class St>
+LBFGS_HD inline bool lbfgs_is_trial(const St& s) { return s.phase == 1; }
+
+template <class St>
+LBFGS_HD inline bool lbfgs_trial_accepted(const St& s, double fe) {
+  if (s.phase != 1) return false;
+  if (fe != fe) fe = INFINITY;
+  return lbfgs_detail::finite(fe) && fe <= s.f + 1e-4 * s.gs;
+}
+
+template <class St>
 LBFGS_HD inline bool lbfgs_advance(St& s, double fe, const double* ge) {
   using namespace lbfgs_detail;
   const int n = s.n;
@@ -162,7 +172,7 @@
     next = finite(fe) ? begin_iteration(s) : 2;
   } else if (s.phase == 1) {
     const double fn = fe;
-    if (finite(fn) && fn <= s.f + 1e-4 * s.gs) {
+    if (lbfgs_trial_accepted(s, fn)) {
       ++s.iterations;
       double sv_stack[LbfgsWork<St>::N], yv_stack[LbfgsWork<St>::N];
       double* sv = LbfgsWork<St>::get(s, sv_stack, 2);
diff --git a/hbetune_rs_amd/_lib.py b/hbetune_rs_amd/_lib.py
--- a/hbetune_rs_amd/_lib.py
+++ b/hbetune_rs_amd/_lib.py
@@ -37,6 +37,15 @@
     def __init__(self, *a, **k):
         super().__init__(*a, **k)
         self.struct_size = C.sizeof(FitOptions)
+
+
+class FitStats(C.Structure):
+
+    _fields_ = [("struct_size", C.c_size_t), ("n_evals", C.c_int), ("n_not_pd", C.c_int), ("n_lml_only", C.c_int)]
+
+    def __init__(self, *a, **k):
+        super().__init__(*a, **k)
+        self.struct_size = C.sizeof(FitStats)
 
 
 OBJECTIVE_FN = C.CFUNCTYPE(C.c_double, C.POINTER(C.c_double), C.POINTER(C.c_double), C.c_void_p)
@@ -120,6 +129,10 @@
     "hbegp_model_retain": (None, [_vp]),
     "hbegp_model_release": (None, [_vp]),
     "hbegp_debug_lbfgs_replay": (C.c_int, [C.c_int, _dp, _dp, _dp, C.c_int, C.c_int, C.c_int, C.c_int, _dp, _dp, _dp, _ip]),
+    "hbegp_last_fit_stats": (C.c_int, [C.POINTER(FitStats)]),
+    "hbegp_debug_lbfgs_decisions": (C.c_int, [C.c_int, _dp, _dp, _dp, C.c_int, C.c_int, C.c_int, C.c_int, _dp, _dp, _dp, _ip, _ip, _ip, _ip]),
+    "hbegp_debug_dag_queues": (C.c_int, [C.c_int, C.c_int, C.c_int, C.c_int, C.c_int, C.c_int, C.c_int, _ip, _ip, C.c_int, C.c_char_p,
+                                         C.c_int]),
     "hbegp_debug_dag_plan": (C.c_int, [C.c_int, C.c_int, C.c_int, C.c_int, C.c_int, _ip, _ip, _ip, _dp, _dp, _dp, C.c_char_p,
                                        C.c_int]),
     "hbegp_minimize_by_gradient": (C.c_double, [OBJECTIVE_FN, _vp, _dp, _dp, _dp, C.c_int, C.c_int]),
diff --git a/hbetune_rs_amd/gpr.py b/hbetune_rs_amd/gpr.py
--- a/hbetune_rs_amd/gpr.py
+++ b/hbetune_rs_amd/gpr.py
@@ -229,7 +229,8 @@
             opt.trace_cap = cap
             opt.trace_theta = _lib.dptr(tr["theta"])
             opt.trace_lml = _lib.dptr(tr["lml"])
-            opt.trace_grad = _lib.dptr(tr["grad"])
+            if trace != "lml":
+                opt.trace_grad = _lib.dptr(tr["grad"])
             opt.trace_run = tr["run"].ctypes.data_as(C.POINTER(C.c_int))
             opt.trace_count = C.pointer(tr["count"])
         handle = C.c_void_p()
@@ -241,12 +242,17 @@
         fk = FittedKernel(handle, dtype, n, d, nu)
         fk.x_train, fk.y_train = x, y
         fk.n_evals, fk.n_not_pd = n_evals.value, n_not_pd.value
+        stats = _lib.FitStats()
+        _lib.check(lib.hbegp_last_fit_stats(C.byref(stats)))
+        fk.n_lml_only = stats.n_lml_only
         fk.theta_best = theta_best
         if symbol == "hbegp_fit_loo":
             fk.loo_best = lml_best.value
         if trace:
             k = tr["count"].value
-            fk.trace = dict(theta=tr["theta"][:k], lml=tr["lml"][:k], grad=tr["grad"][:k], run=tr["run"][:k])
+            fk.trace = dict(theta=tr["theta"][:k], lml=tr["lml"][:k], run=tr["run"][:k])
+            if trace != "lml":
+                fk.trace["grad"] = tr["grad"][:k]
         return fk
 
     @staticmethod
diff --git a/include/hbegp.h b/include/hbegp.h
--- a/include/hbegp.h
+++ b/include/hbegp.h
@@ -70,6 +70,15 @@
 } hbegp_fit_options;
 #define HBEGP_FIT_OPTIONS_INIT { sizeof(hbegp_fit_options) }
 
+typedef struct hbegp_fit_stats {
+  size_t struct_size;
+  int n_evals;
+  int n_not_pd;
+  int n_lml_only;
+} hbegp_fit_stats;
+#define HBEGP_FIT_STATS_INIT { sizeof(hbegp_fit_stats) }
+int hbegp_last_fit_stats(hbegp_fit_stats* out);
+
 int hbegp_fit_f64(hbegp_ctx* ctx, const double* X, const double* y, int n, int d, double nu, const double* theta0,
                   const double* lo, const double* hi, const double* starts, int n_restarts,
                   const hbegp_fit_options* opt, double* theta_best, double* lml_best, hbegp_model** model);
@@ -158,6 +167,13 @@
 
 int hbegp_debug_lbfgs_replay(int n, const double* x0, const double* lo, const double* hi, int maxeval, int memory, int fixed_work,
                              int count, const double* f, const double* g, double* requested, int* n_requested);
+
+int hbegp_debug_lbfgs_decisions(int n, const double* x0, const double* lo, const double* hi, int maxeval, int memory, int fixed_work,
+                                int count, const double* f, const double* g, double* requested, int* trial, int* accepted, int* took,
+                                int* n_requested);
+
+int hbegp_debug_dag_queues(int nblocks, int bk, int small_h, int nwg, int fine, int big128, int which, int* ntasks, int* tasks, int cap,
+                           char* err, int errlen);
 
 int hbegp_debug_posterior_phases(int enable, double* phase_ms);
 int hbegp_debug_batch_select_phases(int enable, double* phase_ms);
```

Measured after the change: 1.933 fit+predict/s (median of 6 runs). 1.09x the previous value.
